# rpng/open_vins

Hardware: NVIDIA H100
Metric: msckf_updates_per_sec (higher is better)
Workload: dtype f64

## Files before the change

### open_vins_b200/csrc/chol_tiles.cuh

```cuda
#pragma once
#include "chol.cuh"
#ifdef CQ_PROBE
#include <cstdio>
#endif

#define CT_XP 12

__device__ __forceinline__ void ct_dmma(double &d0, double &d1, double a, double b) {
  asm volatile("mma.sync.aligned.m8n8k4.row.col.f64.f64.f64.f64 {%0,%1}, {%2}, {%3}, {%0,%1};" : "+d"(d0), "+d"(d1) : "d"(a), "d"(b));
}
__device__ __forceinline__ int ct_tri(int b) { return (b * (b + 1)) >> 1; }
__device__ __forceinline__ void ct_bar_group(int id, int nthreads) { asm volatile("bar.sync %0, %1;" ::"r"(id), "r"(nthreads) : "memory"); }
__device__ __forceinline__ size_t ct_idx(int i, int j) { return (size_t)(ct_tri(i >> 3) + (j >> 3)) * 64 + (i & 7) * 8 + (j & 7); }

struct CtView {
  double *T, *Xp0, *Xp1, *invd, *Linv0, *Linv1, *dummyT, *dummyX;
  int *flag;
};
__host__ __device__ inline size_t ct_view_doubles(int NRB) {
  return (size_t)((NRB * (NRB + 1)) / 2) * 64 + 2 * (size_t)NRB * 8 * CT_XP + (size_t)NRB * 8 + 128 + 64 + 2 * CT_XP;
}
__device__ __forceinline__ CtView ct_view_carve(double *base, int NRB, int *flag_word) {
  CtView v;
  v.T = base;
// ... 53 lines not shown
        d0 = (g == j) ? d * iv : d0 * iv;
    }
    const double lg = ag * iv, lc0 = ac0 * iv, lc1 = ac1 * iv;
    if (2 * q > j)
      d0 = fma(-lg, lc0, d0);
    if (2 * q + 1 > j)
      d1 = fma(-lg, lc1, d1);
  }
  if (lane < 8)
    invd[lane] = myinv;
  if (bad && lane == 0)
    *flag = 1;
}

__device__ __forceinline__ void ct_linv8(const double *Lt, const double *invd, double *Linv) {
  const int lane = threadIdx.x & 31, cc = lane & 7;
  double mc[8];
#pragma unroll
  for (int j = 0; j < 8; j++) {
    double s0 = (j == cc) ? 1.0 : 0.0, s1 = 0.0;
#pragma unroll
    for (int t = 0; t < j; t++) {
      if (t & 1)
        s1 = fma(-Lt[j * 8 + t], mc[t], s1);
      else
        s0 = fma(-Lt[j * 8 + t], mc[t], s0);
    }
    mc[j] = (s0 + s1) * invd[j];
  }
  if (lane < 8) {
#pragma unroll
    for (int i = 0; i < 8; i++)
      Linv[i * 8 + cc] = (i >= cc) ? mc[i] : 0.0;
  }
}

__device__ __forceinline__ void ct_panel_tile(const CtView &sm, int i, int k, const double *Linv, double *Xb) {
  const int lane = threadIdx.x & 31, g = lane >> 2, q = lane & 3;
  double *t = sm.T + (size_t)(ct_tri(i) + k) * 64;
  const double a0 = t[g * 8 + q], a1 = t[g * 8 + q + 4];
  const double b0 = Linv[g * 8 + q], b1 = Linv[g * 8 + q + 4];
  double2 d = make_double2(0.0, 0.0);
  ct_dmma(d.x, d.y, a0, b0);
  ct_dmma(d.x, d.y, a1, b1);
  *reinterpret_cast<double2 *>(t + 2 * lane) = d;
  *reinterpret_cast<double2 *>(Xb + (size_t)(8 * i + g) * CT_XP + 2 * q) = d;
}

__device__ __forceinline__ void ct_panel_rows(double *T, double *Xp, const double *invd, int i0, int stride, int nrows, int k, int nbk) {
  if (i0 >= nrows)
    return;
  const double *Lk = T + (size_t)(ct_tri(k) + k) * 64;
  double L[8][8], iv[8];
#pragma unroll
  for (int c = 0; c < 8; c++) {
    iv[c] = (c < nbk) ? invd[8 * k + c] : 0.0;
#pragma unroll
    for (int t2 = 0; t2 < 4; t2++) {
      if (2 * t2 < c) {
        const double2 v = *reinterpret_cast<const double2 *>(Lk + c * 8 + 2 * t2);
        L[c][2 * t2] = v.x;
        L[c][2 * t2 + 1] = v.y;
      }
    }
  }
  for (int i = i0; i < nrows; i += stride) {
    double *src = T + (size_t)(ct_tri(i >> 3) + k) * 64 + (i & 7) * 8;
    double v[8], x[8];
    {
      const double2 v01 = *reinterpret_cast<const double2 *>(src), v23 = *reinterpret_cast<const double2 *>(src + 2);
      const double2 v45 = *reinterpret_cast<const double2 *>(src + 4), v67 = *reinterpret_cast<const double2 *>(src + 6);
      v[0] = v01.x, v[1] = v01.y, v[2] = v23.x, v[3] = v23.y, v[4] = v45.x, v[5] = v45.y, v[6] = v67.x, v[7] = v67.y;
    }
#pragma unroll
    for (int c = 0; c < 8; c++) {
      x[c] = (c < nbk) ? v[c] * iv[c] : 0.0;
#pragma unroll
      for (int t = c + 1; t < 8; t++)
        v[t] = fma(-x[c], L[t][c], v[t]);
    }
    if (nbk == 8) {
      *reinterpret_cast<double2 *>(src) = make_double2(x[0], x[1]);
      *reinterpret_cast<double2 *>(src + 2) = make_double2(x[2], x[3]);
      *reinterpret_cast<double2 *>(src + 4) = make_double2(x[4], x[5]);
      *reinterpret_cast<double2 *>(src + 6) = make_double2(x[6], x[7]);
    } else {
#pragma unroll
      for (int c = 0; c < 8; c++)
        if (c < nbk)
          src[c] = x[c];
    }
    double *xp = Xp + (size_t)i * CT_XP;
    *reinterpret_cast<double2 *>(xp) = make_double2(x[0], x[1]);
    *reinterpret_cast<double2 *>(xp + 2) = make_double2(x[2], x[3]);
    *reinterpret_cast<double2 *>(xp + 4) = make_double2(x[4], x[5]);
    *reinterpret_cast<double2 *>(xp + 6) = make_double2(x[6], x[7]);
  }
}

struct CtTileOps {
  double a0, a1, b0, b1;
  double2 c;
  double2 *cp;
};
__device__ __forceinline__ void ct_tile_load(CtTileOps &o, const CtView &sm, const double *Xp, int bi, int bj, int lane, bool valid) {
  const int g = lane >> 2, q = lane & 3;
  const double *xa = valid ? Xp + (size_t)(8 * bi + g) * CT_XP + q : sm.dummyX + q;
  const double *xb = valid ? Xp + (size_t)(8 * bj + g) * CT_XP + q : sm.dummyX + q;
  o.cp = reinterpret_cast<double2 *>((valid ? sm.T + (size_t)(ct_tri(bi) + bj) * 64 : sm.dummyT) + 2 * lane);
  o.a0 = -xa[0];
  o.a1 = -xa[4];
  o.b0 = xb[0];
  o.b1 = xb[4];
  o.c = *o.cp;
}
__device__ __forceinline__ void ct_tile_mma(CtTileOps &o) {
  ct_dmma(o.c.x, o.c.y, o.a0, o.b0);
  ct_dmma(o.c.x, o.c.y, o.a1, o.b1);
}
__device__ __forceinline__ void ct_tile_mma_store(CtTileOps &o) {
  ct_tile_mma(o);
  *o.cp = o.c;
}

#ifdef CQ_PROBE
#define CT_PROBE_T(v) v = clock64()
#else
#define CT_PROBE_T(v) do { } while (0)
#endif

__device__ __forceinline__ void ct_trail_row(const CtView &sm, const double *Xk, int bi, int j0, int jmax, int lane) {
  const int g = lane >> 2, q = lane & 3;
  const double *xa = Xk + (size_t)(8 * bi + g) * CT_XP + q;
  const double a0 = -xa[0], a1 = -xa[4];
  double *trow = sm.T + (size_t)ct_tri(bi) * 64 + 2 * lane;
  for (int bj = j0; bj <= jmax; bj += 2) {
    const bool two = bj + 1 <= jmax;
    const double *xb0 = Xk + (size_t)(8 * bj + g) * CT_XP + q;
    const double *xb1 = two ? xb0 + 8 * CT_XP : sm.dummyX + q;
    double2 *c0p = reinterpret_cast<double2 *>(trow + (size_t)bj * 64);
    double2 *c1p = two ? c0p + 32 : reinterpret_cast<double2 *>(sm.dummyT + 2 * lane);
    const double b00 = xb0[0], b01 = xb0[4], b10 = xb1[0], b11 = xb1[4];
    double2 c0 = *c0p, c1 = *c1p;
    ct_dmma(c0.x, c0.y, a0, b00);
    ct_dmma(c1.x, c1.y, a0, b10);
    ct_dmma(c0.x, c0.y, a1, b01);
    ct_dmma(c1.x, c1.y, a1, b11);
    *c0p = c0;
    *c1p = c1;
  }
}

struct CtNoPublish {
  __device__ __forceinline__ void column(const CtView &, int) const {}
};
template <int THREADS, typename PUB = CtNoPublish>
__device__ __forceinline__ void ct_chol_tiles(const CtView &sm, int n, int nrows, bool strict, double floor_d, const PUB &pub = PUB()) {
  const int tid = threadIdx.x, lane = tid & 31, wid = tid >> 5;
  constexpr int NW = THREADS / 32, NH = NW - (NW + 3) / 4;
  static_assert(NH >= 1, "need at least one helper warp");
  const bool helper = (wid & 3) != 0;
  const int hr = wid - 1 - (wid >> 2);
  constexpr bool LINV = NW >= 8;
#ifdef CQ_PROBE
  long long p0 = 0, p1 = 0, p2 = 0, p3 = 0, p4 = 0, p5 = 0, acc[6] = {0, 0, 0, 0, 0, 0};
#endif
  const int NB = (n + 7) >> 3, NRB = (nrows + 7) >> 3;
  if (wid == 0) {
    double2 c = *reinterpret_cast<const double2 *>(sm.T + 2 * lane);
    ct_diag8_frag(c.x, c.y, min(8, n), sm.invd, strict, floor_d, sm.flag);
    *reinterpret_cast<double2 *>(sm.T + 2 * lane) = c;
    __syncwarp();
    if (LINV)
      asm volatile("bar.arrive 3, 64;" ::: "memory");
    ct_panel_rows(sm.T, sm.Xp0, sm.invd, lane < 8 ? 8 + lane : nrows, 1 << 30, nrows, 0, min(8, n));
  } else if (LINV && wid == 4) {
    asm volatile("bar.sync 3, 64;" ::: "memory");
    ct_linv8(sm.T, sm.invd, sm.Linv0);
  }
  __syncthreads();
  for (int k = 0; k < NB; k++) {
    const int par = k & 1;
    double *Xk = par ? sm.Xp1 : sm.Xp0, *Xn = par ? sm.Xp0 : sm.Xp1;
    const bool more = k + 1 < NB;
    CT_PROBE_T(p0);
#ifdef CQ_PROBE
    p1 = p2 = p3 = p4 = p0;
#endif
    if (wid == 0) {
      if (more) {
        const int k1 = k + 1, nbk1 = min(8, n - 8 * k1);
        CtTileOps o;
        ct_tile_load(o, sm, Xk, k1, k1, lane, true);
        ct_tile_mma(o);
        CT_PROBE_T(p1);
        ct_diag8_frag(o.c.x, o.c.y, nbk1, sm.invd + 8 * k1, strict, floor_d, sm.flag);
        *o.cp = o.c;
        __syncwarp();
        if (LINV)
          asm volatile("bar.arrive 3, 64;" ::: "memory");
        CT_PROBE_T(p2);
        asm volatile("bar.sync 2, %0;" ::"r"((NH + 1) * 32) : "memory");
        CT_PROBE_T(p3);
        ct_panel_rows(sm.T, Xn, sm.invd, lane < 8 ? 8 * (k + 2) + lane : nrows, 1 << 30, nrows, k1, nbk1);
        CT_PROBE_T(p4);
      }
    } else if (LINV && wid == 4) {
      if (more) {
        asm volatile("bar.sync 3, 64;" ::: "memory");
        ct_linv8(sm.T + (size_t)(ct_tri(k + 1) + k + 1) * 64, sm.invd + 8 * (k + 1), par ? sm.Linv0 : sm.Linv1);
      }
    } else if (helper) {
      if (LINV) {
        const double *Lk = par ? sm.Linv1 : sm.Linv0;
        for (int i = k + 2 + hr; i < NRB; i += NH)
          ct_panel_tile(sm, i, k, Lk, Xk);
      } else {
        ct_panel_rows(sm.T, Xk, sm.invd, 8 * (k + 2) + hr * 32 + lane, NH * 32, nrows, k, min(8, n - 8 * k));
      }
      if (NH > 1)
        ct_bar_group(1, NH * 32);
      else
        __syncwarp();
      CT_PROBE_T(p1);
      if (more) {
        for (int i = k + 2 + hr; i < NRB; i += 2 * NH) {
          CtTileOps o0, o1;
          ct_tile_load(o0, sm, Xk, i, k + 1, lane, true);
          ct_tile_load(o1, sm, Xk, i + NH, k + 1, lane, i + NH < NRB);
          ct_tile_mma_store(o0);
          ct_tile_mma_store(o1);
        }
        asm volatile("bar.arrive 2, %0;" ::"r"((NH + 1) * 32) : "memory");
        CT_PROBE_T(p2);
        const int R = NRB - (k + 2), jmaxc = NB - 1;
        for (int pr = hr; 2 * pr < R; pr += NH) {
          const int rb = R - 1 - pr;
          ct_trail_row(sm, Xk, k + 2 + rb, k + 2, min(k + 2 + rb, jmaxc), lane);
          if (rb != pr)
            ct_trail_row(sm, Xk, k + 2 + pr, k + 2, min(k + 2 + pr, jmaxc), lane);
        }
      }
      CT_PROBE_T(p3);
    } else if (wid == 8 && k > 0) {
      pub.column(sm, k - 1);
    }
    __syncthreads();
    CT_PROBE_T(p5);
#ifdef CQ_PROBE
    if (wid == 0) {
      acc[0] += p1 - p0, acc[1] += p2 - p1, acc[2] += p3 - p2, acc[3] += p4 - p3, acc[4] += p5 - p4;
    } else {
      acc[0] += p1 - p0, acc[1] += p2 - p1, acc[2] += p3 - p2, acc[3] += p5 - p3;
    }
    acc[5] += p5 - p0;
#endif
  }
#ifdef CQ_PROBE
  if (tid == 0)
    printf("chol n=%d W0 (cycles over %d steps): diag update %lld pivots %lld wait %lld rows below %lld step tail %lld | %lld\n", n, NB, acc[0], acc[1], acc[2], acc[3],
           acc[4], acc[5]);
  if (tid == 32 || tid == THREADS - 32)
    printf("chol n=%d helper warp %d: panel rows %lld column k+1 %lld trailing %lld wait %lld | %lld\n", n, wid, acc[0], acc[1], acc[2], acc[3], acc[5]);
#endif
}
```

### open_vins_b200/csrc/k_cholqr.cu

```cuda
#include "chol.cuh"
#include "chol_tiles.cuh"
#include "ovb_internal.cuh"
#include <math.h>
#include <cstdio>

#define CQ_MAXN 160
#define CQ_MAXB 20
#define CQ_MAXRB 22
#define CQ_GRAM_T 512
#define CQ_KB 32
#ifndef CQ_CHOL_T
#define CQ_CHOL_T 384
#endif
#define CQ_XP CT_XP
#define CQ_TRSM_T 640

namespace {

__device__ __forceinline__ void dmma(double &d0, double &d1, double a, double b) {
  asm volatile("mma.sync.aligned.m8n8k4.row.col.f64.f64.f64.f64 {%0,%1}, {%2}, {%3}, {%0,%1};" : "+d"(d0), "+d"(d1) : "d"(a), "d"(b));
}
__device__ __forceinline__ unsigned s_u32(const void *p) { return (unsigned)__cvta_generic_to_shared(p); }
__device__ __forceinline__ void cpa16(unsigned dst, const void *src, unsigned bytes) {
  asm volatile("cp.async.cg.shared.global [%0], [%1], 16, %2;" ::"r"(dst), "l"(src), "r"(bytes) : "memory");
}
__device__ __forceinline__ void cpa8(unsigned dst, const void *src, unsigned bytes) {
  asm volatile("cp.async.ca.shared.global [%0], [%1], 8, %2;" ::"r"(dst), "l"(src), "r"(bytes) : "memory");
}
__device__ __forceinline__ void cpa_commit() { asm volatile("cp.async.commit_group;" ::: "memory"); }
template <int N> __device__ __forceinline__ void cpa_wait() { asm volatile("cp.async.wait_group %0;" ::"n"(N) : "memory"); }
__device__ __forceinline__ void bar_group(int id, int nthreads) { asm volatile("bar.sync %0, %1;" ::"r"(id), "r"(nthreads) : "memory"); }
__device__ __forceinline__ int tri(int b) { return (b * (b + 1)) >> 1; }

__device__ __forceinline__ void cq_pub_store(unsigned long long *ctr, unsigned long long v) {
  asm volatile("st.release.gpu.global.u64 [%0], %1;" ::"l"(ctr), "l"(v) : "memory");
}
__device__ __forceinline__ unsigned long long cq_pub_load(const unsigned long long *ctr) {
  unsigned long long v;
  asm volatile("ld.acquire.gpu.global.u64 %0, [%1];" : "=l"(v) : "l"(ctr) : "memory");
  return v;
}
__device__ __forceinline__ void cq_fence_proxy() { asm volatile("fence.proxy.async.global;" ::: "memory"); }
__device__ __forceinline__ void cq_mbar_init(unsigned bar) { asm volatile("mbarrier.init.shared::cta.b64 [%0], 1;" ::"r"(bar) : "memory"); }
__device__ __forceinline__ void cq_mbar_arrive(unsigned bar) { asm volatile("mbarrier.arrive.shared::cta.b64 _, [%0];" ::"r"(bar) : "memory"); }
__device__ __forceinline__ void cq_mbar_wait(unsigned bar) {
  asm volatile("{\n\t.reg .pred p;\n\tCQ_MWAIT:\n\tmbarrier.try_wait.parity.shared::cta.b64 p, [%0], 0;\n\t@!p bra CQ_MWAIT;\n\t}" ::"r"(bar) : "memory");
}

__device__ __forceinline__ bool cq_tile_origin(int blk, int w, int BW, int nblk_side, int &ci, int &cj, int &offI, int &offJ, bool &diag) {
  int bI = 0, t = blk;
  while (t >= nblk_side - bI) {
    t -= nblk_side - bI;
    bI++;
  }
  const int bJ = bI + t;
  diag = (bI == bJ);
  int a, b;
  if (diag) {
    a = 0;
    int u = w;
    while (a < BW && u >= BW - a) {
      u -= BW - a;
      a++;
    }
    if (a >= BW)
      return false;
    b = a + u;
  } else {
    if (w >= BW * BW)
      return false;
    a = w / BW;
    b = w % BW;
  }
  offI = a * 32;
  offJ = (diag ? 0 : BW * 32) + b * 32;
  ci = (bI * BW + a) * 32;
  cj = (bJ * BW + b) * 32;
  return true;
}

template <int NT>
__device__ __forceinline__ void cq_issue_rows(double *buf, int pitch, const double *__restrict__ A, int ldA, int rc, int nrows, int r1, int nt, int cI0, int cJ0,
                                              int WI, int nrng) {
  const int units_per_row = nrng * WI / 2;
  for (int e = threadIdx.x; e < nrows * units_per_row; e += NT) {
    const int k = e / units_per_row, u = e - k * units_per_row;
    const int r = rc + k;
    const int dcol = 2 * u, col = (dcol < WI) ? cI0 + dcol : cJ0 + (dcol - WI);
    unsigned bytes = 0;
    if (r < r1)
      bytes = (col + 1 < nt) ? 16u : (col < nt ? 8u : 0u);
    const double *src = bytes ? (A + (size_t)r * ldA + col) : A;
    cpa16(s_u32(buf + (size_t)k * pitch + dcol), src, bytes);
  }
  cpa_commit();
}

__device__ __forceinline__ void cq_gram_kstep(double (&acc)[4][4][2], const double *row0, int pitch, int offI, int offJ, bool same, int g, int q) {
  const double *row = row0 + (size_t)q * pitch + g;
  double fa[4], fb[4];
#pragma unroll
  for (int b = 0; b < 4; b++)
    fa[b] = row[offI + 8 * b];
  if (same) {
#pragma unroll
    for (int b = 0; b < 4; b++)
      fb[b] = fa[b];
  } else {
#pragma unroll
    for (int b = 0; b < 4; b++)
      fb[b] = row[offJ + 8 * b];
  }
#pragma unroll
  for (int a = 0; a < 4; a++)
#pragma unroll
    for (int b = 0; b < 4; b++)
      dmma(acc[a][b][0], acc[a][b][1], fa[a], fb[b]);
}

}

__global__ void __launch_bounds__(CQ_GRAM_T) k_cq_gram(const double *__restrict__ A, int ldA, int m, int nt, int slab_rows, int BW, int nblk_side,
                                                      double *__restrict__ Gpart, int cs) {
  OVB_PDL_ENTER();
  extern __shared__ __align__(16) double gsm[];
  const int tid = threadIdx.x, lane = tid & 31, wid = tid >> 5, g = lane >> 2, q = lane & 3;
  int ci, cj, offI, offJ;
  bool diag;
  const bool active = cq_tile_origin(blockIdx.x, wid, BW, nblk_side, ci, cj, offI, offJ, diag);
  int bI = 0, tt = blockIdx.x;
  while (tt >= nblk_side - bI) {
    tt -= nblk_side - bI;
    bI++;
  }
  const int bJ = bI + tt;
  const int WI = BW * 32;
  const int nrng = (bI == bJ) ? 1 : 2;
  const int pitch = nrng * WI + 4;
  const int cI0 = bI * WI, cJ0 = bJ * WI;
  const int r0 = blockIdx.y * slab_rows, r1 = min(m, r0 + slab_rows);
  const int nchunks = (r1 > r0) ? (r1 - r0 + CQ_KB - 1) / CQ_KB : 0;
  double acc[4][4][2];
#pragma unroll
  for (int a = 0; a < 4; a++)
#pragma unroll
    for (int b = 0; b < 4; b++)
      acc[a][b][0] = acc[a][b][1] = 0.0;

  auto issue = [&](int c) { cq_issue_rows<CQ_GRAM_T>(gsm + (size_t)(c & 1) * CQ_KB * pitch, pitch, A, ldA, r0 + c * CQ_KB, CQ_KB, r1, nt, cI0, cJ0, WI, nrng); };
  if (nchunks > 0)
    issue(0);
  for (int c = 0; c < nchunks; c++) {
    if (c + 1 < nchunks) {
      issue(c + 1);
      cpa_wait<1>();
    } else {
      cpa_wait<0>();
    }
    __syncthreads();
    if (active) {
      const double *buf = gsm + (size_t)(c & 1) * CQ_KB * pitch;
#pragma unroll
      for (int ks = 0; ks < CQ_KB / 4; ks++)
        cq_gram_kstep(acc, buf + (size_t)4 * ks * pitch, pitch, offI, offJ, diag && offI == offJ, g, q);
    }
    __syncthreads();
  }
  if (cs <= 1) {
    if (active) {
      double *dst = Gpart + (((size_t)blockIdx.y * gridDim.x + blockIdx.x) * 16 + wid) * 1024;
#pragma unroll
      for (int a = 0; a < 4; a++)
#pragma unroll
        for (int b = 0; b < 4; b++)
          *reinterpret_cast<double2 *>(dst + (8 * a + g) * 32 + 8 * b + 2 * q) = make_double2(acc[a][b][0], acc[a][b][1]);
    }
    return;
  }
  double *stage = gsm;
  if (active) {
    double *dst = stage + (size_t)wid * 1024;
#pragma unroll
    for (int a = 0; a < 4; a++)
#pragma unroll
      for (int b = 0; b < 4; b++)
        *reinterpret_cast<double2 *>(dst + (8 * a + g) * 32 + 8 * b + 2 * q) = make_double2(acc[a][b][0], acc[a][b][1]);
  }
  asm volatile("barrier.cluster.arrive.release.aligned;" ::: "memory");
  asm volatile("barrier.cluster.wait.acquire.aligned;" ::: "memory");
  unsigned rank;
  asm volatile("mov.u32 %0, %%cluster_ctarank;" : "=r"(rank));
  if (active) {
    const int per = 1024 / cs;
    double *dst = Gpart + ((((size_t)blockIdx.y / cs) * gridDim.x + blockIdx.x) * 16 + wid) * 1024 + (size_t)rank * per;
    const unsigned base = s_u32(stage + (size_t)wid * 1024 + (size_t)rank * per);
    for (int e = lane; e < per; e += 32) {
      double sum = 0.0;
      for (int r = 0; r < cs; r++) {
        unsigned ra;
        double v;
        asm volatile("mapa.shared::cluster.u32 %0, %1, %2;" : "=r"(ra) : "r"(base + 8u * (unsigned)e), "r"((unsigned)r));
        asm volatile("ld.shared::cluster.f64 %0, [%1];" : "=d"(v) : "r"(ra) : "memory");
        sum += v;
      }
      dst[e] = sum;
    }
  }
  asm volatile("barrier.cluster.arrive.release.aligned;" ::: "memory");
  asm volatile("barrier.cluster.wait.acquire.aligned;" ::: "memory");
}

#define CQ_RED_T 1024
#define CQ_RED_CH 8
#define CQ_RED_GX (16 * CQ_RED_CH)
__global__ void __launch_bounds__(CQ_RED_T) k_cq_reduce(const double *__restrict__ Gpart, int nslab, int nblk, int BW, int nblk_side, int nt,
                                                       double *__restrict__ G, int ldG, int tiled) {
  OVB_PDL_ENTER();
  __shared__ double red[8][128];
  int ci, cj, offI, offJ;
  bool diag;
  const int w = blockIdx.x / CQ_RED_CH, ch = blockIdx.x % CQ_RED_CH, blk = blockIdx.y;
  if (!cq_tile_origin(blk, w, BW, nblk_side, ci, cj, offI, offJ, diag))
    return;
  if (ci >= nt || cj >= nt)
    return;
  const int el = threadIdx.x & 127, sg = threadIdx.x >> 7;
  const int e = ch * 128 + el;
  const double *src = Gpart + ((size_t)blk * 16 + w) * 1024 + e;
  const size_t stride = (size_t)nblk * 16 * 1024;
  double s0 = 0.0, s1 = 0.0;
  int sl = sg;
  for (; sl + 8 < nslab; sl += 16) {
    s0 += src[(size_t)sl * stride];
    s1 += src[(size_t)(sl + 8) * stride];
  }
  if (sl < nslab)
    s0 += src[(size_t)sl * stride];
  red[sg][el] = s0 + s1;
  __syncthreads();
  if (sg == 0) {
    const int i = ci + (e >> 5), j = cj + (e & 31);
    if (i < nt && j < nt && i <= j) {
      const double s = ((red[0][el] + red[1][el]) + (red[2][el] + red[3][el])) + ((red[4][el] + red[5][el]) + (red[6][el] + red[7][el]));
      if (tiled) {
        G[ct_idx(j, i)] = s;
        if ((i >> 3) == (j >> 3))
          G[(size_t)(tri(j >> 3) + (j >> 3)) * 64 + (i & 7) * 8 + (j & 7)] = s;
      } else {
        G[(size_t)i * ldG + j] = s;
        G[(size_t)j * ldG + i] = s;
      }
    }
  }
}

struct CqCholSmem {
  double T[(CQ_MAXRB * (CQ_MAXRB + 1) / 2) * 64];
  double Xp[2][CQ_MAXRB * 8 * CQ_XP];
  double invd[CQ_MAXRB * 8];
  double Linv[2][64];
  double red[32];
  double dummyT[64];
  double dummyX[2 * CQ_XP];
  int flag;
};

#define CQ_PK_INV ((CQ_MAXB * (CQ_MAXB + 1) / 2) * 64)
#define CQ_PK_DOUBLES (CQ_PK_INV + CQ_MAXB * 8)

namespace {

struct CqPublish {
  double *Lpk;
  unsigned long long *ctr, epoch;
  int n;
  __device__ __forceinline__ void column(const CtView &sm, int k) const {
    if (ctr == nullptr)
      return;
    const int lane = threadIdx.x & 31, NB = (n + 7) >> 3;
    for (int i = k; i < NB; i++) {
      const size_t o = (size_t)(ct_tri(i) + k) * 64 + 2 * lane;
      *reinterpret_cast<double2 *>(Lpk + o) = *reinterpret_cast<const double2 *>(sm.T + o);
    }
    if (lane < 8)
      Lpk[CQ_PK_INV + 8 * k + lane] = (8 * k + lane < n) ? sm.invd[8 * k + lane] : 1.0;
    cq_fence_proxy();
    __threadfence();
    __syncwarp();
    if (lane == 0)
      cq_pub_store(ctr, (epoch << 6) | (unsigned long long)(k + 2));
  }
  __device__ __forceinline__ int first_tile_el() const { return ctr ? (tri((n + 7) >> 3) - 1) * 64 : 0; }
  __device__ __forceinline__ int first_pivot() const { return ctr ? 8 * (((n + 7) >> 3) - 1) : 0; }
  __device__ __forceinline__ void finish() const {
    if (ctr == nullptr)
      return;
    cq_fence_proxy();
    __threadfence();
    __syncthreads();
    if (threadIdx.x == 0)
      cq_pub_store(ctr, (epoch << 6) | (unsigned long long)(((n + 7) >> 3) + 1));
  }
};

__device__ __forceinline__ void cq_chol_tiles(CqCholSmem &sm, int n, int nrows, bool strict, double floor_d, const CqPublish &pub) {
  CtView v;
  v.T = sm.T;
  v.Xp0 = sm.Xp[0];
  v.Xp1 = sm.Xp[1];
  v.invd = sm.invd;
  v.Linv0 = sm.Linv[0];
  v.Linv1 = sm.Linv[1];
  v.dummyT = sm.dummyT;
  v.dummyX = sm.dummyX;
  v.flag = &sm.flag;
  ct_chol_tiles<CQ_CHOL_T>(v, n, nrows, strict, floor_d, pub);
}

__device__ void cq_load_tiles(CqCholSmem &sm, const double *__restrict__ G, size_t ldG, int n, int nrows, const double *__restrict__ rhs, int ld_rhs) {
  const int tid = threadIdx.x, lane = tid & 31, wid = tid >> 5;
  const int NB = (n + 7) >> 3, NRB = (nrows + 7) >> 3;
  for (int i = wid; i < 8 * NRB; i += CQ_CHOL_T / 32) {
    const double *row = (i >= n && rhs != nullptr) ? rhs + (size_t)(i - n) * ld_rhs : G + (size_t)i * ldG;
    const int jmax = min(i | 7, 8 * NB - 1);
    double *dst = sm.T + (size_t)tri(i >> 3) * 64 + (i & 7) * 8;
    for (int j = 2 * lane; j <= jmax; j += 64) {
      unsigned bytes = 0;
      if (i < nrows)
        bytes = (j + 1 < n) ? 16u : (j < n ? 8u : 0u);
      cpa16(s_u32(dst + (size_t)(j >> 3) * 64 + (j & 7)), bytes ? (const void *)(row + j) : (const void *)G, bytes);
    }
  }
  cpa_commit();
  for (int e = tid; e < 2 * CQ_MAXRB * 8 * CQ_XP; e += CQ_CHOL_T)
    (&sm.Xp[0][0])[e] = 0.0;
  if (tid < 64)
    sm.dummyT[tid] = 0.0;
  if (tid < 2 * CQ_XP)
    sm.dummyX[tid] = 0.0;
  if (tid == 0)
    sm.flag = 0;
  cpa_wait<0>();
}

__device__ __forceinline__ double cq_el(const double *T, int i, int j) { return T[(size_t)(tri(i >> 3) + (j >> 3)) * 64 + (i & 7) * 8 + (j & 7)]; }

}

__global__ void __launch_bounds__(CQ_CHOL_T) k_cq_chol_gram(const double *__restrict__ G, int ldG, int n, double shift_rel, double *__restrict__ Lpk, int tiled,
                                                           unsigned long long *pub_ctr, unsigned long long epoch) {
  OVB_PDL_ENTER();
  if (pub_ctr != nullptr && threadIdx.x == 0)
    cq_pub_store(pub_ctr, (epoch << 6) | 1ull);
  const CqPublish pub{Lpk, pub_ctr, epoch, n};
  extern __shared__ __align__(16) unsigned char cq_raw[];
  CqCholSmem &sm = *reinterpret_cast<CqCholSmem *>(cq_raw);
  const int tid = threadIdx.x, lane = tid & 31, wid = tid >> 5;
#ifdef CQ_PROBE
  const long long q0 = clock64();
#endif
  if (tiled) {
    __shared__ __align__(8) unsigned long long g_bar;
    const unsigned bar = s_u32(&g_bar);
    const int NB = (n + 7) >> 3;
    if (tid == 0) {
      asm volatile("mbarrier.init.shared::cta.b64 [%0], 1;" ::"r"(bar) : "memory");
      asm volatile("fence.mbarrier_init.release.cluster;" ::: "memory");
    }
    __syncthreads();
    if (tid == 0) {
      const unsigned bytes = (unsigned)(tri(NB) * 64 * sizeof(double));
      asm volatile("mbarrier.arrive.expect_tx.shared::cta.b64 _, [%0], %1;" ::"r"(bar), "r"(bytes) : "memory");
      asm volatile("cp.async.bulk.shared::cluster.global.mbarrier::complete_tx::bytes [%0], [%1], %2, [%3];" ::"r"(s_u32(sm.T)), "l"(G), "r"(bytes), "r"(bar)
                   : "memory");
    }
    for (int e = tid; e < 2 * CQ_MAXRB * 8 * CQ_XP; e += CQ_CHOL_T)
      (&sm.Xp[0][0])[e] = 0.0;
    if (tid < 64)
      sm.dummyT[tid] = 0.0;
    if (tid < 2 * CQ_XP)
      sm.dummyX[tid] = 0.0;
    if (tid == 0)
      sm.flag = 0;
    asm volatile("{\n\t.reg .pred p;\n\tCQ_GWAIT:\n\tmbarrier.try_wait.parity.shared::cta.b64 p, [%0], 0;\n\t@p bra CQ_GDONE;\n\tbra CQ_GWAIT;\n\tCQ_GDONE:\n\t}" ::"r"(bar)
                 : "memory");
    const int r0 = n - 8 * (NB - 1);
    if (r0 < 8) {
      double *last = sm.T + (size_t)tri(NB - 1) * 64;
      for (int e = tid; e < NB * 64; e += CQ_CHOL_T)
        if (((e >> 3) & 7) >= r0)
          last[e] = 0.0;
    }
  } else {
    cq_load_tiles(sm, G, (size_t)ldG, n, n, nullptr, 0);
  }
  __syncthreads();
  double mx = 0.0;
  for (int i = tid; i < n; i += CQ_CHOL_T) {
    const double d = sm.T[(size_t)(tri(i >> 3) + (i >> 3)) * 64 + (i & 7) * 9];
    mx = (d > mx) ? d : mx;
  }
#pragma unroll
  for (int o = 16; o > 0; o >>= 1) {
    const double y = __shfl_xor_sync(0xffffffffu, mx, o);
    mx = (y > mx) ? y : mx;
  }
  if (lane == 0)
    sm.red[wid] = mx;
  __syncthreads();
  mx = 0.0;
  for (int w = 0; w < CQ_CHOL_T / 32; w++)
    mx = (sm.red[w] > mx) ? sm.red[w] : mx;
  const double shift = shift_rel * mx;
  for (int i = tid; i < n; i += CQ_CHOL_T)
    sm.T[(size_t)(tri(i >> 3) + (i >> 3)) * 64 + (i & 7) * 9] += shift;
  __syncthreads();
#ifdef CQ_PROBE
  const long long q1 = clock64();
#endif
  cq_chol_tiles(sm, n, n, false, 0.25 * shift, pub);
#ifdef CQ_PROBE
  const long long q2 = clock64();
#endif
  const int NB = (n + 7) >> 3;
  for (int e = pub.first_tile_el() + 2 * tid; e < tri(NB) * 64; e += 2 * CQ_CHOL_T)
// ... 13 lines not shown
  OVB_PDL_ENTER();
  if (pub_ctr != nullptr && threadIdx.x == 0)
    cq_pub_store(pub_ctr, (epoch << 6) | 1ull);
  const CqPublish pub{Lpk, pub_ctr, epoch, r};
  extern __shared__ __align__(16) unsigned char cq_raw[];
  CqCholSmem &sm = *reinterpret_cast<CqCholSmem *>(cq_raw);
  const int tid = threadIdx.x, lane = tid & 31, wid = tid >> 5;
  const int nrows = r + (res != nullptr ? 1 : 0);
  cq_load_tiles(sm, S, (size_t)ldS, r, nrows, res, 0);
  __syncthreads();
  if (floor_dev != nullptr)
    cq_chol_tiles(sm, r, nrows, false, *floor_dev, pub);
  else
    cq_chol_tiles(sm, r, nrows, true, 0.0, pub);
  if (Lpk != nullptr) {
    const int NB = (r + 7) >> 3;
    for (int e = pub.first_tile_el() + 2 * tid; e < tri(NB) * 64; e += 2 * CQ_CHOL_T)
      *reinterpret_cast<double2 *>(Lpk + e) = *reinterpret_cast<const double2 *>(sm.T + e);
    for (int e = pub.first_pivot() + tid; e < CQ_MAXB * 8; e += CQ_CHOL_T)
      Lpk[CQ_PK_INV + e] = (e < r) ? sm.invd[e] : 1.0;
    pub.finish();
  }
  for (int i = wid; i < r; i += CQ_CHOL_T / 32)
    for (int j = lane; j <= i; j += 32)
      S[(size_t)i * ldS + j] = cq_el(sm.T, i, j);
  if (res != nullptr)
    for (int j = tid; j < r; j += CQ_CHOL_T)
      w[j] = cq_el(sm.T, r, j);
  if (invdiag != nullptr)
    for (int j = tid; j < r; j += CQ_CHOL_T)
      invdiag[j] = sm.invd[j];
  if (tid == 0 && sm.flag && info != nullptr)
    info->not_spd = 1;
}

#define CQ_TRSM_NH 10
#define CQ_TRSM_SMEM (sizeof(double) * ((size_t)CQ_PK_DOUBLES + (size_t)(CQ_TRSM_T / 32) * CQ_TRSM_NH * 2 * 32))
template <int NH, bool WAIT = false>
__device__ __forceinline__ void cq_trsm_half(double (&acc)[NH][2], int b0, const double *Lt, const double *Ri, double *xs, int lane, unsigned cbar = 0) {
  const int g = lane >> 2, q = lane & 3;
#pragma unroll
  for (int jb = 0; jb < NH; jb++) {
    const int B = b0 + jb;
    if constexpr (WAIT)
      cq_mbar_wait(cbar + 8 * B);
    const double *Ld = Lt + (size_t)(tri(B) + B) * 64;
    const double *ri = Ri + B * 8;
    double x[8];
#pragma unroll
    for (int qq = 0; qq < 4; qq++) {
      x[2 * qq] = __shfl_sync(0xffffffffu, acc[jb][0], (lane & ~3) | qq);
      x[2 * qq + 1] = __shfl_sync(0xffffffffu, acc[jb][1], (lane & ~3) | qq);
    }
#pragma unroll
    for (int c = 0; c < 8; c++) {
      x[c] *= ri[c];
#pragma unroll
      for (int c2 = c + 1; c2 < 8; c2++)
        x[c2] -= x[c] * Ld[c2 * 8 + c];
    }
    acc[jb][0] = (q == 0) ? x[0] : (q == 1) ? x[2] : (q == 2) ? x[4] : x[6];
    acc[jb][1] = (q == 0) ? x[1] : (q == 1) ? x[3] : (q == 2) ? x[5] : x[7];
    const double af0 = -((q == 0) ? x[0] : (q == 1) ? x[1] : (q == 2) ? x[2] : x[3]);
    const double af1 = -((q == 0) ? x[4] : (q == 1) ? x[5] : (q == 2) ? x[6] : x[7]);
    if (xs != nullptr) {
      xs[(2 * jb) * 32 + lane] = af0;
      xs[(2 * jb + 1) * 32 + lane] = af1;
    }
#pragma unroll
    for (int j = jb + 1; j < NH; j++) {
      const double *lf = Lt + (size_t)(tri(b0 + j) + B) * 64 + g * 8 + q;
      dmma(acc[j][0], acc[j][1], af0, lf[0]);
      dmma(acc[j][0], acc[j][1], af1, lf[4]);
    }
  }
}

template <int NH>
__device__ __forceinline__ void cq_trsm_load(double (&acc)[NH][2], const double *arow, bool row_ok, int b0, int nt, int q) {
#pragma unroll
  for (int jb = 0; jb < NH; jb++) {
    const int col = 8 * (b0 + jb) + 2 * q;
    acc[jb][0] = acc[jb][1] = 0.0;
    if (row_ok) {
      if (col + 1 < nt) {
        const double2 v = *reinterpret_cast<const double2 *>(arow + col);
        acc[jb][0] = v.x;
        acc[jb][1] = v.y;
      } else if (col < nt) {
        acc[jb][0] = arow[col];
      }
    }
  }
}
template <int NH>
__device__ __forceinline__ void cq_trsm_store(const double (&acc)[NH][2], double *arow, bool row_ok, int b0, int nt, int q) {
  if (!row_ok)
    return;
#pragma unroll
  for (int jb = 0; jb < NH; jb++) {
    const int col = 8 * (b0 + jb) + 2 * q;
    if (col + 1 < nt)
      *reinterpret_cast<double2 *>(arow + col) = make_double2(acc[jb][0], acc[jb][1]);
    else if (col < nt)
      arow[col] = acc[jb][0];
  }
}

template <int NBP, int NT>
__device__ __forceinline__ void cq_fetch_factor(double *Lt, double *Ri, const double *__restrict__ Lpk, int NB) {
  const int tid = threadIdx.x;
  __shared__ __align__(8) unsigned long long l_bar;
  const unsigned bar = s_u32(&l_bar);
  if (tid == 0) {
    asm volatile("mbarrier.init.shared::cta.b64 [%0], 1;" ::"r"(bar) : "memory");
    asm volatile("fence.mbarrier_init.release.cluster;" ::: "memory");
  }
  __syncthreads();
  if (tid == 0) {
    const unsigned bytesL = (unsigned)(tri(NB) * 64 * sizeof(double)), bytesR = (unsigned)(NB * 8 * sizeof(double));
    asm volatile("mbarrier.arrive.expect_tx.shared::cta.b64 _, [%0], %1;" ::"r"(bar), "r"(bytesL + bytesR) : "memory");
    asm volatile("cp.async.bulk.shared::cluster.global.mbarrier::complete_tx::bytes [%0], [%1], %2, [%3];" ::"r"(s_u32(Lt)), "l"(Lpk), "r"(bytesL), "r"(bar)
                 : "memory");
    asm volatile("cp.async.bulk.shared::cluster.global.mbarrier::complete_tx::bytes [%0], [%1], %2, [%3];" ::"r"(s_u32(Ri)), "l"(Lpk + CQ_PK_INV), "r"(bytesR),
                 "r"(bar)
                 : "memory");
  }
  for (int e = tri(NB) * 64 + tid; e < tri(NBP) * 64; e += NT)
    Lt[e] = 0.0;
  for (int e = NB * 8 + tid; e < NBP * 8; e += NT)
    Ri[e] = 1.0;
  asm volatile("{\n\t.reg .pred p;\n\tCQ_LWAIT:\n\tmbarrier.try_wait.parity.shared::cta.b64 p, [%0], 0;\n\t@p bra CQ_LDONE;\n\tbra CQ_LWAIT;\n\tCQ_LDONE:\n\t}" ::"r"(bar)
               : "memory");
  __syncthreads();
}

template <int NBP, int NT>
__device__ __forceinline__ void cq_stream_init(unsigned long long *bars, double *Lt, double *Ri, int NB) {
  const int tid = threadIdx.x;
  if (tid == 0) {
    for (int j = 0; j <= NBP; j++)
      cq_mbar_init(s_u32(bars + j));
    asm volatile("fence.mbarrier_init.release.cluster;" ::: "memory");
  }
  for (int e = tri(NB) * 64 + tid; e < tri(NBP) * 64; e += NT)
    Lt[e] = 0.0;
  for (int e = NB * 8 + tid; e < NBP * 8; e += NT)
    Ri[e] = 1.0;
  __syncthreads();
}

#define CQ_STREAM_POLL_NS 20000000ull

__device__ void cq_stream_fetch(unsigned long long *bars, double *Lt, double *Ri, const double *__restrict__ Lpk, int NB, int NBP,
                                const unsigned long long *ctr, unsigned long long epoch) {
  const unsigned long long base = epoch << 6;
  unsigned long long t0, t;
  asm volatile("mov.u64 %0, %%globaltimer;" : "=l"(t0));
  bool poll = true;
  auto reach = [&](int s) {
    while (poll && cq_pub_load(ctr) < (base | (unsigned long long)s)) {
      asm volatile("mov.u64 %0, %%globaltimer;" : "=l"(t));
      if (t - t0 > CQ_STREAM_POLL_NS) {
        asm volatile("griddepcontrol.wait;" ::: "memory");
        poll = false;
      } else {
        __nanosleep(64);
      }
    }
  };
  reach(1);
  cq_mbar_arrive(s_u32(bars));
  for (int j = NB; j < NBP; j++)
    cq_mbar_arrive(s_u32(bars + 1 + j));
  for (int j = 0; j < NB; j++) {
    reach(j + 2);
    cq_fence_proxy();
    const unsigned bar = s_u32(bars + 1 + j);
    asm volatile("mbarrier.arrive.expect_tx.shared::cta.b64 _, [%0], %1;" ::"r"(bar), "r"((unsigned)((NB - j) * 64 + 8) * 8u) : "memory");
    for (int i = j; i < NB; i++) {
      const size_t o = (size_t)(tri(i) + j) * 64;
      asm volatile("cp.async.bulk.shared::cluster.global.mbarrier::complete_tx::bytes [%0], [%1], 512, [%2];" ::"r"(s_u32(Lt + o)), "l"(Lpk + o), "r"(bar)
                   : "memory");
    }
    asm volatile("cp.async.bulk.shared::cluster.global.mbarrier::complete_tx::bytes [%0], [%1], 64, [%2];" ::"r"(s_u32(Ri + 8 * j)), "l"(Lpk + CQ_PK_INV + 8 * j),
                 "r"(bar)
                 : "memory");
  }
  asm volatile("griddepcontrol.wait;" ::: "memory");
  for (int j = 0; j < NB; j++)
    cq_mbar_wait(s_u32(bars + 1 + j));
}

template <int NH1, int NH2, bool STREAM>
__device__ __forceinline__ void cq_trsm_rows(double *__restrict__ A, int ldA, int m, int nt, const double *__restrict__ Lpk,
                                             const unsigned long long *__restrict__ pub_ctr, unsigned long long epoch) {
  extern __shared__ __align__(16) double tsm[];
  double *Lt = tsm;
  double *Ri = tsm + CQ_PK_INV;
  double *Xs = tsm + CQ_PK_DOUBLES;
  const int tid = threadIdx.x, lane = tid & 31, wid = tid >> 5, g = lane >> 2, q = lane & 3;
  unsigned cbar = 0;
  if constexpr (STREAM) {
    asm volatile("griddepcontrol.launch_dependents;" ::: "memory");
    __shared__ __align__(8) unsigned long long bars[CQ_MAXB + 1];
    cq_stream_init<NH1 + NH2, CQ_TRSM_T>(bars, Lt, Ri, (nt + 7) >> 3);
    if (wid == CQ_TRSM_T / 32 - 1) {
      if (lane == 0)
        cq_stream_fetch(bars, Lt, Ri, Lpk, (nt + 7) >> 3, NH1 + NH2, pub_ctr, epoch);
      return;
    }
    cq_mbar_wait(s_u32(bars));
    cbar = s_u32(bars + 1);
  } else {
    OVB_PDL_ENTER();
    cq_fetch_factor<NH1 + NH2, CQ_TRSM_T>(Lt, Ri, Lpk, (nt + 7) >> 3);
  }
  double *xs = Xs + (size_t)wid * (CQ_TRSM_NH * 2 * 32);
  const int ngroups = (m + 7) >> 3;
  constexpr int NSW = CQ_TRSM_T / 32 - (STREAM ? 1 : 0);
  for (int rg = blockIdx.x + gridDim.x * wid; rg < ngroups; rg += gridDim.x * NSW) {
    const int row = 8 * rg + g;
    const bool row_ok = row < m;
    double *arow = A + (size_t)row * ldA;
#ifdef CQ_PROBE
    long long t0 = clock64(), t1, t2, t3 = 0, t4 = 0;
#endif
    {
      double acc[NH1][2];
      cq_trsm_load<NH1>(acc, arow, row_ok, 0, nt, q);
#ifdef CQ_PROBE
      t1 = clock64();
#endif
      cq_trsm_half<NH1, STREAM>(acc, 0, Lt, Ri, NH2 > 0 ? xs : nullptr, lane, cbar);
#ifdef CQ_PROBE
      t2 = clock64();
#endif
      cq_trsm_store<NH1>(acc, arow, row_ok, 0, nt, q);
    }
    if constexpr (NH2 > 0) {
      double acc[NH2][2];
      cq_trsm_load<NH2>(acc, arow, row_ok, NH1, nt, q);
      __syncwarp();
#pragma unroll 2
      for (int jb = 0; jb < NH1; jb++) {
        const double af0 = xs[(2 * jb) * 32 + lane], af1 = xs[(2 * jb + 1) * 32 + lane];
#pragma unroll
        for (int j = 0; j < NH2; j++) {
          const double *lf = Lt + (size_t)(tri(NH1 + j) + jb) * 64 + g * 8 + q;
          dmma(acc[j][0], acc[j][1], af0, lf[0]);
          dmma(acc[j][0], acc[j][1], af1, lf[4]);
        }
      }
#ifdef CQ_PROBE
      t3 = clock64();
#endif
      cq_trsm_half<NH2, STREAM>(acc, NH1, Lt, Ri, nullptr, lane, cbar);
#ifdef CQ_PROBE
      t4 = clock64();
#endif
      cq_trsm_store<NH2>(acc, arow, row_ok, NH1, nt, q);
      __syncwarp();
    }
#ifdef CQ_PROBE
    if (blockIdx.x == 0 && (tid == 0 || tid == 32 * 7) && rg < 40)
      printf("trsm rg=%d tid=%d: load %lld half1 %lld gemm+load %lld half2 %lld total %lld\n", rg, tid, t1 - t0, t2 - t1, t3 - t2, t4 - t3, clock64() - t0);
#endif
  }
}
template <int NH1, int NH2>
__global__ void __launch_bounds__(CQ_TRSM_T) k_cq_trsm(double *__restrict__ A, int ldA, int m, int nt, const double *__restrict__ Lpk) {
  cq_trsm_rows<NH1, NH2, false>(A, ldA, m, nt, Lpk, nullptr, 0);
}
template <int NH1, int NH2>
__global__ void __launch_bounds__(CQ_TRSM_T) k_cq_trsm(double *__restrict__ A, int ldA, int m, int nt, const double *__restrict__ Lpk,
                                                      const unsigned long long *__restrict__ pub_ctr, unsigned long long epoch) {
  cq_trsm_rows<NH1, NH2, true>(A, ldA, m, nt, Lpk, pub_ctr, epoch);
}
using CqTrsmKernel = void (*)(double *, int, int, int, const double *);
using CqTrsmStreamKernel = void (*)(double *, int, int, int, const double *, const unsigned long long *, unsigned long long);

template <bool STREAM>
static void cq_launch_trsm_t(ovb_ctx *ctx, int ctas, double *A, int ldA, int m, int nt, const double *Lpk, const unsigned long long *pub_ctr,
                             unsigned long long epoch) {
  const int NB = (nt + 7) / 8;
  const size_t smem = CQ_TRSM_SMEM;
  const dim3 grid(ctas), block(CQ_TRSM_T);
  auto go = [&](auto plain, auto streaming) {
    if constexpr (STREAM)
      ovb_launch(ctx, streaming, grid, block, smem, A, ldA, m, nt, Lpk, pub_ctr, epoch);
    else
      ovb_launch(ctx, plain, grid, block, smem, A, ldA, m, nt, Lpk);
  };
  if (NB <= 5)
    go((CqTrsmKernel)k_cq_trsm<5, 0>, (CqTrsmStreamKernel)k_cq_trsm<5, 0>);
  else if (NB <= 10)
    go((CqTrsmKernel)k_cq_trsm<10, 0>, (CqTrsmStreamKernel)k_cq_trsm<10, 0>);
  else if (NB <= 15)
    go((CqTrsmKernel)k_cq_trsm<10, 5>, (CqTrsmStreamKernel)k_cq_trsm<10, 5>);
  else
    go((CqTrsmKernel)k_cq_trsm<10, 10>, (CqTrsmStreamKernel)k_cq_trsm<10, 10>);
}
static void cq_launch_trsm(ovb_ctx *ctx, int ctas, double *A, int ldA, int m, int nt, const double *Lpk, const unsigned long long *pub_ctr = nullptr,
                           unsigned long long epoch = 0) {
  if (pub_ctr != nullptr)
    cq_launch_trsm_t<true>(ctx, ctas, A, ldA, m, nt, Lpk, pub_ctr, epoch);
  else
    cq_launch_trsm_t<false>(ctx, ctas, A, ldA, m, nt, Lpk, pub_ctr, epoch);
}

#define CQ_SG_SMEM (226 * 1024)

__host__ __device__ __forceinline__ int cq_sg_pitch(int BW, int NBP) {
  const int w = (8 * NBP > 32 * BW) ? 8 * NBP : 32 * BW;
  return ((w + 15) & ~15) + 4;
}

template <int NH1, int NH2>
__device__ __forceinline__ void cq_solve_group(double *xrow, bool row_ok, const double *Lt, const double *Ri, int lane, unsigned cbar) {
  constexpr int NBP = NH1 + NH2;
  const int g = lane >> 2, q = lane & 3;
  {
    double acc[NH1][2];
    cq_trsm_load<NH1>(acc, xrow, row_ok, 0, 8 * NBP, q);
    cq_trsm_half<NH1, true>(acc, 0, Lt, Ri, nullptr, lane, cbar);
    cq_trsm_store<NH1>(acc, xrow, row_ok, 0, 8 * NBP, q);
  }
  if constexpr (NH2 > 0) {
    double acc[NH2][2];
    __syncwarp();
    cq_trsm_load<NH2>(acc, xrow, row_ok, NH1, 8 * NBP, q);
#pragma unroll 2
    for (int jb = 0; jb < NH1; jb++) {
      const double af0 = -xrow[8 * jb + q], af1 = -xrow[8 * jb + 4 + q];
#pragma unroll
      for (int j = 0; j < NH2; j++) {
        const double *lf = Lt + (size_t)(tri(NH1 + j) + jb) * 64 + g * 8 + q;
        dmma(acc[j][0], acc[j][1], af0, lf[0]);
        dmma(acc[j][0], acc[j][1], af1, lf[4]);
      }
    }
    cq_trsm_half<NH2, true>(acc, NH1, Lt, Ri, nullptr, lane, cbar);
    cq_trsm_store<NH2>(acc, xrow, row_ok, NH1, 8 * NBP, q);
  }
}

template <int NH1, int NH2>
__global__ void __launch_bounds__(CQ_GRAM_T) k_cq_solve_gram(const double *__restrict__ A, int ldA, int m, int nt, const double *__restrict__ Lpk, int slab_rows,
                                                          int cb, int ntail_max, int BW, double *__restrict__ Gpart, double *__restrict__ Qtail,
                                                          const unsigned long long *__restrict__ pub_ctr, unsigned long long epoch) {
  asm volatile("griddepcontrol.launch_dependents;" ::: "memory");
  extern __shared__ __align__(16) double ssm[];
  double *Lt = ssm;
  double *Ri = ssm + CQ_PK_INV;
  double *X = ssm + CQ_PK_DOUBLES;
  constexpr int NBP = NH1 + NH2;
  const int pitch = cq_sg_pitch(BW, NBP);
  const int r0 = blockIdx.x * slab_rows, r1 = min(m, r0 + slab_rows);
  double *tail = Qtail + (size_t)blockIdx.x * ntail_max * pitch;
  auto split_at = [&](int rc) { return r1 - rc > cb && r1 - rc <= 8 * (CQ_GRAM_T / 32); };
  auto nbuf_at = [&](int rc) { return split_at(rc) ? cb & ~7 : min(cb, (r1 - rc + 3) & ~3); };
  constexpr int NF = CQ_GRAM_T - 32;
  const int lane = threadIdx.x & 31, wid = threadIdx.x >> 5, g = lane >> 2, q = lane & 3, lr = 8 * wid + g;
  const bool fetcher = threadIdx.x >= NF;
  __shared__ __align__(8) unsigned long long bars[CQ_MAXB + 1];
  cq_stream_init<NBP, CQ_GRAM_T>(bars, Lt, Ri, (nt + 7) >> 3);
  const unsigned cbar = s_u32(bars + 1);
  if (fetcher) {
    if (lane == 0)
      cq_stream_fetch(bars, Lt, Ri, Lpk, (nt + 7) >> 3, NBP, pub_ctr, epoch);
    __syncwarp();
  } else {
    cq_mbar_wait(s_u32(bars));
    if (r0 < r1)
      cq_issue_rows<NF>(X, pitch, A, ldA, r0, nbuf_at(r0), r1, nt, 0, 0, pitch - 4, 1);
  }
  for (int rc = r0, nbuf = nbuf_at(r0), ntail = 0; rc < r1; rc += nbuf + ntail, nbuf = nbuf_at(rc)) {
    ntail = split_at(rc) ? (r1 - rc - nbuf + 3) & ~3 : 0;
    const int nact = nbuf + ntail;
    const bool first = rc == r0;
    if (!first)
      cq_issue_rows<CQ_GRAM_T>(X, pitch, A, ldA, rc, nbuf, r1, nt, 0, 0, pitch - 4, 1);
    if (!(first && fetcher))
      for (int e = threadIdx.x; e < ntail * (pitch - 4); e += first ? NF : CQ_GRAM_T) {
        const int k = e / (pitch - 4), col = e - k * (pitch - 4), r = rc + nbuf + k;
        tail[(size_t)k * pitch + col] = (r < r1 && col < nt) ? A[(size_t)r * ldA + col] : 0.0;
      }
    cpa_wait<0>();
    if (!first) {
      bar_group(1, CQ_GRAM_T);
    } else if (fetcher) {
      asm volatile("bar.sync 3, %0;" ::"n"(CQ_GRAM_T) : "memory");
    } else {
      asm volatile("bar.arrive 3, %0;" ::"n"(CQ_GRAM_T) : "memory");
      bar_group(2, NF);
    }
    if (8 * wid < nbuf)
      cq_solve_group<NH1, NH2>(X + (size_t)min(lr, nbuf - 1) * pitch, lr < nbuf, Lt, Ri, lane, cbar);
    else if (8 * wid < nact)
      cq_solve_group<NH1, NH2>(tail + (size_t)min(lr - nbuf, ntail - 1) * pitch, lr < nact, Lt, Ri, lane, cbar);
    bar_group(1, CQ_GRAM_T);
    int ci, cj, offI, offJ;
    bool diag;
    const bool active = cq_tile_origin(0, wid, BW, 1, ci, cj, offI, offJ, diag);
    double *part = Gpart + ((size_t)blockIdx.x * 16 + wid) * 1024 + g * 32 + 2 * q;
    if (active) {
      double acc[4][4][2];
#pragma unroll
      for (int a = 0; a < 4; a++)
#pragma unroll
        for (int b = 0; b < 4; b++) {
          const double2 v = rc > r0 ? *reinterpret_cast<const double2 *>(part + a * 256 + 8 * b) : make_double2(0.0, 0.0);
          acc[a][b][0] = v.x;
          acc[a][b][1] = v.y;
        }
#pragma unroll 1
      for (int k = 0; k < nact; k += 4)
        cq_gram_kstep(acc, k < nbuf ? X + (size_t)k * pitch : tail + (size_t)(k - nbuf) * pitch, pitch, offI, offJ, offI == offJ, g, q);
#pragma unroll
      for (int a = 0; a < 4; a++)
#pragma unroll
        for (int b = 0; b < 4; b++)
          *reinterpret_cast<double2 *>(part + a * 256 + 8 * b) = make_double2(acc[a][b][0], acc[a][b][1]);
    }
    bar_group(1, CQ_GRAM_T);
  }
}

struct CqSgShape {
  int pitch, cb, ntail;
};
static CqSgShape cq_sg_shape(int nt, int BW, int slab_rows) {
  const int NB = (nt + 7) / 8, NBP = NB <= 5 ? 5 : NB <= 10 ? 10 : NB <= 15 ? 15 : 20;
  CqSgShape s;
  s.pitch = cq_sg_pitch(BW, NBP);
  const int round = slab_rows < 8 * (CQ_GRAM_T / 32) ? slab_rows : 8 * (CQ_GRAM_T / 32);
  const int fit = (int)((CQ_SG_SMEM - sizeof(double) * CQ_PK_DOUBLES) / (sizeof(double) * s.pitch)) & ~3;
  s.cb = fit < round ? fit : round;
  s.ntail = slab_rows > s.cb ? round - (s.cb & ~7) : 0;
  return s;
}
static size_t cq_solve_gram_scratch(int nslab, int nt, int BW, int slab_rows) {
  const CqSgShape s = cq_sg_shape(nt, BW, slab_rows);
  return (size_t)nslab * s.ntail * s.pitch;
}

template <int NH1, int NH2>
static void cq_launch_solve_gram_t(ovb_ctx *ctx, int nslab, const double *A, int ldA, int m, int nt, const double *Lpk, int slab_rows, int BW, double *Gpart,
                                   double *Qtail, const unsigned long long *pub_ctr, unsigned long long epoch) {
  const CqSgShape s = cq_sg_shape(nt, BW, slab_rows);
  const size_t smem = sizeof(double) * (CQ_PK_DOUBLES + (size_t)s.cb * s.pitch);
  ovb_launch(ctx, k_cq_solve_gram<NH1, NH2>, dim3(nslab), dim3(CQ_GRAM_T), smem, A, ldA, m, nt, Lpk, slab_rows, s.cb, s.ntail, BW, Gpart, Qtail, pub_ctr, epoch);
}
static void cq_launch_solve_gram(ovb_ctx *ctx, int nslab, const double *A, int ldA, int m, int nt, const double *Lpk, int slab_rows, int BW, double *Gpart,
                                 double *Qtail, const unsigned long long *pub_ctr, unsigned long long epoch) {
  const int NB = (nt + 7) / 8;
  if (NB <= 5)
    cq_launch_solve_gram_t<5, 0>(ctx, nslab, A, ldA, m, nt, Lpk, slab_rows, BW, Gpart, Qtail, pub_ctr, epoch);
  else if (NB <= 10)
    cq_launch_solve_gram_t<10, 0>(ctx, nslab, A, ldA, m, nt, Lpk, slab_rows, BW, Gpart, Qtail, pub_ctr, epoch);
  else if (NB <= 15)
    cq_launch_solve_gram_t<10, 5>(ctx, nslab, A, ldA, m, nt, Lpk, slab_rows, BW, Gpart, Qtail, pub_ctr, epoch);
  else
    cq_launch_solve_gram_t<10, 10>(ctx, nslab, A, ldA, m, nt, Lpk, slab_rows, BW, Gpart, Qtail, pub_ctr, epoch);
}

__global__ void __launch_bounds__(256) k_cq_trmm(const double *__restrict__ L2, const double *__restrict__ L1, int nt, double *__restrict__ Rout, int ldR) {
  OVB_PDL_ENTER();
  __shared__ double As[16][CQ_MAXN + 1];
  __shared__ double Bs[CQ_MAXN][17];
  const int ti = blockIdx.y, tj = blockIdx.x;
  const int tid = threadIdx.x, tx = tid & 15, ty = tid >> 4;
  const int n = nt - 1;
  const int i = ti * 16 + ty, j = tj * 16 + tx;
  double acc = 0.0;
  if (tj >= ti) {
    const int k0 = ti * 16, k1 = min(nt, tj * 16 + 16);
    const int K = k1 - k0;
    for (int e = tid; e < 16 * K; e += 256) {
      const int a = e / K, k = e - a * K;
      const int ii = ti * 16 + a, kk = k0 + k;
      As[a][k] = (ii < nt && kk >= ii) ? L2[(size_t)(tri(kk >> 3) + (ii >> 3)) * 64 + (kk & 7) * 8 + (ii & 7)] : 0.0;
    }
    for (int e = tid; e < 16 * K; e += 256) {
      const int k = e >> 4, b = e & 15;
      const int kk = k0 + k, jj = tj * 16 + b;
      Bs[k][b] = (jj < nt && jj >= kk) ? L1[(size_t)(tri(jj >> 3) + (kk >> 3)) * 64 + (jj & 7) * 8 + (kk & 7)] : 0.0;
    }
    __syncthreads();
    double a0 = 0.0, a1 = 0.0, a2 = 0.0, a3 = 0.0;
    int k = 0;
    for (; k + 3 < K; k += 4) {
      a0 += As[ty][k] * Bs[k][tx];
      a1 += As[ty][k + 1] * Bs[k + 1][tx];
      a2 += As[ty][k + 2] * Bs[k + 2][tx];
      a3 += As[ty][k + 3] * Bs[k + 3][tx];
    }
    for (; k < K; k++)
      a0 += As[ty][k] * Bs[k][tx];
    acc = (a0 + a1) + (a2 + a3);
  }
  if (i < n && j < nt)
    Rout[(size_t)i * ldR + j] = (j >= i) ? acc : 0.0;
}

#define CQ_GN_T 256
__global__ void __launch_bounds__(CQ_GN_T) k_cq_gemm_nt(double *__restrict__ C, int ldc, const double *__restrict__ A, int lda, const double *__restrict__ B,
                                                       int ldb, int M, int N, int K, int lower_only) {
  OVB_PDL_ENTER();
  __shared__ __align__(16) double As[64][36];
  __shared__ __align__(16) double Bs[64][36];
  const int m0 = blockIdx.y * 64, n0 = blockIdx.x * 64;
  if (lower_only && n0 > m0 + 63)
    return;
  const int tid = threadIdx.x, lane = tid & 31, wid = tid >> 5, g = lane >> 2, q = lane & 3;
  const int wm = (wid >> 2) * 32, wn = (wid & 3) * 16;
  double acc[4][2][2];
#pragma unroll
  for (int a = 0; a < 4; a++)
#pragma unroll
    for (int b = 0; b < 2; b++)
      acc[a][b][0] = acc[a][b][1] = 0.0;
  for (int k0 = 0; k0 < K; k0 += 32) {
    for (int e = tid; e < 64 * 16; e += CQ_GN_T) {
      const int r = e >> 4, u = e & 15, k = k0 + 2 * u;
      unsigned ba = 0, bb = 0;
      if (m0 + r < M)
        ba = (k + 1 < K) ? 16u : (k < K ? 8u : 0u);
      if (n0 + r < N)
        bb = (k + 1 < K) ? 16u : (k < K ? 8u : 0u);
      cpa16(s_u32(&As[r][2 * u]), ba ? (const void *)(A + (size_t)(m0 + r) * lda + k) : (const void *)A, ba);
      cpa16(s_u32(&Bs[r][2 * u]), bb ? (const void *)(B + (size_t)(n0 + r) * ldb + k) : (const void *)B, bb);
    }
    cpa_commit();
    cpa_wait<0>();
    __syncthreads();
#pragma unroll
    for (int ks = 0; ks < 8; ks++) {
      double fa[4], fb[2];
#pragma unroll
      for (int a = 0; a < 4; a++)
        fa[a] = As[wm + 8 * a + g][4 * ks + q];
#pragma unroll
      for (int b = 0; b < 2; b++)
        fb[b] = Bs[wn + 8 * b + g][4 * ks + q];
#pragma unroll
      for (int a = 0; a < 4; a++)
#pragma unroll
        for (int b = 0; b < 2; b++)
          dmma(acc[a][b][0], acc[a][b][1], fa[a], fb[b]);
    }
    __syncthreads();
  }
#pragma unroll
  for (int a = 0; a < 4; a++)
#pragma unroll
    for (int b = 0; b < 2; b++) {
      const int i = m0 + wm + 8 * a + g, j = n0 + wn + 8 * b + 2 * q;
      if (i < M) {
        double *c = C + (size_t)i * ldc + j;
        if (j + 1 < N) {
          double2 v = *reinterpret_cast<double2 *>(c);
          v.x -= acc[a][b][0];
          v.y -= acc[a][b][1];
          *reinterpret_cast<double2 *>(c) = v;
        } else if (j < N) {
          c[0] -= acc[a][b][0];
        }
      }
    }
}

__global__ void __launch_bounds__(256) k_cq_shift(double *__restrict__ G, int ldG, int n, double shift_rel, double *__restrict__ floor_out) {
  OVB_PDL_ENTER();
  __shared__ double red[8];
  double mx = 0.0;
  for (int i = threadIdx.x; i < n; i += 256) {
    const double d = G[(size_t)i * ldG + i];
    mx = (d > mx) ? d : mx;
  }
#pragma unroll
  for (int o = 16; o > 0; o >>= 1) {
    const double y = __shfl_xor_sync(0xffffffffu, mx, o);
    mx = (y > mx) ? y : mx;
  }
  if ((threadIdx.x & 31) == 0)
    red[threadIdx.x >> 5] = mx;
  __syncthreads();
  mx = 0.0;
  for (int w = 0; w < 8; w++)
    mx = (red[w] > mx) ? red[w] : mx;
  const double shift = shift_rel * mx;
  for (int i = threadIdx.x; i < n; i += 256)
    G[(size_t)i * ldG + i] += shift;
  if (threadIdx.x == 0)
    *floor_out = 0.25 * shift;
}

__global__ void __launch_bounds__(256) k_cq_trmm_wide(const double *__restrict__ L2, const double *__restrict__ L1, int ldL, int nt, double *__restrict__ Rout,
                                                     int ldR) {
  OVB_PDL_ENTER();
  __shared__ double As[32][33];
  __shared__ double Bs[32][33];
  const int ti = blockIdx.y, tj = blockIdx.x;
  const int tid = threadIdx.x, tx = tid & 31, ty = tid >> 5;
  const int n = nt - 1;
  double acc[4] = {0, 0, 0, 0};
  if (tj >= ti) {
    for (int tk = ti; tk <= tj; tk++) {
      for (int e = tid; e < 1024; e += 256) {
        const int a = e >> 5, b = e & 31;
        const int k = tk * 32 + a, i = ti * 32 + b;
        As[a][b] = (k < nt && i < nt && k >= i) ? L2[(size_t)k * ldL + i] : 0.0;
        const int j = tj * 32 + a, k2 = tk * 32 + b;
        Bs[a][b] = (j < nt && k2 < nt && j >= k2) ? L1[(size_t)j * ldL + k2] : 0.0;
      }
      __syncthreads();
#pragma unroll 8
      for (int kk = 0; kk < 32; kk++) {
        const double b = Bs[tx][kk];
#pragma unroll
        for (int u = 0; u < 4; u++)
          acc[u] += As[kk][ty + 8 * u] * b;
      }
      __syncthreads();
    }
  }
#pragma unroll
  for (int u = 0; u < 4; u++) {
    const int i = ti * 32 + ty + 8 * u, j = tj * 32 + tx;
    if (i < n && j < nt)
      Rout[(size_t)i * ldR + j] = (j >= i) ? acc[u] : 0.0;
  }
}

#define CQ_GRAM_CS 4
static void cq_launch_gram(ovb_ctx *ctx, int nblk, int nslab_padded, size_t smem, const double *A, int ldA, int m, int nt, int slab_rows, int BW, int nblk_side,
                           double *Gpart, int cs) {
  cudaLaunchConfig_t cfg = {};
  cfg.gridDim = dim3(nblk, nslab_padded);
  cfg.blockDim = dim3(CQ_GRAM_T);
  cfg.dynamicSmemBytes = smem;
  cfg.stream = ctx->stream;
  cudaLaunchAttribute at[2];
  int na = 0;
  if (ctx->tsqr_pdl && !ctx->prof_on) {
    at[na].id = cudaLaunchAttributeProgrammaticStreamSerialization;
    at[na].val.programmaticStreamSerializationAllowed = 1;
    na++;
  }
  if (cs > 1) {
    at[na].id = cudaLaunchAttributeClusterDimension;
    at[na].val.clusterDim.x = 1;
    at[na].val.clusterDim.y = cs;
    at[na].val.clusterDim.z = 1;
    na++;
// ... 61 lines not shown
  double *Lpk = nullptr;
  if (cq_ensure_G(ctx)) {
    const int ldW = CQ_MAXN + 8;
    Lpk = ctx->d_G + (size_t)3 * ldW * ldW;
  }
  const unsigned long long epoch = (epoch_out != nullptr && Lpk != nullptr) ? ++ctx->pub_epoch : 0;
  ovb_launch(ctx, k_cq_chol_ekf, dim3(1), dim3(CQ_CHOL_T), sizeof(CqCholSmem), S, ldS, r, res, w, invdiag, ctx->d_info, Lpk, (const double *)nullptr,
             epoch ? ctx->d_pub : (unsigned long long *)nullptr, epoch);
  if (Lpk_out)
    *Lpk_out = Lpk;
  if (epoch_out)
    *epoch_out = epoch;
  return true;
}

bool launch_trsm_rows(ovb_ctx *ctx, double *A, int ldA, int m, int nt, const double *Lpk, unsigned long long epoch) {
  if (nt > CQ_MAXN || (ldA & 1) || m < 1 || Lpk == nullptr)
    return false;
  cq_attrs(ctx);
  const int ngroups = (m + 7) / 8;
  int ctas = ngroups;
  if (ctas > ctx->sm_count)
    ctas = ctx->sm_count;
  cq_launch_trsm(ctx, ctas, A, ldA, m, nt, Lpk, epoch ? ctx->d_pub : nullptr, epoch);
  return true;
}

#define CQ_WB 128
#define CQ_WMAX 520
#define CQ_WBLOCKS ((CQ_WMAX + CQ_WB - 1) / CQ_WB)
static bool cq_ensure_wide(ovb_ctx *ctx) {
  const size_t need = (size_t)2 * CQ_WMAX * CQ_WMAX + (size_t)2 * CQ_WBLOCKS * CQ_PK_DOUBLES + 64;
  if (need > ctx->cqw_cap) {
    if (ctx->d_cqw)
      cudaFree(ctx->d_cqw);
    ctx->d_cqw = nullptr;
    if (cudaMalloc(&ctx->d_cqw, sizeof(double) * need) != cudaSuccess)
      return false;
    ctx->cqw_cap = need;
  }
  return true;
}
static void cq_gemm_nt(ovb_ctx *ctx, double *C, int ldc, const double *A, int lda, const double *B, int ldb, int M, int N, int K, int lower_only) {
  if (M <= 0 || N <= 0 || K <= 0)
    return;
  ovb_launch(ctx, k_cq_gemm_nt, dim3((N + 63) / 64, (M + 63) / 64), dim3(CQ_GN_T), (size_t)0, C, ldc, A, lda, B, ldb, M, N, K, lower_only);
}
static void cq_trsm_any(ovb_ctx *ctx, double *A, int ldA, int m, int nt, const double *Lpk) {
  const int ngroups = (m + 7) / 8;
  int ctas = (ngroups + CQ_TRSM_T / 32 - 1) / (CQ_TRSM_T / 32);
  if (ngroups <= ctx->sm_count)
    ctas = ngroups;
  if (ctas > ctx->sm_count)
    ctas = ctx->sm_count;
  cq_launch_trsm(ctx, ctas, A, ldA, m, nt, Lpk);
}
static void cq_chol_blocked(ovb_ctx *ctx, double *S, int ld, int n, int extra, double *Lpk, const double *floor_dev, DevUpdateInfo *info) {
  for (int J = 0, b = 0; J < n; J += CQ_WB, b++) {
    const int nb = (n - J < CQ_WB) ? n - J : CQ_WB;
    double *Lb = Lpk + (size_t)b * CQ_PK_DOUBLES;
    ovb_launch(ctx, k_cq_chol_ekf, dim3(1), dim3(CQ_CHOL_T), sizeof(CqCholSmem), S + (size_t)J * ld + J, ld, nb, (const double *)nullptr, (double *)nullptr,
               (double *)nullptr, info, Lb, floor_dev, (unsigned long long *)nullptr, 0ull);
    const int mrem = n + extra - (J + nb);
    if (mrem > 0) {
      double *panel = S + (size_t)(J + nb) * ld + J;
      cq_trsm_any(ctx, panel, ld, mrem, nb, Lb);
      const int ncols = n - (J + nb);
      cq_gemm_nt(ctx, S + (size_t)(J + nb) * ld + (J + nb), ld, panel, ld, panel, ld, mrem, ncols, nb, 1);
    }
  }
}
static void cq_trsm_blocked(ovb_ctx *ctx, double *X, int ldx, int m, int n, const double *S, int ld, const double *Lpk) {
  for (int J = 0, b = 0; J < n; J += CQ_WB, b++) {
    const int nb = (n - J < CQ_WB) ? n - J : CQ_WB;
    if (J > 0)
      cq_gemm_nt(ctx, X + J, ldx, X, ldx, S + (size_t)J * ld, ld, m, nb, J, 0);
    cq_trsm_any(ctx, X + J, ldx, m, nb, Lpk + (size_t)b * CQ_PK_DOUBLES);
  }
}

__global__ void k_cq_copy_row(const double *__restrict__ src, double *__restrict__ dst, int n) {
  OVB_PDL_ENTER();
  const int i = blockIdx.x * blockDim.x + threadIdx.x;
  if (i < n)
    dst[i] = src[i];
}
__global__ void k_cq_inv_diag(const double *__restrict__ S, int ld, int n, double *__restrict__ inv) {
  OVB_PDL_ENTER();
  const int i = blockIdx.x * blockDim.x + threadIdx.x;
  if (i < n) {
    const double d = S[(size_t)i * ld + i];
    inv[i] = d != 0.0 ? 1.0 / d : 0.0;
  }
}

bool launch_chol_solve_wide(ovb_ctx *ctx, double *S, int ldS, int r, double *w, double *invdiag, double *M, int ldM, int N, bool gate_only) {
  if (r > CQ_WMAX - 8 || (ldS & 1) || (ldM & 1) || r + 1 > ctx->cfg.max_state + 1)
    return false;
  cq_attrs(ctx);
  if (!cq_ensure_wide(ctx))
    return false;
  double *Lpk = ctx->d_cqw + (size_t)2 * CQ_WMAX * CQ_WMAX;
  ovb_launch(ctx, k_cq_copy_row, dim3((r + 127) / 128), dim3(128), (size_t)0, (const double *)w, S + (size_t)r * ldS, r);
  cq_chol_blocked(ctx, S, ldS, r, 1, Lpk, nullptr, ctx->d_info);
  ovb_launch(ctx, k_cq_copy_row, dim3((r + 127) / 128), dim3(128), (size_t)0, (const double *)(S + (size_t)r * ldS), w, r);
  ovb_launch(ctx, k_cq_inv_diag, dim3((r + 127) / 128), dim3(128), (size_t)0, (const double *)S, ldS, r, invdiag);
  if (!gate_only)
    cq_trsm_blocked(ctx, M, ldM, N, r, S, ldS, Lpk);
  return true;
}

static int cq_compress_wide(ovb_ctx *ctx, double *A, int m, int n, int ldA, double *Rout, int ldR) {
  const int nt = n + 1;
  if (nt > CQ_WMAX - 7 || !cq_ensure_wide(ctx))
    return -1;
  const int nT = (nt + 31) / 32, BW = 4, nblk_side = (nT + BW - 1) / BW, nblk = nblk_side * (nblk_side + 1) / 2;
  int nslab = ctx->sm_count / nblk;
  if (nslab < 1)
    nslab = 1;
  const int max_slabs = (m + CQ_KB - 1) / CQ_KB;
  if (nslab > max_slabs)
    nslab = max_slabs;
  int slab_rows = (((m + nslab - 1) / nslab) + 3) & ~3;
  nslab = (m + slab_rows - 1) / slab_rows;
  const size_t need_part = (size_t)nslab * nblk * 16 * 1024;
  if (need_part > ctx->Gpart_cap) {
    if (ctx->d_Gpart)
      cudaFree(ctx->d_Gpart);
    ctx->d_Gpart = nullptr;
    if (cudaMalloc(&ctx->d_Gpart, sizeof(double) * need_part) != cudaSuccess)
      return -1;
    ctx->Gpart_cap = need_part;
  }
  double *G1 = ctx->d_cqw, *G2 = G1 + (size_t)CQ_WMAX * CQ_WMAX, *Lpk1 = G2 + (size_t)CQ_WMAX * CQ_WMAX, *Lpk2 = Lpk1 + (size_t)CQ_WBLOCKS * CQ_PK_DOUBLES;
  double *floor_dev = Lpk2 + (size_t)CQ_WBLOCKS * CQ_PK_DOUBLES;
  const size_t gram_smem = sizeof(double) * 2 * CQ_KB * (size_t)(2 * BW * 32 + 4);
  int launches = 0;
  for (int pass = 0; pass < 2; pass++) {
    double *G = pass == 0 ? G1 : G2;
    cq_launch_gram(ctx, nblk, nslab, gram_smem, (const double *)A, ldA, m, nt, slab_rows, BW, nblk_side, ctx->d_Gpart, 1);
    ovb_launch(ctx, k_cq_reduce, dim3(CQ_RED_GX, nblk), dim3(CQ_RED_T), (size_t)0, (const double *)ctx->d_Gpart, nslab, nblk, BW, nblk_side, nt, G, (int)CQ_WMAX, 0);
    ovb_launch(ctx, k_cq_shift, dim3(1), dim3(256), (size_t)0, G, (int)CQ_WMAX, nt, pass == 0 ? 1e-11 : 1e-13, floor_dev + pass);
    cq_chol_blocked(ctx, G, CQ_WMAX, nt, 0, pass == 0 ? Lpk1 : Lpk2, floor_dev + pass, (DevUpdateInfo *)nullptr);
    if (pass == 0)
      cq_trsm_blocked(ctx, A, ldA, m, nt, G1, CQ_WMAX, Lpk1);
    launches += 3 + 3 * ((nt + CQ_WB - 1) / CQ_WB);
  }
  const int nT32 = (nt + 31) / 32;
  ovb_launch(ctx, k_cq_trmm_wide, dim3(nT32, nT32), dim3(256), (size_t)0, (const double *)G2, (const double *)G1, (int)CQ_WMAX, nt, Rout, ldR);
  ctx->n_launch += launches + 1;
  return launches + 1;
}

int launch_compress_cholqr2(ovb_ctx *ctx, double *A, int m, int n, int ldA, double *Rout, int ldR) {
  const int nt = n + 1;
  if ((ldA & 1) || m < 1)
    return -1;
  cq_attrs(ctx);
  if (nt > CQ_MAXN)
    return cq_compress_wide(ctx, A, m, n, ldA, Rout, ldR);
  const int nT = (nt + 31) / 32;
  const int BW = nT, nblk_side = 1, nblk = 1;
  int nslab = ctx->sm_count;
  const int max_slabs = (m + CQ_KB - 1) / CQ_KB;
  if (nslab > max_slabs)
    nslab = max_slabs;
  int slab_rows = (m + nslab - 1) / nslab;
  slab_rows = (slab_rows + 3) & ~3;
  nslab = (m + slab_rows - 1) / slab_rows;
  const int cs = (ctx->gram_cluster && nslab >= 2 * CQ_GRAM_CS) ? CQ_GRAM_CS : 1;
  const int nslab_pad = (nslab + cs - 1) / cs * cs, npart = nslab_pad / cs;
  const size_t part_doubles = (size_t)nslab_pad * nblk * 16 * 1024;
  const size_t need_part = part_doubles + cq_solve_gram_scratch(nslab, nt, BW, slab_rows);
  const int ldW = CQ_MAXN + 8;
  if (!cq_ensure_G(ctx))
    return -1;
  if (need_part > ctx->Gpart_cap) {
    const size_t cap = need_part + need_part / 2;
    if (ctx->d_Gpart)
      cudaFree(ctx->d_Gpart);
    ctx->d_Gpart = nullptr;
    ctx->Gpart_cap = 0;
    if (cudaMalloc(&ctx->d_Gpart, sizeof(double) * cap) != cudaSuccess)
      return -1;
    ctx->Gpart_cap = cap;
  }
  double *G = ctx->d_G, *L1 = G + (size_t)ldW * ldW, *L2 = L1 + (size_t)ldW * ldW;
  static_assert(CQ_PK_DOUBLES <= (CQ_MAXN + 8) * (CQ_MAXN + 8), "packed factor must fit its slot");
  size_t gram_smem = sizeof(double) * 2 * CQ_KB * (size_t)(BW * 32 + 4);
  if (cs > 1 && gram_smem < sizeof(double) * 16 * 1024)
    gram_smem = sizeof(double) * 16 * 1024;
  cq_launch_gram(ctx, nblk, nslab_pad, gram_smem, (const double *)A, ldA, m, nt, slab_rows, BW, nblk_side, ctx->d_Gpart, cs);
  ovb_launch(ctx, k_cq_reduce, dim3(CQ_RED_GX, nblk), dim3(CQ_RED_T), (size_t)0, (const double *)ctx->d_Gpart, npart, nblk, BW, nblk_side, nt, G, ldW, 1);
  const unsigned long long epoch = ++ctx->pub_epoch;
  ovb_launch(ctx, k_cq_chol_gram, dim3(1), dim3(CQ_CHOL_T), sizeof(CqCholSmem), (const double *)G, ldW, nt, 1e-11, L1, 1, ctx->d_pub, epoch);
  cq_launch_solve_gram(ctx, nslab, (const double *)A, ldA, m, nt, (const double *)L1, slab_rows, BW, ctx->d_Gpart, ctx->d_Gpart + part_doubles, ctx->d_pub, epoch);
  ovb_launch(ctx, k_cq_reduce, dim3(CQ_RED_GX, nblk), dim3(CQ_RED_T), (size_t)0, (const double *)ctx->d_Gpart, nslab, nblk, BW, nblk_side, nt, G, ldW, 1);
  ovb_launch(ctx, k_cq_chol_gram, dim3(1), dim3(CQ_CHOL_T), sizeof(CqCholSmem), (const double *)G, ldW, nt, 1e-13, L2, 1, (unsigned long long *)nullptr, 0ull);
  const int nT16 = (nt + 15) / 16;
  ovb_launch(ctx, k_cq_trmm, dim3(nT16, nT16), dim3(256), (size_t)0, (const double *)L2, (const double *)L1, nt, Rout, ldR);
  ctx->n_launch += 7;
  return 7;
}
```

### open_vins_b200/csrc/k_ekf.cu

```cuda
#include "chol.cuh"
#include "ovb_internal.cuh"

#define EK_T 32

__global__ void __launch_bounds__(256) k_ekf_gemm(int mode, const double *__restrict__ P, int ldP, const double *__restrict__ H, int ldH,
                                                  const double *__restrict__ Min, int ldM, const DevUpdateInfo *__restrict__ info, int X, int Y,
                                                  int K, double *__restrict__ Cout, int ldC, double sigma2, const double *__restrict__ Rdiag) {
  OVB_PDL_ENTER();
  __shared__ double As[EK_T][EK_T + 1];
  __shared__ double Bs[EK_T][EK_T + 1];
  const int x0 = blockIdx.x * EK_T, y0 = blockIdx.y * EK_T;
  if (mode == 1 && y0 > x0 + EK_T - 1)
    return;
  const int tid = threadIdx.x, tx = tid & 31, ty = tid >> 5;
  double acc[4] = {0, 0, 0, 0};
  const int *cs = info->col_state;
  for (int j0 = 0; j0 < K; j0 += EK_T) {
    for (int e = tid; e < EK_T * EK_T; e += 256) {
      int jj = e >> 5, q = e & 31;
      int j = j0 + jj;
      double av = 0.0, bv = 0.0;
      if (j < K) {
        if (mode == 0) {
          int a = x0 + q;
// ... 192 lines not shown
    if (a < N && b < N && b >= a) {
      double v = P[(size_t)a * ldP + b] - acc[u];
      P[(size_t)a * ldP + b] = v;
      P[(size_t)b * ldP + a] = v;
      if (a == b && v < 0.0)
        atomicMin(&info->neg_diag_index, a);
      if (!isfinite(v))
        info->nonfinite = 1;
    }
  }
  if (a0 == b0 && tid < EK_T && a0 + tid < N)
    dx[a0 + tid] = dxa;
}

#define EK1_KMAX 160
__device__ __forceinline__ void ek_cpa8(double *dst_smem, const double *src) {
  asm volatile("cp.async.ca.shared.global [%0], [%1], 8;" ::"r"((unsigned)__cvta_generic_to_shared(dst_smem)), "l"(src) : "memory");
}
__global__ void __launch_bounds__(256) k_ekf_gemm1(int mode, const double *__restrict__ P, int ldP, const double *__restrict__ H, int ldH,
                                                   const double *__restrict__ Min, int ldM, const DevUpdateInfo *__restrict__ info, int X, int Y,
                                                   int K, double *__restrict__ Cout, int ldC, double sigma2, const double *__restrict__ Rdiag) {
  OVB_PDL_ENTER();
  extern __shared__ __align__(16) double g1[];
  const int x0 = blockIdx.x * EK_T, y0 = blockIdx.y * EK_T;
  if (mode == 1 && y0 > x0 + EK_T - 1)
    return;
  const int tid = threadIdx.x, tx = tid & 31, ty = tid >> 5;
  const int *cs = info->col_state;
  const int pk = K | 1;
  double *Gs = g1, *Hs = g1 + (size_t)K * 33;
  const double *Gsrc = (mode == 0) ? P : Min;
  const int ldG = (mode == 0) ? ldP : ldM;
  const int g0 = (mode == 0) ? x0 : y0, gmax = (mode == 0) ? X : Y;
  const int h0 = (mode == 0) ? y0 : x0, hmax = (mode == 0) ? Y : X;
  __shared__ int cs_s[EK1_KMAX];
  for (int j = tid; j < K; j += 256)
    cs_s[j] = cs[j];
  __syncthreads();
  for (int e = tid; e < K * 32; e += 256) {
    const int j = e >> 5, a = e & 31;
    if (g0 + a < gmax)
      ek_cpa8(&Gs[j * 33 + a], &Gsrc[(size_t)cs_s[j] * ldG + g0 + a]);
    else
      Gs[j * 33 + a] = 0.0;
  }
  for (int i = ty; i < 32; i += 8)
    for (int j = tx; j < K; j += 32) {
      if (h0 + i < hmax)
        ek_cpa8(&Hs[i * pk + j], &H[(size_t)(h0 + i) * ldH + j]);
      else
        Hs[i * pk + j] = 0.0;
    }
  asm volatile("cp.async.commit_group;" ::: "memory");
  asm volatile("cp.async.wait_group 0;" ::: "memory");
  __syncthreads();
  double acc[4] = {0, 0, 0, 0};
  if (mode == 0) {
    for (int j = 0; j < K; j++) {
      const double gv = Gs[j * 33 + tx];
#pragma unroll
      for (int u = 0; u < 4; u++)
        acc[u] += gv * Hs[(ty + 8 * u) * pk + j];
    }
#pragma unroll
    for (int u = 0; u < 4; u++) {
      const int a = x0 + tx, i = y0 + ty + 8 * u;
      if (a < X && i < Y)
        Cout[(size_t)a * ldC + i] = acc[u];
    }
  } else {
    for (int j = 0; j < K; j++) {
      const double gv = Gs[j * 33 + tx];
#pragma unroll
      for (int u = 0; u < 4; u++)
        acc[u] += Hs[(ty + 8 * u) * pk + j] * gv;
    }
#pragma unroll
    for (int u = 0; u < 4; u++) {
      const int i = x0 + ty + 8 * u, k = y0 + tx;
      if (i < X && k < Y) {
        double v = acc[u];
        if (i == k)
          v += Rdiag ? Rdiag[i] : sigma2;
        Cout[(size_t)i * ldC + k] = v;
      }
    }
  }
}

__global__ void __launch_bounds__(256) k_ekf_downdate1(double *__restrict__ P, int ldP, const double *__restrict__ Yin, int ldY, int N, int r,
                                                       const double *__restrict__ w, double *__restrict__ dx, DevUpdateInfo *__restrict__ info) {
  OVB_PDL_ENTER();
  extern __shared__ __align__(16) double d1[];
  const int a0 = blockIdx.x * EK_T, b0 = blockIdx.y * EK_T;
  if (b0 < a0)
    return;
  const int tid = threadIdx.x, tx = tid & 31, ty = tid >> 5;
  if (info->not_spd) {
    if (a0 == b0 && tid < EK_T && a0 + tid < N)
      dx[a0 + tid] = 0.0;
    return;
  }
  const int pk = r | 1;
  double *As = d1, *Bs = d1 + (size_t)32 * pk, *ws = Bs + (size_t)32 * pk;
  for (int i = ty; i < 32; i += 8)
    for (int k = tx; k < r; k += 32) {
      if (a0 + i < N)
        ek_cpa8(&As[i * pk + k], &Yin[(size_t)(a0 + i) * ldY + k]);
      else
        As[i * pk + k] = 0.0;
      if (b0 + i < N)
        ek_cpa8(&Bs[i * pk + k], &Yin[(size_t)(b0 + i) * ldY + k]);
      else
        Bs[i * pk + k] = 0.0;
    }
  for (int k = tid; k < r; k += 256)
    ek_cpa8(&ws[k], &w[k]);
  asm volatile("cp.async.commit_group;" ::: "memory");
  asm volatile("cp.async.wait_group 0;" ::: "memory");
  __syncthreads();
  double acc[4] = {0, 0, 0, 0};
  for (int k = 0; k < r; k++) {
    const double bv = Bs[tx * pk + k];
#pragma unroll
    for (int u = 0; u < 4; u++)
      acc[u] += As[(ty + 8 * u) * pk + k] * bv;
  }
#pragma unroll
  for (int u = 0; u < 4; u++) {
    const int a = a0 + ty + 8 * u, b = b0 + tx;
    if (a < N && b < N && b >= a) {
      const double v = P[(size_t)a * ldP + b] - acc[u];
      P[(size_t)a * ldP + b] = v;
      P[(size_t)b * ldP + a] = v;
      if (a == b && v < 0.0)
        atomicMin(&info->neg_diag_index, a);
      if (!isfinite(v))
        info->nonfinite = 1;
    }
  }
  if (a0 == b0 && tid < EK_T && a0 + tid < N) {
    double s0 = 0.0, s1 = 0.0;
    int k = 0;
    for (; k + 1 < r; k += 2) {
      s0 += As[tid * pk + k] * ws[k];
      s1 += As[tid * pk + k + 1] * ws[k + 1];
    }
    if (k < r)
      s0 += As[tid * pk + k] * ws[k];
    dx[a0 + tid] = s0 + s1;
  }
}

__global__ void k_ekf_prep(DevUpdateInfo *info, const int *skip) {
  OVB_PDL_ENTER();
  info->neg_diag_index = 0x7fffffff;
  info->not_spd = (skip && *skip) ? 1 : 0;
  info->nonfinite = 0;
}

void launch_ekf_update(ovb_ctx *ctx, const double *H, int ldHm, int r, int n, bool gate_only, double sigma2, const double *Rdiag_dev,
                       const int *skip_dev) {
  const int N = ctx->N;
  const int ld = ctx->ldP;
  double *P = ctx->P[ctx->cur];
  ovb_launch(ctx, k_ekf_prep, dim3(1), dim3(1), (size_t)(0), ctx->d_info, skip_dev);
  if (r <= 0 || n <= 0)
    return;
  if (!ctx->attr_done[2]) {
    cudaFuncSetAttribute(k_ekf_chol, cudaFuncAttributeMaxDynamicSharedMemorySize, 200 * 1024);
    cudaFuncSetAttribute(k_ekf_trsm, cudaFuncAttributeMaxDynamicSharedMemorySize, 200 * 1024);
    cudaFuncSetAttribute(k_ekf_gemm1, cudaFuncAttributeMaxDynamicSharedMemorySize, 100 * 1024);
    cudaFuncSetAttribute(k_ekf_downdate1, cudaFuncAttributeMaxDynamicSharedMemorySize, 100 * 1024);
    ctx->attr_done[2] = 1;
  }
  const bool one_shot = ctx->ekf_chol_dmma && n <= EK1_KMAX && r <= EK1_KMAX;
  dim3 g0((N + EK_T - 1) / EK_T, (r + EK_T - 1) / EK_T);
  dim3 g1((r + EK_T - 1) / EK_T, (r + EK_T - 1) / EK_T);
  if (one_shot) {
    const size_t sm01 = sizeof(double) * ((size_t)n * 33 + (size_t)32 * (n | 1));
    ovb_launch(ctx, k_ekf_gemm1, dim3(g0), dim3(256), sm01, 0, P, ld, H, ldHm, nullptr, 0, ctx->d_info, N, r, n, ctx->d_M, ld, 0.0, nullptr);
    ovb_launch(ctx, k_ekf_gemm1, dim3(g1), dim3(256), sm01, 1, P, ld, H, ldHm, ctx->d_M, ld, ctx->d_info, r, r, n, ctx->d_S, ld, sigma2, Rdiag_dev);
  } else {
    ovb_launch(ctx, k_ekf_gemm, dim3(g0), dim3(256), (size_t)(0), 0, P, ld, H, ldHm, nullptr, 0, ctx->d_info, N, r, n, ctx->d_M, ld, 0.0, nullptr);
    ovb_launch(ctx, k_ekf_gemm, dim3(g1), dim3(256), (size_t)(0), 1, P, ld, H, ldHm, ctx->d_M, ld, ctx->d_info, r, r, n, ctx->d_S, ld, sigma2, Rdiag_dev);
  }
  size_t chol_bytes = sizeof(double) * (size_t)(r + 1) * (size_t)(r | 1);
  int use_smem = chol_bytes <= 200 * 1024;
  double *invdiag = ctx->d_w + ctx->cfg.max_state;
  double *Lpk = nullptr;
  unsigned long long epoch = 0;
  const bool dmma_chol = ctx->ekf_chol_dmma && launch_chol_ekf_dmma(ctx, ctx->d_S, ld, r, ctx->d_w, ctx->d_w, invdiag, &Lpk, gate_only ? nullptr : &epoch);
  const bool wide = !dmma_chol && ctx->ekf_chol_dmma && r < ld && launch_chol_solve_wide(ctx, ctx->d_S, ld, r, ctx->d_w, invdiag, ctx->d_M, ld, N, gate_only);
  if (wide) {
    if (gate_only)
      return;
    dim3 g2w((N + EK_T - 1) / EK_T, (N + EK_T - 1) / EK_T);
    ovb_launch(ctx, k_ekf_downdate, dim3(g2w), dim3(256), (size_t)(0), P, ld, (const double *)ctx->d_M, ld, N, r, ctx->d_w, ctx->d_dx, ctx->d_info);
    return;
  }
  if (!dmma_chol)
    ovb_launch(ctx, k_ekf_chol, dim3(1), dim3(EKC_THREADS), (size_t)(use_smem ? chol_bytes : 0), ctx->d_S, ld, r, ctx->d_w, ctx->d_w, invdiag, ctx->d_info, use_smem);
  if (gate_only)
    return;
  const double *Yd = ctx->d_Y;
  if (dmma_chol && Lpk != nullptr && launch_trsm_rows(ctx, ctx->d_M, ld, N, r, Lpk, epoch)) {
    Yd = ctx->d_M;
  } else {
    size_t trsm_small = sizeof(double) * ((size_t)TR_ROWS * r + r);
    size_t trsm_full = trsm_small + sizeof(double) * (size_t)r * (size_t)(r | 1);
    int L_in_smem = trsm_full <= 200 * 1024;
    ovb_launch(ctx, k_ekf_trsm, dim3((N + TR_ROWS - 1) / TR_ROWS), dim3(32 * TR_ROWS), (size_t)(L_in_smem ? trsm_full : trsm_small), ctx->d_M, ld, ctx->d_S, ld, invdiag, N,
               r, ctx->d_Y, ld, L_in_smem, ctx->d_info);
  }
  dim3 g2((N + EK_T - 1) / EK_T, (N + EK_T - 1) / EK_T);
  if (one_shot) {
    const size_t smd = sizeof(double) * ((size_t)64 * (r | 1) + r);
    ovb_launch(ctx, k_ekf_downdate1, dim3(g2), dim3(256), smd, P, ld, Yd, ld, N, r, ctx->d_w, ctx->d_dx, ctx->d_info);
  } else {
    ovb_launch(ctx, k_ekf_downdate, dim3(g2), dim3(256), (size_t)(0), P, ld, Yd, ld, N, r, ctx->d_w, ctx->d_dx, ctx->d_info);
  }
}


__global__ void k_cov_init_augment(double *__restrict__ P, int ld, int N, int k, int n, const DevUpdateInfo *__restrict__ info,
                                   const double *__restrict__ Hx, const double *__restrict__ Hinv, double sigma2, const int *__restrict__ skip) {
  extern __shared__ double ism[];
  double *m = ism, *M = ism + (size_t)N * k;
  const int tid = threadIdx.x;
  if (skip && *skip)
    return;
  for (int a = tid; a < N; a += blockDim.x) {
    for (int i = 0; i < k; i++) {
      double acc = 0.0;
      for (int j = 0; j < n; j++)
        acc += P[(size_t)a * ld + info->col_state[j]] * Hx[i * n + j];
      m[a * k + i] = acc;
    }
  }
  __syncthreads();
  if (tid < k * k) {
    const int i = tid / k, i2 = tid % k;
    double acc = 0.0;
    for (int j = 0; j < n; j++)
      acc += Hx[i * n + j] * m[info->col_state[j] * k + i2];
    M[i * k + i2] = acc + (i == i2 ? sigma2 : 0.0);
  }
  __syncthreads();
  if (tid < k * k) {
    const int i = tid / k, i2 = tid % k;
    if (i2 < i)
      M[i * k + i2] = M[i2 * k + i];
  }
  __syncthreads();
  for (int a = tid; a < N; a += blockDim.x) {
    for (int q = 0; q < k; q++) {
      double acc = 0.0;
      for (int i = 0; i < k; i++)
        acc += m[a * k + i] * Hinv[q * k + i];
      P[(size_t)a * ld + N + q] = -acc;
      P[(size_t)(N + q) * ld + a] = -acc;
    }
  }
  if (tid < k * k) {
    const int q = tid / k, q2 = tid % k;
    double acc = 0.0;
    for (int i = 0; i < k; i++)
      for (int i2 = 0; i2 < k; i2++)
        acc += Hinv[q * k + i] * M[i * k + i2] * Hinv[q2 * k + i2];
    if (q <= q2) {
      P[(size_t)(N + q) * ld + N + q2] = acc;
      P[(size_t)(N + q2) * ld + N + q] = acc;
    }
  }
}

bool launch_cov_init_augment(ovb_ctx *ctx, int k, int n, const double *Hx_dev, const double *Hinv_dev, double sigma2, const int *skip_dev) {
  const int N = ctx->N;
  size_t smem = sizeof(double) * ((size_t)N * k + (size_t)k * k);
  if (smem > 200 * 1024)
    return false;
  if (!ctx->attr_done[5]) {
    cudaFuncSetAttribute(k_cov_init_augment, cudaFuncAttributeMaxDynamicSharedMemorySize, 200 * 1024);
    ctx->attr_done[5] = 1;
  }
  k_cov_init_augment<<<1, 256, smem, ctx->stream>>>(ctx->P[ctx->cur], ctx->ldP, N, k, n, ctx->d_info, Hx_dev, Hinv_dev, sigma2, skip_dev);
  return cudaGetLastError() == cudaSuccess;
}

__global__ void k_init_prep(const DevFeat *__restrict__ feat, DevInitSys *__restrict__ sys, DevUpdateInfo *__restrict__ info, int k, int n) {
  const int tid = threadIdx.x;
  const bool ok = feat->status == OVB_FEAT_OK;
  if (ok)
    for (int j = tid; j < n; j += blockDim.x)
      info->col_state[j] = sys->col_state[j];
  if (tid != 0)
    return;
  sys->status = feat->status;
  sys->chi2 = feat->chi2;
  int fail = sys->n != n ? 2 : 0;
  const int o = 3 - k;
  double A[9], Inv[9];
  for (int i = 0; i < k; i++)
    for (int j = 0; j < k; j++) {
      A[i * k + j] = sys->HL[(o + i) * 3 + o + j];
      Inv[i * k + j] = (i == j) ? 1.0 : 0.0;
    }
  for (int c0 = 0; c0 < k && !fail; c0++) {
    int piv = c0;
    for (int i = c0 + 1; i < k; i++)
      if (fabs(A[i * k + c0]) > fabs(A[piv * k + c0]))
        piv = i;
    if (!(fabs(A[piv * k + c0]) > 0.0)) {
      fail = 1;
      break;
    }
    if (piv != c0)
      for (int j = 0; j < k; j++) {
        double t = A[c0 * k + j];
        A[c0 * k + j] = A[piv * k + j];
        A[piv * k + j] = t;
        t = Inv[c0 * k + j];
        Inv[c0 * k + j] = Inv[piv * k + j];
        Inv[piv * k + j] = t;
      }
    const double d = A[c0 * k + c0];
    for (int j = 0; j < k; j++) {
      A[c0 * k + j] /= d;
      Inv[c0 * k + j] /= d;
    }
    for (int i = 0; i < k; i++) {
      if (i == c0)
        continue;
      const double f = A[i * k + c0];
      for (int j = 0; j < k; j++) {
        A[i * k + j] -= f * A[c0 * k + j];
        Inv[i * k + j] -= f * Inv[c0 * k + j];
      }
    }
  }
  for (int q = 0; q < 3; q++) {
    double acc = 0.0;
    if (q < k)
      for (int i = 0; i < k; i++)
        acc += Inv[q * k + i] * sys->res[o + i];
    sys->dx_new[q] = acc;
  }
  for (int i = 0; i < k * k; i++)
    sys->Hinv[i] = Inv[i];
  sys->fail = ok ? fail : 0;
  sys->skip = (!ok || fail) ? 1 : 0;
}

void launch_init_prep(ovb_ctx *ctx, int feat, int k, int n) {
  k_init_prep<<<1, 256, 0, ctx->stream>>>(ctx->d_feat + feat, ctx->d_init, ctx->d_info, k, n);
}

__global__ void k_cov_clone(double *P, int ld, int N, int old_off, int size, const int *neg_diag) {
  int idx = blockIdx.x * blockDim.x + threadIdx.x;
  int N2 = N + size;
  if (idx >= N2 * size || (neg_diag && *neg_diag != 0x7fffffff))
    return;
  int i = idx / size, j = idx % size;
  double v;
  if (i < N)
    v = P[(size_t)i * ld + old_off + j];
  else
    v = P[(size_t)(old_off + (i - N)) * ld + old_off + j];
  double vr = (i < N) ? P[(size_t)(old_off + j) * ld + i] : v;
  P[(size_t)i * ld + N + j] = v;
  if (i < N)
    P[(size_t)(N + j) * ld + i] = vr;
}
__global__ void k_cov_dt_cols(double *P, int ld, int N2, int new_off, int size, int dt_off, const double *dnc, const int *neg_diag) {
  int idx = blockIdx.x * blockDim.x + threadIdx.x;
  if (idx >= N2 * size || (neg_diag && *neg_diag != 0x7fffffff))
    return;
  int i = idx / size, j = idx % size;
  P[(size_t)i * ld + new_off + j] += P[(size_t)i * ld + dt_off] * dnc[j];
}
__global__ void k_cov_dt_rows(double *P, int ld, int N2, int new_off, int size, int dt_off, const double *dnc, const int *neg_diag) {
  int idx = blockIdx.x * blockDim.x + threadIdx.x;
  if (idx >= N2 * size || (neg_diag && *neg_diag != 0x7fffffff))
    return;
  int i = idx / N2, j = idx % N2;
  P[(size_t)(new_off + i) * ld + j] += dnc[i] * P[(size_t)dt_off * ld + j];
}

void launch_cov_clone(ovb_ctx *ctx, int old_off, int size, const double *dnc_dt_dev, int dt_off, const int *neg_diag_dev) {
  double *P = ctx->P[ctx->cur];
  int N = ctx->N, N2 = N + size;
  int tot = N2 * size;
  k_cov_clone<<<(tot + 255) / 256, 256, 0, ctx->stream>>>(P, ctx->ldP, N, old_off, size, neg_diag_dev);
  if (dnc_dt_dev) {
    k_cov_dt_cols<<<(tot + 255) / 256, 256, 0, ctx->stream>>>(P, ctx->ldP, N2, N, size, dt_off, dnc_dt_dev, neg_diag_dev);
    k_cov_dt_rows<<<(tot + 255) / 256, 256, 0, ctx->stream>>>(P, ctx->ldP, N2, N, size, dt_off, dnc_dt_dev, neg_diag_dev);
  }
}

__global__ void k_cov_marg(const double *Pin, double *Pout, int ld, int N, int off, int size) {
  int N2 = N - size;
  int i = blockIdx.y * blockDim.y + threadIdx.y, j = blockIdx.x * blockDim.x + threadIdx.x;
  if (i >= N2 || j >= N2)
    return;
  int si = i < off ? i : i + size, sj = j < off ? j : j + size;
  double v = (i >= off && j < off) ? Pin[(size_t)sj * ld + si] : Pin[(size_t)si * ld + sj];
  Pout[(size_t)i * ld + j] = v;
}

void launch_cov_marginalize(ovb_ctx *ctx, int off, int size) {
  int N2 = ctx->N - size;
  dim3 b(32, 8), g((N2 + 31) / 32, (N2 + 7) / 8);
  k_cov_marg<<<g, b, 0, ctx->stream>>>(ctx->P[ctx->cur], ctx->P[ctx->cur ^ 1], ctx->ldP, ctx->N, off, size);
}

__global__ void k_prop_C(const double *P, int ld, int N, int p, int q, const int *old_idx, const double *Phi, double *Cbuf, int ldC) {
  int idx = blockIdx.x * blockDim.x + threadIdx.x;
  if (idx >= N * p)
    return;
  int a = idx / p, j = idx % p;
  double acc = 0.0;
  for (int k = 0; k < q; k++)
    acc += P[(size_t)a * ld + old_idx[k]] * Phi[(size_t)j * q + k];
  Cbuf[(size_t)a * ldC + j] = acc;
}
__global__ void k_prop_PCP(const double *Cbuf, int ldC, int p, int q, const int *old_idx, const double *Phi, const double *Q, double *Sbuf,
                           int ldS) {
  int idx = blockIdx.x * blockDim.x + threadIdx.x;
  if (idx >= p * p)
    return;
  int i = idx / p, j = idx % p;
  double acc = (i <= j) ? Q[(size_t)i * p + j] : Q[(size_t)j * p + i];
  for (int k = 0; k < q; k++)
    acc += Phi[(size_t)i * q + k] * Cbuf[(size_t)old_idx[k] * ldC + j];
  Sbuf[(size_t)i * ldS + j] = acc;
}
__global__ void k_prop_write(double *P, int ld, int N, int new_off, int p, const double *Cbuf, int ldC, const double *Sbuf, int ldS,
                             DevUpdateInfo *info) {
  int idx = blockIdx.x * blockDim.x + threadIdx.x;
  if (idx >= N * p)
    return;
  int a = idx / p, j = idx % p;
  if (a >= new_off && a < new_off + p) {
    double v = Sbuf[(size_t)(a - new_off) * ldS + j];
    P[(size_t)a * ld + new_off + j] = v;
    if (a - new_off == j && v < 0.0)
      atomicMin(&info->neg_diag_index, a);
  } else {
    double v = Cbuf[(size_t)a * ldC + j];
    P[(size_t)a * ld + new_off + j] = v;
    P[(size_t)(new_off + j) * ld + a] = v;
  }
}

void launch_cov_propagate(ovb_ctx *ctx, int new_off, int p, int q, const int *old_idx_dev, const double *Phi_dev, const double *Q_dev) {
  double *P = ctx->P[ctx->cur];
  int N = ctx->N, ld = ctx->ldP;
  ovb_launch(ctx, k_ekf_prep, dim3(1), dim3(1), (size_t)(0), ctx->d_info, (const int *)nullptr);
  k_prop_C<<<(N * p + 255) / 256, 256, 0, ctx->stream>>>(P, ld, N, p, q, old_idx_dev, Phi_dev, ctx->d_M, ld);
  k_prop_PCP<<<(p * p + 255) / 256, 256, 0, ctx->stream>>>(ctx->d_M, ld, p, q, old_idx_dev, Phi_dev, Q_dev, ctx->d_S, ld);
  k_prop_write<<<(N * p + 255) / 256, 256, 0, ctx->stream>>>(P, ld, N, new_off, p, ctx->d_M, ld, ctx->d_S, ld, ctx->d_info);
}

#define PA_THREADS 1024

__device__ __forceinline__ void pa_stage(double *dst, const double *src, int count, int tid) {
  for (int e = tid; e < count; e += PA_THREADS) {
    const unsigned d = (unsigned)__cvta_generic_to_shared(dst + e);
    asm volatile("cp.async.ca.shared.global [%0], [%1], 8;" ::"r"(d), "l"(src + e) : "memory");
  }
}

__global__ void __launch_bounds__(PA_THREADS) k_prop_accumulate(int n, int steps, const double *__restrict__ F, const double *__restrict__ G,
                                                                const double *__restrict__ qc, double *__restrict__ Phi_out,
                                                                double *__restrict__ Q_out) {
  extern __shared__ double pa_sm[];
  const int tid = threadIdx.x, nn = n * n, rec = nn + 12 * n + 4, npairs = n * (n + 1) / 2;
  double *Phi = pa_sm, *Phi2 = Phi + nn, *Q = Phi2 + nn, *T = Q + nn, *stg = T + nn;
  unsigned char *pi = (unsigned char *)(stg + 2 * rec), *pj = pi + npairs;
  for (int e = tid; e < nn; e += PA_THREADS) {
    Phi[e] = (e / n == e % n) ? 1.0 : 0.0;
    Q[e] = 0.0;
  }
  if (tid < n)
    for (int j = tid, t = tid * n - tid * (tid - 1) / 2; j < n; j++, t++)
      pi[t] = (unsigned char)tid, pj[t] = (unsigned char)j;
  auto stage = [&](int s) {
    double *r = stg + (s & 1) * rec;
    pa_stage(r, F + (size_t)s * nn, nn, tid);
    pa_stage(r + nn, G + (size_t)s * 12 * n, 12 * n, tid);
    pa_stage(r + nn + 12 * n, qc + (size_t)s * 4, 4, tid);
    asm volatile("cp.async.commit_group;" ::: "memory");
  };
  if (steps > 0)
    stage(0);
  for (int s = 0; s < steps; s++) {
    asm volatile("cp.async.wait_all;" ::: "memory");
    __syncthreads();
    if (s + 1 < steps)
      stage(s + 1);
    const double *f = stg + (s & 1) * rec, *g = f + nn, *w = g + 12 * n;
    for (int e = tid; e < 2 * nn; e += PA_THREADS) {
      const bool phi = e >= nn;
      const int ee = phi ? e - nn : e, i = ee / n, j = ee % n;
      const double *B = phi ? Phi : Q;
      double acc = 0.0;
      for (int k = 0; k < n; k++)
        acc = __dadd_rn(acc, __dmul_rn(f[i * n + k], B[k * n + j]));
      (phi ? Phi2 : T)[ee] = acc;
    }
    __syncthreads();
    for (int t = tid; t < npairs; t += PA_THREADS) {
      const int i = pi[t], j = pj[t];
      double qij = 0.0, qji = 0.0, tij = 0.0, tji = 0.0;
      for (int k = 0; k < 12; k++) {
        qij = __dadd_rn(qij, __dmul_rn(__dmul_rn(g[i * 12 + k], w[k / 3]), g[j * 12 + k]));
        qji = __dadd_rn(qji, __dmul_rn(__dmul_rn(g[j * 12 + k], w[k / 3]), g[i * 12 + k]));
      }
      for (int k = 0; k < n; k++) {
        tij = __dadd_rn(tij, __dmul_rn(T[i * n + k], f[j * n + k]));
        tji = __dadd_rn(tji, __dmul_rn(T[j * n + k], f[i * n + k]));
      }
      const double qd = __dmul_rn(0.5, __dadd_rn(qij, qji));
      const double v = __dmul_rn(0.5, __dadd_rn(__dadd_rn(tij, qd), __dadd_rn(tji, qd)));
      Q[i * n + j] = v;
      Q[j * n + i] = v;
    }
    double *x = Phi;
    Phi = Phi2, Phi2 = x;
  }
  __syncthreads();
  for (int e = tid; e < nn; e += PA_THREADS) {
    Phi_out[e] = Phi[e];
    Q_out[e] = Q[e];
  }
}

static size_t prop_accumulate_smem(int n) {
  const size_t nn = (size_t)n * n;
  return sizeof(double) * (4 * nn + 2 * (nn + 12 * (size_t)n + 4)) + (size_t)n * (n + 1);
}

bool launch_prop_accumulate(ovb_ctx *ctx, int n, int steps, const double *F_dev, const double *G_dev, const double *qc_dev, double *Phi_dev,
                            double *Q_dev) {
  const size_t smem = prop_accumulate_smem(n);
  if (!ctx->attr_done[7]) {
    if (cudaFuncSetAttribute(k_prop_accumulate, cudaFuncAttributeMaxDynamicSharedMemorySize, (int)prop_accumulate_smem(OVB_PROP_MAX_N)) != cudaSuccess)
      return false;
    ctx->attr_done[7] = 1;
  }
  k_prop_accumulate<<<1, PA_THREADS, smem, ctx->stream>>>(n, steps, F_dev, G_dev, qc_dev, Phi_dev, Q_dev);
  return cudaGetLastError() == cudaSuccess;
}
```

### open_vins_b200/csrc/ovb_api.cu

```cuda
#include "ovb_internal.cuh"
#include <chrono>
#include <algorithm>
#include <cmath>
#include <cstdio>
#include <cstdlib>
#include <cstring>
#include <new>
#include <vector>

static const double g_chi2_table[OVB_CHI2_TABLE_LEN] = {
#include "chi2_table.inc"
};

unsigned char *ovb_feat_order_ptr(ovb_ctx *ctx) { return ctx->d_feat_order; }

static size_t align_up(size_t v, size_t a) { return (v + a - 1) / a * a; }

extern "C" {

static ovb_status ensure_stage(ovb_ctx *ctx, size_t doubles);

int ovb_abi_version(void) { return OVB_ABI_VERSION; }

double ovb_chi2_quantile95(int dof) {
// ... 782 lines not shown
    e = cudaMemcpyAsync(ctx->d_grp, ctx->h_grp, sizeof(DevGroup) * (size_t)pk->n_groups, cudaMemcpyHostToDevice, ctx->stream);
    ctx->last_h2d_bytes += sizeof(DevGroup) * (size_t)pk->n_groups;
  }
  if (e != cudaSuccess) {
    snprintf(ctx->err, sizeof(ctx->err), "H2D arena copy: %s", cudaGetErrorString(e));
    return OVB_ERR_CUDA;
  }
  return OVB_OK;
}

static void unpack_feats(ovb_ctx *ctx, int F, ovb_feat_out *out) {
  if (!out)
    return;
  for (int f = 0; f < F; f++) {
    const DevFeat &d = ctx->h_feat[f];
    if (out->status)
      out->status[f] = d.status;
    if (out->anchor_cam)
      out->anchor_cam[f] = d.anchor_cam;
    if (out->anchor_clone)
      out->anchor_clone[f] = d.anchor_clone;
    if (out->chi2)
      out->chi2[f] = d.chi2;
    for (int k = 0; k < 3; k++) {
      if (out->p_FinA)
        out->p_FinA[3 * f + k] = d.p_FinA[k];
      if (out->p_FinG)
        out->p_FinG[3 * f + k] = d.p_FinG[k];
    }
  }
}

ovb_status ovb_triangulate(ovb_ctx *ctx, const ovb_frame *frame, const ovb_feat_batch *feats, const ovb_opts *opts, ovb_feat_out *out) {
  if (!ctx || !out)
    return OVB_ERR_ARG;
  OVB_CUDA_CHECK(ctx, cudaSetDevice(ctx->device));
  Packed pk;
  int saveN = ctx->N;
  if (ctx->N == 0)
    ctx->N = ctx->cfg.max_state;
  ovb_status st = pack_inputs(ctx, frame, feats, opts, nullptr, &pk, nullptr, false);
  ctx->N = saveN;
  if (st != OVB_OK)
    return st;
  launch_cam_poses(ctx);
  launch_triangulate(ctx, pk.n_feats, pk.bv);
  OVB_CUDA_CHECK(ctx, cudaGetLastError());
  OVB_CUDA_CHECK(ctx, cudaMemcpyAsync(ctx->h_feat, ctx->d_feat, sizeof(DevFeat) * (size_t)pk.n_feats, cudaMemcpyDeviceToHost, ctx->stream));
  OVB_CUDA_CHECK(ctx, cudaStreamSynchronize(ctx->stream));
  unpack_feats(ctx, pk.n_feats, out);
  return OVB_OK;
}

ovb_status ovb_feature_jacobians(ovb_ctx *ctx, const ovb_frame *frame, const ovb_feat_batch *feats, const ovb_opts *opts, ovb_feat_out *out,
                                 int stage, double *Hf_out, double *Hx_out, double *res_out, int32_t *row_off_out, int32_t *ncols_out,
                                 int32_t *col_index_out, int ld_out) {
  if (!ctx || !out || !row_off_out || !ncols_out || !col_index_out)
    return OVB_ERR_ARG;
  if (ctx->N < 1) {
    snprintf(ctx->err, sizeof(ctx->err), "ovb_feature_jacobians: no covariance loaded (ovb_cov_set)");
    return OVB_ERR_ARG;
  }
  OVB_CUDA_CHECK(ctx, cudaSetDevice(ctx->device));
  Packed pk;
  ovb_status st = pack_inputs(ctx, frame, feats, opts, out, &pk);
  if (st != OVB_OK)
    return st;
  const int F = pk.n_feats, n_all = pk.n_all;
  if (ld_out < n_all)
    return OVB_ERR_ARG;
  *ncols_out = n_all;
  for (int s = 0, c = 0; s < ctx->h_frame->n_slots; s++)
    for (int k = 0; k < ctx->h_frame->slot_size[s]; k++)
      col_index_out[c++] = ctx->h_frame->slot_off[s] + k;
  launch_cam_poses(ctx);
  if (stage == 0) {
    int rows = 2 * pk.n_meas;
    size_t need = (size_t)rows * (OVB_MAX_COLS + 4);
    if (!ctx->d_dump || need > ctx->dump_cap) {
      if (ctx->d_dump)
        cudaFree(ctx->d_dump);
      ctx->dump_cap = need;
      OVB_CUDA_CHECK(ctx, cudaMalloc(&ctx->d_dump, sizeof(double) * ctx->dump_cap));
    }
    ctx->dump_rows = rows;
    OVB_CUDA_CHECK(ctx, cudaMemsetAsync(ctx->d_dump, 0, sizeof(double) * need, ctx->stream));
    launch_feature_system(ctx, F, pk.bv, pk.ldH, 1);
    OVB_CUDA_CHECK(ctx, cudaGetLastError());
    std::vector<double> host(need);
    OVB_CUDA_CHECK(ctx, cudaMemcpyAsync(host.data(), ctx->d_dump, sizeof(double) * need, cudaMemcpyDeviceToHost, ctx->stream));
    OVB_CUDA_CHECK(ctx, cudaStreamSynchronize(ctx->stream));
    int dump_rows = rows;
    const double *dHf = host.data(), *dres = host.data() + (size_t)dump_rows * 3, *dHx = host.data() + (size_t)dump_rows * 4;
    for (int f = 0; f <= F; f++)
      row_off_out[f] = 2 * feats->meas_off[f];
    for (int i = 0; i < rows; i++) {
      if (Hf_out)
        for (int k = 0; k < 3; k++)
          Hf_out[(size_t)i * 3 + k] = dHf[(size_t)i * 3 + k];
      if (res_out)
        res_out[i] = dres[i];
      if (Hx_out)
        for (int j = 0; j < n_all; j++)
          Hx_out[(size_t)i * ld_out + j] = dHx[(size_t)i * OVB_MAX_COLS + j];
    }
    return OVB_OK;
  }
  launch_feature_system(ctx, F, pk.bv, pk.ldH, 0);
  OVB_CUDA_CHECK(ctx, cudaGetLastError());
  std::vector<double> host((size_t)pk.m_total * pk.ldH);
  if (pk.m_total > 0)
    OVB_CUDA_CHECK(ctx, cudaMemcpyAsync(host.data(), ctx->d_Hs, sizeof(double) * host.size(), cudaMemcpyDeviceToHost, ctx->stream));
  OVB_CUDA_CHECK(ctx, cudaMemcpyAsync(ctx->h_feat, ctx->d_feat, sizeof(DevFeat) * (size_t)F, cudaMemcpyDeviceToHost, ctx->stream));
  OVB_CUDA_CHECK(ctx, cudaStreamSynchronize(ctx->stream));
  unpack_feats(ctx, F, out);
  for (int f = 0; f < F; f++)
    row_off_out[f] = ctx->h_feat[f].row0;
  row_off_out[F] = pk.m_total;
  for (int i = 0; i < pk.m_total; i++) {
    if (res_out)
      res_out[i] = host[(size_t)i * pk.ldH + n_all];
    if (Hx_out)
      for (int j = 0; j < n_all; j++)
        Hx_out[(size_t)i * ld_out + j] = host[(size_t)i * pk.ldH + j];
  }
  return OVB_OK;
}

static void make_givens(double p, double q, double &gc, double &gs) {
  if (q == 0.0) {
    gc = p < 0.0 ? -1.0 : 1.0;
    gs = 0.0;
  } else if (p == 0.0) {
    gc = 0.0;
    gs = q < 0.0 ? 1.0 : -1.0;
  } else if (std::fabs(p) > std::fabs(q)) {
    const double t = q / p;
    double u = std::sqrt(1.0 + t * t);
    if (p < 0.0)
      u = -u;
    gc = 1.0 / u;
    gs = -t * gc;
  } else {
    const double t = p / q;
    double u = std::sqrt(1.0 + t * t);
    if (q < 0.0)
      u = -u;
    gs = -1.0 / u;
    gc = -t * gs;
  }
}

__global__ void k_take_z(const double *R, int ldR, int rows, int col, double *w);
static int compress_system(ovb_ctx *ctx, int mode, double *A, int m, int n, int ldA, double *Rout, int ldR);

ovb_status ovb_slam_delayed_init(ovb_ctx *ctx, const ovb_frame *frame, const ovb_feat_batch *feats, const ovb_opts *opts, const double *sigma_pix,
                                 const double *chi2_multipler, ovb_init_callback on_init, void *user, ovb_feat_out *out, int32_t *lm_off_out) {
  return ovb_slam_delayed_init_reps(ctx, frame, feats, opts, nullptr, sigma_pix, chi2_multipler, on_init, user, out, lm_off_out);
}

ovb_status ovb_slam_delayed_init_reps(ovb_ctx *ctx, const ovb_frame *frame, const ovb_feat_batch *feats, const ovb_opts *opts,
                                      const int32_t *feat_rep, const double *sigma_pix, const double *chi2_multipler, ovb_init_callback on_init,
                                      void *user, ovb_feat_out *out, int32_t *lm_off_out) {
  if (!ctx || !frame || !feats || !opts || !out || !out->status || !out->p_FinA || !out->p_FinG || !out->anchor_cam || !out->anchor_clone || !lm_off_out)
    return OVB_ERR_ARG;
  const int F = feats->n_feats;
  auto rep_of = [&](int f) { return feat_rep ? feat_rep[f] : opts->feat_rep; };
  int n_single = 0;
  for (int f = 0; f < F; f++) {
    if (rep_of(f) < OVB_REP_GLOBAL_3D || rep_of(f) > OVB_REP_ANCHORED_INVERSE_DEPTH_SINGLE) {
      snprintf(ctx->err, sizeof(ctx->err), "feature %d: representation %d is not an ovb_feat_rep", f, rep_of(f));
      return OVB_ERR_ARG;
    }
    n_single += rep_of(f) == OVB_REP_ANCHORED_INVERSE_DEPTH_SINGLE ? 1 : 0;
  }
  if (n_single > 0 && n_single < F) {
    snprintf(ctx->err, sizeof(ctx->err), "ovb_slam_delayed_init: ANCHORED_INVERSE_DEPTH_SINGLE mixed with a 3-wide representation in one call");
    return OVB_ERR_ARG;
  }
  for (int f = 0; f < F; f++)
    lm_off_out[f] = -1;
  if (F <= 0)
    return OVB_OK;
  int64_t *cnt = ctx->init_counters;
  cnt[0] = cnt[1] = cnt[2] = cnt[3] = 0;
  OVB_CUDA_CHECK(ctx, cudaSetDevice(ctx->device));
  Packed pk;
  const int saveN = ctx->N;
  if (ctx->N == 0)
    ctx->N = ctx->cfg.max_state;
  ovb_status st = pack_inputs(ctx, frame, feats, opts, nullptr, &pk, nullptr, false, feat_rep, sigma_pix, chi2_multipler);
  ctx->N = saveN;
  if (st != OVB_OK)
    return st;
  st = feature_scratch_reserve(ctx, F, false, true);
  if (st != OVB_OK)
    return st;
  cnt[2] += (int64_t)ctx->last_h2d_bytes;
  launch_cam_poses(ctx);
  launch_triangulate(ctx, F, pk.bv);
  OVB_CUDA_CHECK(ctx, cudaGetLastError());
  OVB_CUDA_CHECK(ctx, cudaMemcpyAsync(ctx->h_feat, ctx->d_feat, sizeof(DevFeat) * (size_t)F, cudaMemcpyDeviceToHost, ctx->stream));
  OVB_CUDA_CHECK(ctx, cudaStreamSynchronize(ctx->stream));
  cnt[1]++;
  cnt[3] += (int64_t)(sizeof(DevFeat) * (size_t)F);
  unpack_feats(ctx, F, out);
  if (!ctx->d_init) {
    OVB_CUDA_CHECK(ctx, cudaMalloc(&ctx->d_init, sizeof(DevInitSys)));
    OVB_CUDA_CHECK(ctx, cudaMallocHost(&ctx->h_init, sizeof(DevInitSys)));
  }
  std::vector<int> sched_of(F);
  for (int i = 0; i < F; i++)
    sched_of[ctx->h_feat[i].sched] = i;
  const DevFrame *hf = ctx->h_frame;
  const unsigned char *hkeys = ctx->h_blob + (pk.bv.keys - ctx->d_blob);
  bool moved = false;
  for (int f = 0; f < F; f++) {
    if (out->status[f] != OVB_FEAT_OK)
      continue;
    const DevFeat &d = ctx->h_feat[f];
    const int rep = rep_of(f);
    const int k = rep == OVB_REP_ANCHORED_INVERSE_DEPTH_SINGLE ? 1 : 3;
    const int N0 = ctx->N;
    if (N0 < 1) {
      snprintf(ctx->err, sizeof(ctx->err), "ovb_slam_delayed_init: no covariance loaded (ovb_cov_set)");
      return OVB_ERR_ARG;
    }
    if (!(d.sigma_sq > 0.0))
      return OVB_ERR_ARG;
    if (N0 + k > ctx->ldP) {
      snprintf(ctx->err, sizeof(ctx->err), "initialize: covariance would grow to %d (max_state %d)", N0 + k, ctx->ldP);
      return OVB_ERR_CAPACITY;
    }
    unsigned long long seen = 0ull;
    for (int q = d.key0; q < d.key1; q++) {
      const int key = hkeys[q];
      if (opts->do_calib_camera_pose && hf->cam_ext_slot[key] >= 0)
        seen |= 1ull << hf->cam_ext_slot[key];
      if (opts->do_calib_camera_intrinsics && hf->cam_intr_slot[key] >= 0)
        seen |= 1ull << hf->cam_intr_slot[key];
      for (int i = d.m0; i < d.m1; i++)
        if (feats->cam[i] == key)
          seen |= 1ull << hf->clone_slot[feats->clone[i]];
    }
    if (rep >= OVB_REP_ANCHORED_3D) {
      seen |= 1ull << hf->clone_slot[d.anchor_clone];
      if (opts->do_calib_camera_pose && hf->cam_ext_slot[d.anchor_cam] >= 0)
        seen |= 1ull << hf->cam_ext_slot[d.anchor_cam];
    }
    int n = 0;
    for (int s = 0; s < hf->n_slots; s++)
      if ((seen >> s) & 1ull)
        n += hf->slot_size[s];
    if (n > ctx->cfg.max_state)
      return OVB_ERR_CAPACITY;
    cnt[0]++;
    if (moved) {
      copy_frame_values(ctx->h_frame, frame);
      OVB_CUDA_CHECK(ctx, cudaMemcpyAsync(ctx->d_frame, ctx->h_frame, sizeof(DevFrame), cudaMemcpyHostToDevice, ctx->stream));
      cnt[2] += (int64_t)sizeof(DevFrame);
      launch_cam_poses(ctx);
    }
    launch_feature_init(ctx, sched_of[f], pk.bv, pk.ldH);
    launch_init_prep(ctx, f, k, n);
    const int *skip = &ctx->d_init->skip;
    if (!launch_cov_init_augment(ctx, k, n, ctx->d_init->HR, ctx->d_init->Hinv, d.sigma_sq, skip)) {
      snprintf(ctx->err, sizeof(ctx->err), "ovb_slam_delayed_init: covariance augmentation kernel could not be launched (N=%d, k=%d)", N0, k);
      return OVB_ERR_CAPACITY;
    }
    const double *Hdev = ctx->d_Hs + (size_t)d.row0 * pk.ldH;
    const int rows = 2 * (d.m1 - d.m0) - 3;
    int rr = rows;
    if (rows > n) {
      rr = compress_system(ctx, OVB_COMPRESS_CHOLQR2, ctx->d_Hs + (size_t)d.row0 * pk.ldH, rows, n, pk.ldH, ctx->d_R, pk.ldH);
      Hdev = ctx->d_R;
    }
    ovb_launch(ctx, k_take_z, dim3((rr + 127) / 128), dim3(128), (size_t)(0), Hdev, pk.ldH, rr, n, ctx->d_w);
    ctx->N = N0 + k;
    launch_ekf_update(ctx, Hdev, pk.ldH, rr, n, false, d.sigma_sq, nullptr, skip);
    ctx->N = N0;
    OVB_CUDA_CHECK(ctx, cudaGetLastError());
    const size_t flag_bytes = sizeof(DevUpdateInfo) - offsetof(DevUpdateInfo, neg_diag_index);
    OVB_CUDA_CHECK(ctx, cudaMemcpyAsync(ctx->h_init, ctx->d_init, OVB_INIT_HEAD_BYTES, cudaMemcpyDeviceToHost, ctx->stream));
    OVB_CUDA_CHECK(ctx, cudaMemcpyAsync(&ctx->h_info->neg_diag_index, &ctx->d_info->neg_diag_index, flag_bytes, cudaMemcpyDeviceToHost, ctx->stream));
    OVB_CUDA_CHECK(ctx, cudaMemcpyAsync(ctx->h_dx, ctx->d_dx, sizeof(double) * (size_t)(N0 + k), cudaMemcpyDeviceToHost, ctx->stream));
    OVB_CUDA_CHECK(ctx, cudaStreamSynchronize(ctx->stream));
    cnt[1]++;
    cnt[3] += (int64_t)(OVB_INIT_HEAD_BYTES + flag_bytes + sizeof(double) * (size_t)(N0 + k));
    const DevInitSys *hs = ctx->h_init;
    if (hs->fail == 1) {
      snprintf(ctx->err, sizeof(ctx->err), "initialize: H_L is rank deficient");
      return OVB_ERR_ARG;
    }
    if (hs->fail == 2) {
      snprintf(ctx->err, sizeof(ctx->err), "ovb_slam_delayed_init: feature %d touches %d columns, the host counted %d", f, ctx->h_init->n, n);
      return OVB_ERR_CUDA;
    }
    if (out->chi2)
      out->chi2[f] = hs->chi2;
    if (hs->status != OVB_FEAT_OK) {
      out->status[f] = hs->status;
      continue;
    }
    ctx->N = N0 + k;
    if (ctx->h_info->not_spd) {
      snprintf(ctx->err, sizeof(ctx->err), "EKFUpdate: innovation covariance not positive definite");
      return OVB_ERR_NOT_SPD;
    }
    if (ctx->h_info->nonfinite)
      return OVB_ERR_NONFINITE;
    if (ctx->h_info->neg_diag_index != 0x7fffffff) {
      snprintf(ctx->err, sizeof(ctx->err), "EKFUpdate: diagonal at %d is negative", ctx->h_info->neg_diag_index);
      return OVB_ERR_NEG_DIAG;
    }
    lm_off_out[f] = N0;
    if (on_init) {
      on_init(user, f, N0, k, hs->dx_new, ctx->h_dx, N0 + k);
      moved = true;
    }
  }
  return OVB_OK;
}

ovb_status ovb_last_init_counters(const ovb_ctx *ctx, int64_t out[4]) {
  if (!ctx || !out)
    return OVB_ERR_ARG;
  for (int i = 0; i < 4; i++)
    out[i] = ctx->init_counters[i];
  return OVB_OK;
}

__global__ void k_take_z(const double *R, int ldR, int rows, int col, double *w) {
  OVB_PDL_ENTER();
  int i = blockIdx.x * blockDim.x + threadIdx.x;
  if (i < rows)
    w[i] = R[(size_t)i * ldR + col];
}
__global__ void k_fill_zero_dx(double *dx, int N) {
  int i = blockIdx.x * blockDim.x + threadIdx.x;
  if (i < N)
    dx[i] = 0.0;
}

__global__ void k_group_take_z(const double *__restrict__ R, int ldR, int rows, int n, const int *__restrict__ col_state,
                               const double *__restrict__ dx_acc, double *__restrict__ w, DevUpdateInfo *__restrict__ info) {
  OVB_PDL_ENTER();
  const int i = blockIdx.x * blockDim.x + threadIdx.x;
  if (i < n)
    info->col_state[i] = col_state[i];
  if (i < rows) {
    const double *Ri = R + (size_t)i * ldR;
    double z = Ri[n];
    for (int j = 0; j < n; j++)
      z -= Ri[j] * dx_acc[col_state[j]];
    w[i] = z;
  }
}
__global__ void k_group_accumulate(const double *__restrict__ dx, double *__restrict__ dx_acc, int N, const DevUpdateInfo *__restrict__ info,
                                   int *__restrict__ flags) {
  OVB_PDL_ENTER();
  const int i = blockIdx.x * blockDim.x + threadIdx.x;
  if (i < N)
    dx_acc[i] += dx[i];
  if (i == 0) {
    if (info->not_spd)
      flags[0] = 1;
    if (info->nonfinite)
      flags[1] = 1;
  }
}
__global__ void k_group_finish(double *__restrict__ P, int ldP, int N, const double *__restrict__ P_prior, const double *__restrict__ dx_acc,
                               double *__restrict__ dx, DevUpdateInfo *__restrict__ info, const int *__restrict__ flags) {
  OVB_PDL_ENTER();
  const bool failed = flags[0] || flags[1] || info->neg_diag_index != 0x7fffffff;
  const int j = blockIdx.x * blockDim.x + threadIdx.x, i = blockIdx.y * blockDim.y + threadIdx.y;
  if (i == 0 && j < N)
    dx[j] = failed ? 0.0 : dx_acc[j];
  if (i == 0 && j == 0) {
    info->not_spd = flags[0];
    info->nonfinite = flags[1];
  }
  if (failed && i < N && j < N)
    P[(size_t)i * ldP + j] = P_prior[(size_t)i * ldP + j];
}

static int compress_system(ovb_ctx *ctx, int mode, double *A, int m, int n, int ldA, double *Rout, int ldR) {
  if (mode == OVB_COMPRESS_CHOLQR2 && launch_compress_cholqr2(ctx, A, m, n, ldA, Rout, ldR) >= 0)
    return n;
  if (mode == OVB_COMPRESS_NORMAL_EQUATIONS && launch_compress_gram(ctx, A, m, n, ldA, Rout, ldR) >= 0)
    return n;
  launch_tsqr(ctx, A, m, n, ldA, Rout, ldR);
  return std::min(m, n);
}

static int enqueue_slam_groups(ovb_ctx *ctx, int n_groups, int ldH);
static int enqueue_update(ovb_ctx *ctx, int F, BlobView bv, int ldH, int m_total, int n_all, int col_order, cudaEvent_t *ev,
                          bool slam = false, int n_groups = 1) {
  const int N = ctx->N;
  ctx->n_launch = 0;
  ctx->n_launch_tsqr_level = 0;
  ctx->prof_n = 0;
  if (!slam) {
    launch_cam_poses(ctx);
    launch_triangulate(ctx, F, bv);
    ctx->n_launch += 2;
  }
  ctx->n_launch += 1;
  if (ev)
    cudaEventRecord(ev[1], ctx->stream);
  launch_feature_system(ctx, F, bv, ldH, slam ? 2 : 0);
  if (ev)
    cudaEventRecord(ev[2], ctx->stream);
  {
    cudaEventRecord(ctx->ev_fork, ctx->stream);
    cudaStreamWaitEvent(ctx->side_stream, ctx->ev_fork, 0);
    cudaStream_t main_stream = ctx->stream;
    ctx->stream = ctx->side_stream;
    if (slam) {
      launch_column_map_slam(ctx, F, n_groups == 1);
    } else {
      launch_column_map(ctx, F, bv, 3);
    }
    ctx->stream = main_stream;
    cudaEventRecord(ctx->ev_join, ctx->side_stream);
  }
  if (ev)
    cudaEventRecord(ev[3], ctx->stream);
  if (slam && n_groups > 1) {
    cudaStreamWaitEvent(ctx->stream, ctx->ev_join, 0);
    if (ev)
      cudaEventRecord(ev[4], ctx->stream);
    const int r = enqueue_slam_groups(ctx, n_groups, ldH);
    if (ev)
      cudaEventRecord(ev[5], ctx->stream);
    return r;
  }
  const int ldR = ldH;
  const double *Rfinal = ctx->d_R;
  int r = 0;
  if (m_total > 0) {
    r = compress_system(ctx, ctx->h_opts->o.compress, ctx->d_Hs, m_total, n_all, ldH, ctx->d_R, ldR);
    cudaStreamWaitEvent(ctx->stream, ctx->ev_join, 0);
    if (col_order == OVB_COLS_REFERENCE_FIRST_SEEN) {
      launch_reorder_R(ctx, ctx->d_R, n_all, ldR, ctx->d_R2, ldR);
      Rfinal = ctx->d_R2;
    }
  }
  else
    cudaStreamWaitEvent(ctx->stream, ctx->ev_join, 0);
  if (ev)
    cudaEventRecord(ev[4], ctx->stream);
  if (r > 0) {
    ovb_launch(ctx, k_take_z, dim3((r + 127) / 128), dim3(128), (size_t)(0), Rfinal, ldR, r, n_all, ctx->d_w);
    launch_ekf_update(ctx, Rfinal, ldR, r, n_all, false, slam ? 1.0 : ctx->h_opts->sigma_pix_sq, nullptr);
    ctx->n_launch += 7;
  } else {
    k_fill_zero_dx<<<(N + 127) / 128, 128, 0, ctx->stream>>>(ctx->d_dx, N);
    ctx->n_launch += 1;
  }
  if (ev)
    cudaEventRecord(ev[5], ctx->stream);
  return r;
}

static int enqueue_slam_groups(ovb_ctx *ctx, int n_groups, int ldH) {
  const int N = ctx->N, ld = ctx->ldP;
  double *P = ctx->P[ctx->cur];
  double *acc = ctx->d_grp_acc;
  int *flags = (int *)(acc + ctx->cfg.max_state);
  cudaMemcpyAsync(ctx->P_snap, P, sizeof(double) * (size_t)ld * N, cudaMemcpyDeviceToDevice, ctx->stream);
  cudaMemsetAsync(acc, 0, sizeof(double) * ((size_t)ctx->cfg.max_state + 4), ctx->stream);
  int r_total = 0;
  for (int g = 0; g < n_groups; g++) {
    const DevGroup &G = ctx->h_grp[g];
    if (G.rows == 0)
      continue;
    const int n = G.n_cols;
    const int r = compress_system(ctx, ctx->h_opts->o.compress, ctx->d_Hs + (size_t)G.row0 * ldH, G.rows, n, ldH, ctx->d_R, ldH);
    ovb_launch(ctx, k_group_take_z, dim3((n + 127) / 128), dim3(128), (size_t)0, (const double *)ctx->d_R, ldH, r, n,
               (const int *)ctx->d_grp[g].col_state, (const double *)acc, ctx->d_w, ctx->d_info);
    launch_ekf_update(ctx, ctx->d_R, ldH, r, n, false, 1.0, nullptr);
    ovb_launch(ctx, k_group_accumulate, dim3((N + 255) / 256), dim3(256), (size_t)0, (const double *)ctx->d_dx, acc, N,
               (const DevUpdateInfo *)ctx->d_info, flags);
    ctx->n_launch += 8;
    r_total += r;
  }
  if (r_total > 0) {
    ovb_launch(ctx, k_group_finish, dim3((N + 31) / 32, (N + 7) / 8), dim3(32, 8), (size_t)0, P, ld, N, (const double *)ctx->P_snap,
               (const double *)acc, ctx->d_dx, ctx->d_info, (const int *)flags);
  } else {
    k_fill_zero_dx<<<(N + 127) / 128, 128, 0, ctx->stream>>>(ctx->d_dx, N);
  }
  ctx->n_launch += 1;
  return r_total;
}

ovb_status ovb_set_profile(ovb_ctx *ctx, int enabled) {
  if (!ctx)
    return OVB_ERR_ARG;
  OVB_CUDA_CHECK(ctx, cudaSetDevice(ctx->device));
  if (enabled && ctx->prof_ev[0] == nullptr)
    for (int i = 0; i < 2 * 96; i++)
      OVB_CUDA_CHECK(ctx, cudaEventCreate(&ctx->prof_ev[i]));
  ctx->prof_on = enabled ? 1 : 0;
  ctx->prof_n = 0;
  return OVB_OK;
}

ovb_status ovb_profile_read(ovb_ctx *ctx, char *names, int name_cap, float *us, int cap, int *n) {
  if (!ctx || !names || !us || !n || name_cap < 1)
    return OVB_ERR_ARG;
  OVB_CUDA_CHECK(ctx, cudaSetDevice(ctx->device));
  int w = 0, k = 0;
  for (; k < ctx->prof_n && k < cap; k++) {
    float ms = 0.f;
    if (cudaEventElapsedTime(&ms, ctx->prof_ev[2 * k], ctx->prof_ev[2 * k + 1]) != cudaSuccess)
      cudaGetLastError();
    us[k] = 1e3f * ms;
    const char *nm = nullptr;
    if (cudaFuncGetName(&nm, ctx->prof_fn[k]) != cudaSuccess || !nm) {
      cudaGetLastError();
      nm = "?";
    }
    for (const char *c = nm; *c && w < name_cap - 2; c++)
      names[w++] = *c;
    names[w++] = 0;
  }
  if (w < name_cap)
    names[w] = 0;
  *n = k;
  return OVB_OK;
}

ovb_status ovb_last_host_us(const ovb_ctx *ctx, double out[4]) {
  if (!ctx || !out)
    return OVB_ERR_ARG;
  for (int i = 0; i < 4; i++)
    out[i] = ctx->host_us[i];
  return OVB_OK;
}

ovb_status ovb_last_counters(const ovb_ctx *ctx, int64_t out[4]) {
  if (!ctx || !out)
    return OVB_ERR_ARG;
  out[0] = ctx->n_launch;
  out[1] = ctx->n_launch_tsqr_level;
  out[2] = (int64_t)ctx->last_h2d_bytes;
  out[3] = (int64_t)ctx->last_d2h_bytes;
  return OVB_OK;
}

ovb_status ovb_set_slam_unbounded(ovb_ctx *ctx, int enabled) {
  if (!ctx)
    return OVB_ERR_ARG;
  ctx->slam_unbounded = enabled ? 1 : 0;
  return OVB_OK;
}

ovb_status ovb_set_replay(ovb_ctx *ctx, int enabled) {
  if (!ctx)
    return OVB_ERR_ARG;
  OVB_CUDA_CHECK(ctx, cudaSetDevice(ctx->device));
  if (enabled && !ctx->P_snap)
    OVB_CUDA_CHECK(ctx, cudaMalloc(&ctx->P_snap, sizeof(double) * (size_t)ctx->ldP * ctx->ldP));
  ctx->replay_enabled = enabled ? 1 : 0;
  ctx->last_pk_valid = 0;
  return OVB_OK;
}

ovb_status ovb_msckf_replay(ovb_ctx *ctx, int steps, int flush_l2, float *ms_per_step, float stage_ms_sum[5]) {
  if (!ctx || steps < 1 || !ms_per_step)
    return OVB_ERR_ARG;
  if (!ctx->replay_enabled || !ctx->last_pk_valid) {
    snprintf(ctx->err, sizeof(ctx->err), "ovb_msckf_replay: call ovb_set_replay(ctx,1) and ovb_msckf_update first");
    return OVB_ERR_ARG;
  }
  OVB_CUDA_CHECK(ctx, cudaSetDevice(ctx->device));
  const size_t flush_bytes = (size_t)256 << 20;
  if (flush_l2 && !ctx->d_flush)
    OVB_CUDA_CHECK(ctx, cudaMalloc(&ctx->d_flush, flush_bytes));
  std::vector<cudaEvent_t> evs((size_t)steps * 6);
  for (auto &e : evs)
    OVB_CUDA_CHECK(ctx, cudaEventCreate(&e));
  const size_t Pbytes = sizeof(double) * (size_t)ctx->ldP * ctx->N;
  for (int s = 0; s < steps; s++) {
    if (flush_l2)
      cudaMemsetAsync(ctx->d_flush, s & 0xff, flush_bytes, ctx->stream);
    cudaMemcpyAsync(ctx->P[ctx->cur], ctx->P_snap, Pbytes, cudaMemcpyDeviceToDevice, ctx->stream);
    cudaEvent_t *ev = &evs[(size_t)s * 6];
    cudaEventRecord(ev[0], ctx->stream);
    enqueue_update(ctx, ctx->last_n_feats, ctx->last_bv, ctx->last_ldH, ctx->last_m_total, ctx->last_n_all, ctx->last_col_order,
                   ev);
  }
  OVB_CUDA_CHECK(ctx, cudaGetLastError());
  OVB_CUDA_CHECK(ctx, cudaStreamSynchronize(ctx->stream));
  if (stage_ms_sum)
    for (int k = 0; k < 5; k++)
      stage_ms_sum[k] = 0.f;
  for (int s = 0; s < steps; s++) {
    cudaEvent_t *ev = &evs[(size_t)s * 6];
    cudaEventElapsedTime(&ms_per_step[s], ev[0], ev[5]);
    if (stage_ms_sum)
      for (int k = 0; k < 5; k++) {
        float t;
        cudaEventElapsedTime(&t, ev[k], ev[k + 1]);
        stage_ms_sum[k] += t;
      }
  }
// ... 138 lines not shown
    dx[i] = ctx->h_dx[i];
  ctx->stage_pending = 1;
  cudaEventElapsedTime(&ctx->stage_ms[5], ctx->ev[0], ctx->ev[6]);
  const DevUpdateInfo *inf = ctx->h_info;
  if (stats) {
    stats->n_feats_in = F;
    stats->n_feats_used = inf->n_feats_used;
    stats->rows_stacked = inf->rows_stacked;
    stats->cols_stacked = inf->n_used;
    stats->rows_update = inf->rows_stacked;
    stats->neg_diag_index = (r > 0 && inf->neg_diag_index != 0x7fffffff) ? inf->neg_diag_index : -1;
    stats->ms_total = ctx->stage_ms[5];
  }
  if (r > 0) {
    if (inf->not_spd) {
      snprintf(ctx->err, sizeof(ctx->err), "EKFUpdate: innovation covariance not positive definite");
      return OVB_ERR_NOT_SPD;
    }
    if (inf->nonfinite) {
      snprintf(ctx->err, sizeof(ctx->err), "EKFUpdate: non-finite covariance entry");
      return OVB_ERR_NONFINITE;
    }
    if (inf->neg_diag_index != 0x7fffffff) {
      snprintf(ctx->err, sizeof(ctx->err), "EKFUpdate: diagonal at %d is negative", inf->neg_diag_index);
      return OVB_ERR_NEG_DIAG;
    }
  }
  return OVB_OK;
}

ovb_status ovb_last_stage_ms(const ovb_ctx *ctx, float ms[6]) {
  if (!ctx || !ms)
    return OVB_ERR_ARG;
  if (ctx->stage_pending) {
    for (int s = 0; s < 5; s++)
      cudaEventElapsedTime(&ctx->stage_ms[s], ctx->ev[s], ctx->ev[s + 1]);
    ctx->stage_pending = 0;
  }
  for (int i = 0; i < 6; i++)
    ms[i] = ctx->stage_ms[i];
  return OVB_OK;
}

ovb_status ovb_set_stream(ovb_ctx *ctx, void *cuda_stream) {
  if (!ctx)
    return OVB_ERR_ARG;
  if (!cuda_stream) {
    snprintf(ctx->err, sizeof(ctx->err), "ovb_set_stream: pass an explicit (non-default) CUDA stream handle");
    return OVB_ERR_ARG;
  }
  OVB_CUDA_CHECK(ctx, cudaSetDevice(ctx->device));
  OVB_CUDA_CHECK(ctx, cudaStreamSynchronize(ctx->stream));
  if (ctx->own_stream && ctx->stream)
    cudaStreamDestroy(ctx->stream);
  ctx->stream = (cudaStream_t)cuda_stream;
  ctx->own_stream = 0;
  return OVB_OK;
}

ovb_status ovb_shard_partition(const int32_t *meas_off, int n_feats, int world, int32_t *bounds) {
  if (!meas_off || !bounds || n_feats < 0 || world < 1)
    return OVB_ERR_ARG;
  long long total = 0;
  for (int f = 0; f < n_feats; f++)
    total += std::max(2 * (meas_off[f + 1] - meas_off[f]) - 3, 0);
  bounds[0] = 0;
  long long cum = 0;
  int f = 0;
  for (int r = 1; r < world; r++) {
    const double target = (double)total * r / world;
    while (f < n_feats && (double)cum < target) {
      cum += std::max(2 * (meas_off[f + 1] - meas_off[f]) - 3, 0);
      f++;
    }
    bounds[r] = f;
  }
  bounds[world] = n_feats;
  return OVB_OK;
}

ovb_status ovb_msckf_shard_compress_range(ovb_ctx *ctx, const ovb_frame *frame, const ovb_feat_batch *feats, int f0, int f1, const ovb_opts *opts,
                                          double *R_dev, int R_cap_doubles, int *n_cols, int *ld) {
  if (!ctx || !feats || f0 < 0 || f1 < f0 || f1 > feats->n_feats)
    return OVB_ERR_ARG;
  const int F = f1 - f0, m0 = feats->meas_off[f0], m1 = feats->meas_off[f1];
  std::vector<int32_t> moff((size_t)F + 1), koff;
  for (int f = 0; f <= F; f++)
    moff[(size_t)f] = feats->meas_off[f0 + f] - m0;
  ovb_feat_batch v = *feats;
  v.n_feats = F;
  v.n_meas = m1 - m0;
  v.meas_off = moff.data();
  v.cam = feats->cam + m0;
  v.clone = feats->clone + m0;
  v.uv = feats->uv + 2 * (size_t)m0;
  v.uvn = feats->uvn + 2 * (size_t)m0;
  if (feats->cam_keys_off && feats->cam_keys) {
    const int k0 = feats->cam_keys_off[f0];
    koff.resize((size_t)F + 1);
    for (int f = 0; f <= F; f++)
      koff[(size_t)f] = feats->cam_keys_off[f0 + f] - k0;
    v.cam_keys_off = koff.data();
    v.cam_keys = feats->cam_keys + k0;
  }
  return ovb_msckf_shard_compress(ctx, frame, &v, opts, R_dev, R_cap_doubles, n_cols, ld);
}

ovb_status ovb_msckf_shard_compress(ovb_ctx *ctx, const ovb_frame *frame, const ovb_feat_batch *feats, const ovb_opts *opts, double *R_dev,
                                    int R_cap_doubles, int *n_cols, int *ld) {
  if (!ctx || !frame || !feats || !opts || !R_dev || !n_cols || !ld || ctx->N < 1)
    return OVB_ERR_ARG;
  OVB_CUDA_CHECK(ctx, cudaSetDevice(ctx->device));
  cudaEventRecord(ctx->ev[0], ctx->stream);
  Packed pk;
  ovb_opts o2 = *opts;
  o2.col_order = OVB_COLS_CANONICAL;
  ovb_status st = pack_inputs(ctx, frame, feats, &o2, nullptr, &pk);
  if (st != OVB_OK)
    return st;
  cudaEventRecord(ctx->ev[1], ctx->stream);
  *n_cols = pk.n_all;
  *ld = pk.ldH;
  if ((size_t)pk.n_all * pk.ldH > (size_t)R_cap_doubles)
    return OVB_ERR_CAPACITY;
  ctx->last_n_feats = pk.n_feats;
  ctx->last_n_all = pk.n_all;
  ctx->last_ldH = pk.ldH;
  ctx->n_launch = 0;
  ctx->n_launch_tsqr_level = 0;
  launch_cam_poses(ctx);
  launch_triangulate(ctx, pk.n_feats, pk.bv);
  launch_feature_system(ctx, pk.n_feats, pk.bv, pk.ldH, 0);
  launch_column_map(ctx, pk.n_feats, pk.bv);
  ctx->n_launch += 3;
  if (pk.m_total > 0)
    compress_system(ctx, o2.compress, ctx->d_Hs, pk.m_total, pk.n_all, pk.ldH, R_dev, pk.ldH);
  else
    OVB_CUDA_CHECK(ctx, cudaMemsetAsync(R_dev, 0, sizeof(double) * (size_t)pk.n_all * pk.ldH, ctx->stream));
  cudaEventRecord(ctx->ev[4], ctx->stream);
  OVB_CUDA_CHECK(ctx, cudaGetLastError());
  return OVB_OK;
}

ovb_status ovb_msckf_shard_finish(ovb_ctx *ctx, double *stacked_dev, int n_blocks, ovb_feat_out *out, double *dx, ovb_stats *stats) {
  if (!ctx || !stacked_dev || n_blocks < 1 || !dx || ctx->N < 1)
    return OVB_ERR_ARG;
  OVB_CUDA_CHECK(ctx, cudaSetDevice(ctx->device));
  const int N = ctx->N, n_all = ctx->last_n_all, ld = ctx->last_ldH, F = ctx->last_n_feats;
  const double *Rfinal = stacked_dev;
  if (n_blocks > 1) {
    compress_system(ctx, ctx->h_opts->o.compress, stacked_dev, n_blocks * n_all, n_all, ld, ctx->d_R, ld);
    Rfinal = ctx->d_R;
  }
  ovb_launch(ctx, k_take_z, dim3((n_all + 127) / 128), dim3(128), (size_t)(0), Rfinal, ld, n_all, n_all, ctx->d_w);
  launch_ekf_update(ctx, Rfinal, ld, n_all, n_all, false, ctx->h_opts->sigma_pix_sq, nullptr);
  ctx->n_launch += 7;
  cudaEventRecord(ctx->ev[5], ctx->stream);
  OVB_CUDA_CHECK(ctx, cudaGetLastError());
  OVB_CUDA_CHECK(ctx, cudaMemcpyAsync(ctx->h_feat, ctx->d_feat, sizeof(DevFeat) * (size_t)F, cudaMemcpyDeviceToHost, ctx->stream));
  OVB_CUDA_CHECK(ctx, cudaMemcpyAsync(ctx->h_info, ctx->d_info, ctx->info_bytes + sizeof(double) * (size_t)N, cudaMemcpyDeviceToHost,
                                      ctx->stream));
  ctx->last_d2h_bytes = sizeof(DevFeat) * (size_t)F + ctx->info_bytes + sizeof(double) * (size_t)N;
  cudaEventRecord(ctx->ev[6], ctx->stream);
  OVB_CUDA_CHECK(ctx, cudaStreamSynchronize(ctx->stream));
  unpack_feats(ctx, F, out);
  for (int i = 0; i < N; i++)
    dx[i] = ctx->h_dx[i];
  ctx->stage_pending = 0;
  cudaEventElapsedTime(&ctx->stage_ms[5], ctx->ev[0], ctx->ev[6]);
  cudaEventElapsedTime(&ctx->stage_ms[3], ctx->ev[0], ctx->ev[4]);
  cudaEventElapsedTime(&ctx->stage_ms[4], ctx->ev[4], ctx->ev[5]);
  cudaEventElapsedTime(&ctx->stage_ms[0], ctx->ev[1], ctx->ev[5]);
  const DevUpdateInfo *inf = ctx->h_info;
  if (stats) {
    memset(stats, 0, sizeof(*stats));
    stats->n_feats_in = F;
    int used = 0, rows = 0;
    for (int f = 0; f < F; f++)
      if (ctx->h_feat[f].status == OVB_FEAT_OK) {
        used++;
        rows += 2 * (ctx->h_feat[f].m1 - ctx->h_feat[f].m0) - 3;
      }
    stats->n_feats_used = used;
    stats->rows_stacked = rows;
    stats->cols_stacked = n_all;
    stats->rows_update = n_all;
    stats->neg_diag_index = inf->neg_diag_index != 0x7fffffff ? inf->neg_diag_index : -1;
    stats->ms_total = ctx->stage_ms[5];
  }
  if (inf->not_spd)
    return OVB_ERR_NOT_SPD;
  if (inf->nonfinite)
    return OVB_ERR_NONFINITE;
  if (inf->neg_diag_index != 0x7fffffff)
    return OVB_ERR_NEG_DIAG;
  return OVB_OK;
}

__global__ void k_whiten_rows(double *A, int ld, int m, int ncols) {
  int i = blockIdx.x;
  double s = 1.0 / sqrt(A[(size_t)i * ld + ncols]);
  __syncthreads();
  for (int j = threadIdx.x; j < ncols; j += blockDim.x)
    A[(size_t)i * ld + j] *= s;
}

static ovb_status ensure_stage(ovb_ctx *ctx, size_t doubles) {
  if (doubles <= ctx->stage_cap && ctx->h_stage)
    return OVB_OK;
  if (ctx->h_stage)
    cudaFreeHost(ctx->h_stage);
  ctx->h_stage = nullptr;
  ctx->stage_cap = 0;
  OVB_CUDA_CHECK(ctx, cudaMallocHost(&ctx->h_stage, sizeof(double) * doubles));
  ctx->stage_cap = doubles;
  return OVB_OK;
}

static ovb_status stage_dense(ovb_ctx *ctx, const double *H, int m, int n, const double *res, const double *extra, int *ld_out) {
  int ld = (int)align_up((size_t)n + 2, 4);
  if ((size_t)std::max(m, n) * ld > ctx->Hs_cap) {
    snprintf(ctx->err, sizeof(ctx->err), "dense system %d x %d exceeds the reserved staging matrix (max_rows/max_state)", m, n);
    return OVB_ERR_CAPACITY;
  }
  ovb_status st = ensure_stage(ctx, (size_t)std::max(m, n) * ld);
  if (st != OVB_OK)
    return st;
  double *hs = ctx->h_stage;
  for (int i = 0; i < m; i++) {
    memcpy(hs + (size_t)i * ld, H + (size_t)i * n, sizeof(double) * n);
    hs[(size_t)i * ld + n] = res[i];
    for (int j = n + 1; j < ld; j++)
      hs[(size_t)i * ld + j] = 0.0;
    if (extra)
      hs[(size_t)i * ld + n + 1] = extra[i];
  }
  OVB_CUDA_CHECK(ctx, cudaMemcpyAsync(ctx->d_Hs, hs, sizeof(double) * (size_t)m * ld, cudaMemcpyHostToDevice, ctx->stream));
  *ld_out = ld;
  return OVB_OK;
}

ovb_status ovb_compress(ovb_ctx *ctx, const double *H, int m, int n, const double *res, double *R_out, double *z_out) {
  if (!ctx || !H || !res || !R_out || !z_out || m < 1 || n < 1)
    return OVB_ERR_ARG;
  if (n + 8 > ctx->cfg.max_state + 8)
    return OVB_ERR_CAPACITY;
  OVB_CUDA_CHECK(ctx, cudaSetDevice(ctx->device));
  int ld;
  ovb_status st = stage_dense(ctx, H, m, n, res, nullptr, &ld);
  if (st != OVB_OK)
    return st;
  launch_tsqr(ctx, ctx->d_Hs, m, n, ld, ctx->d_R, ld);
  OVB_CUDA_CHECK(ctx, cudaGetLastError());
  double *hs = ctx->h_stage;
  OVB_CUDA_CHECK(ctx, cudaMemcpyAsync(hs, ctx->d_R, sizeof(double) * (size_t)n * ld, cudaMemcpyDeviceToHost, ctx->stream));
  OVB_CUDA_CHECK(ctx, cudaStreamSynchronize(ctx->stream));
  for (int i = 0; i < n; i++) {
    for (int j = 0; j < n; j++)
      R_out[(size_t)i * n + j] = hs[(size_t)i * ld + j];
    z_out[i] = hs[(size_t)i * ld + n];
  }
  return OVB_OK;
}

ovb_status ovb_compress_gram(ovb_ctx *ctx, const double *H, int m, int n, const double *res, double *R_out, double *z_out) {
  if (!ctx || !H || !res || !R_out || !z_out || m < 1 || n < 1)
    return OVB_ERR_ARG;
  if (n > ctx->cfg.max_state)
    return OVB_ERR_CAPACITY;
  OVB_CUDA_CHECK(ctx, cudaSetDevice(ctx->device));
  int ld;
  ovb_status st = stage_dense(ctx, H, m, n, res, nullptr, &ld);
  if (st != OVB_OK)
    return st;
  if (launch_compress_gram(ctx, ctx->d_Hs, m, n, ld, ctx->d_R, ld) < 0)
    return OVB_ERR_CUDA;
  OVB_CUDA_CHECK(ctx, cudaGetLastError());
  double *hs = ctx->h_stage;
  OVB_CUDA_CHECK(ctx, cudaMemcpyAsync(hs, ctx->d_R, sizeof(double) * (size_t)n * ld, cudaMemcpyDeviceToHost, ctx->stream));
  OVB_CUDA_CHECK(ctx, cudaStreamSynchronize(ctx->stream));
  for (int i = 0; i < n; i++) {
    for (int j = 0; j < n; j++)
      R_out[(size_t)i * n + j] = hs[(size_t)i * ld + j];
    z_out[i] = hs[(size_t)i * ld + n];
  }
  return OVB_OK;
}

ovb_status ovb_compress_cholqr2(ovb_ctx *ctx, const double *H, int m, int n, const double *res, double *R_out, double *z_out) {
  if (!ctx || !H || !res || !R_out || !z_out || m < 1 || n < 1)
    return OVB_ERR_ARG;
  if (n > ctx->cfg.max_state)
    return OVB_ERR_CAPACITY;
  OVB_CUDA_CHECK(ctx, cudaSetDevice(ctx->device));
  int ld;
  ovb_status st = stage_dense(ctx, H, m, n, res, nullptr, &ld);
  if (st != OVB_OK)
    return st;
  if (launch_compress_cholqr2(ctx, ctx->d_Hs, m, n, ld, ctx->d_R, ld) < 0) {
    snprintf(ctx->err, sizeof(ctx->err), "ovb_compress_cholqr2: %d columns exceed what this path takes", n);
    return OVB_ERR_CAPACITY;
  }
  OVB_CUDA_CHECK(ctx, cudaGetLastError());
  double *hs = ctx->h_stage;
  OVB_CUDA_CHECK(ctx, cudaMemcpyAsync(hs, ctx->d_R, sizeof(double) * (size_t)n * ld, cudaMemcpyDeviceToHost, ctx->stream));
  OVB_CUDA_CHECK(ctx, cudaStreamSynchronize(ctx->stream));
  for (int i = 0; i < n; i++) {
    for (int j = 0; j < n; j++)
      R_out[(size_t)i * n + j] = hs[(size_t)i * ld + j];
    z_out[i] = hs[(size_t)i * ld + n];
  }
  return OVB_OK;
}

ovb_status ovb_ekf_update(ovb_ctx *ctx, const int *off, const int *sz, int nvar, const double *H, int r, const double *res, double sigma2,
                          const double *Rdiag, double *dx) {
  if (!ctx || !off || !sz || !H || !res || !dx || nvar < 1 || r < 1)
    return OVB_ERR_ARG;
  if (ctx->N < 1)
    return OVB_ERR_ARG;
  const int N = ctx->N;
  int n = 0;
  for (int i = 0; i < nvar; i++) {
    if (off[i] < 0 || sz[i] < 1 || off[i] + sz[i] > N)
      return OVB_ERR_ARG;
    n += sz[i];
  }
  if (n > OVB_MAX_COLS || n > ctx->cfg.max_state)
    return OVB_ERR_CAPACITY;
  OVB_CUDA_CHECK(ctx, cudaSetDevice(ctx->device));
  if (Rdiag)
    for (int i = 0; i < r; i++)
      if (!(Rdiag[i] > 0.0))
        return OVB_ERR_ARG;
  int ld;
  ovb_status st = stage_dense(ctx, H, r, n, res, Rdiag, &ld);
  if (st != OVB_OK)
    return st;
  DevUpdateInfo *hi = ctx->h_info;
  memset(hi, 0, sizeof(*hi));
  int c = 0;
  for (int i = 0; i < nvar; i++)
    for (int k = 0; k < sz[i]; k++)
      hi->col_state[c++] = off[i] + k;
  OVB_CUDA_CHECK(ctx, cudaMemcpyAsync(ctx->d_info, hi, sizeof(DevUpdateInfo), cudaMemcpyHostToDevice, ctx->stream));
  const double *Hdev = ctx->d_Hs;
  int rr = r;
  double s2 = sigma2;
  if (Rdiag) {
    k_whiten_rows<<<r, 128, 0, ctx->stream>>>(ctx->d_Hs, ld, r, n + 1);
    s2 = 1.0;
  }
  if (r > n) {
    rr = compress_system(ctx, OVB_COMPRESS_CHOLQR2, ctx->d_Hs, r, n, ld, ctx->d_R, ld);
    Hdev = ctx->d_R;
  }
  ovb_launch(ctx, k_take_z, dim3((rr + 127) / 128), dim3(128), (size_t)(0), Hdev, ld, rr, n, ctx->d_w);
  launch_ekf_update(ctx, Hdev, ld, rr, n, false, s2, nullptr);
  OVB_CUDA_CHECK(ctx, cudaGetLastError());
  OVB_CUDA_CHECK(ctx, cudaMemcpyAsync(ctx->h_info, ctx->d_info, sizeof(DevUpdateInfo), cudaMemcpyDeviceToHost, ctx->stream));
  OVB_CUDA_CHECK(ctx, cudaMemcpyAsync(ctx->h_dx, ctx->d_dx, sizeof(double) * (size_t)N, cudaMemcpyDeviceToHost, ctx->stream));
  OVB_CUDA_CHECK(ctx, cudaStreamSynchronize(ctx->stream));
  for (int i = 0; i < N; i++)
    dx[i] = ctx->h_dx[i];
  if (ctx->h_info->not_spd) {
    snprintf(ctx->err, sizeof(ctx->err), "EKFUpdate: innovation covariance not positive definite");
    return OVB_ERR_NOT_SPD;
  }
  if (ctx->h_info->nonfinite)
    return OVB_ERR_NONFINITE;
  if (ctx->h_info->neg_diag_index != 0x7fffffff) {
    snprintf(ctx->err, sizeof(ctx->err), "EKFUpdate: diagonal at %d is negative", ctx->h_info->neg_diag_index);
    return OVB_ERR_NEG_DIAG;
  }
  return OVB_OK;
}

ovb_status ovb_cov_initialize(ovb_ctx *ctx, const int *off, const int *sz, int nvar, const double *H_R_in, const double *H_L_in,
                              const double *res_in, int r, int k, double sigma2, double chi2_mult, int *accepted, double *dx_new, double *dx) {
  if (!ctx || !off || !sz || !H_R_in || !H_L_in || !res_in || !accepted || !dx_new || !dx || nvar < 1 || k < 1 || k > 3 || r < k)
    return OVB_ERR_ARG;
  if (ctx->N < 1 || !(sigma2 > 0.0))
    return OVB_ERR_ARG;
  const int N = ctx->N;
  int n = 0;
  for (int i = 0; i < nvar; i++) {
    if (off[i] < 0 || sz[i] < 1 || off[i] + sz[i] > N)
      return OVB_ERR_ARG;
    n += sz[i];
  }
  if (n > OVB_MAX_COLS || n > ctx->cfg.max_state)
    return OVB_ERR_CAPACITY;
  if (N + k > ctx->ldP) {
    snprintf(ctx->err, sizeof(ctx->err), "initialize: covariance would grow to %d (max_state %d)", N + k, ctx->ldP);
    return OVB_ERR_CAPACITY;
  }
  OVB_CUDA_CHECK(ctx, cudaSetDevice(ctx->device));
  *accepted = 0;
  std::vector<double> HR(H_R_in, H_R_in + (size_t)r * n), HL(H_L_in, H_L_in + (size_t)r * k), res(res_in, res_in + r);
  auto rot = [](double c, double s, double &x, double &y) {
    const double x0 = x, y0 = y;
    x = c * x0 - s * y0;
    y = s * x0 + c * y0;
  };
  for (int c0 = 0; c0 < k; ++c0) {
    for (int m = r - 1; m > c0; m--) {
      double gc, gs;
      make_givens(HL[(size_t)(m - 1) * k + c0], HL[(size_t)m * k + c0], gc, gs);
      for (int j = c0; j < k; j++)
        rot(gc, gs, HL[(size_t)(m - 1) * k + j], HL[(size_t)m * k + j]);
      rot(gc, gs, res[m - 1], res[m]);
      for (int j = 0; j < n; j++)
        rot(gc, gs, HR[(size_t)(m - 1) * n + j], HR[(size_t)m * n + j]);
    }
  }
  double A[9], Inv[9];
  for (int i = 0; i < k; i++)
    for (int j = 0; j < k; j++) {
      A[i * k + j] = HL[(size_t)i * k + j];
      Inv[i * k + j] = (i == j) ? 1.0 : 0.0;
    }
  for (int c0 = 0; c0 < k; c0++) {
    int piv = c0;
    for (int i = c0 + 1; i < k; i++)
      if (std::fabs(A[i * k + c0]) > std::fabs(A[piv * k + c0]))
        piv = i;
    if (!(std::fabs(A[piv * k + c0]) > 0.0)) {
      snprintf(ctx->err, sizeof(ctx->err), "initialize: H_L is rank deficient");
      return OVB_ERR_ARG;
    }
    if (piv != c0)
      for (int j = 0; j < k; j++) {
        std::swap(A[c0 * k + j], A[piv * k + j]);
        std::swap(Inv[c0 * k + j], Inv[piv * k + j]);
      }
    const double d = A[c0 * k + c0];
    for (int j = 0; j < k; j++) {
      A[c0 * k + j] /= d;
      Inv[c0 * k + j] /= d;
    }
    for (int i = 0; i < k; i++) {
      if (i == c0)
        continue;
      const double f = A[i * k + c0];
      for (int j = 0; j < k; j++) {
        A[i * k + j] -= f * A[c0 * k + j];
        Inv[i * k + j] -= f * Inv[c0 * k + j];
      }
    }
  }
  DevUpdateInfo *hi = ctx->h_info;
  memset(hi, 0, sizeof(*hi));
  {
    int c = 0;
    for (int i = 0; i < nvar; i++)
      for (int q = 0; q < sz[i]; q++)
        hi->col_state[c++] = off[i] + q;
  }
  const int rup = r - k;
  const double *Hdev = nullptr;
  int ld = 0, rr = 0;
  if (rup > 0) {
    ovb_status st = stage_dense(ctx, HR.data() + (size_t)k * n, rup, n, res.data() + k, nullptr, &ld);
    if (st != OVB_OK)
      return st;
    OVB_CUDA_CHECK(ctx, cudaMemcpyAsync(ctx->d_info, hi, sizeof(DevUpdateInfo), cudaMemcpyHostToDevice, ctx->stream));
    Hdev = ctx->d_Hs;
    rr = rup;
    double res2 = 0.0;
    for (int i = k; i < r; i++)
      res2 += res[i] * res[i];
    const bool compressed = rup > n;
    if (compressed) {
      launch_tsqr(ctx, ctx->d_Hs, rup, n, ld, ctx->d_R, ld);
      Hdev = ctx->d_R;
      rr = n;
    }
    ovb_launch(ctx, k_take_z, dim3((rr + 127) / 128), dim3(128), (size_t)(0), Hdev, ld, rr, n, ctx->d_w);
    std::vector<double> zh((size_t)rr), wh((size_t)rr);
    OVB_CUDA_CHECK(ctx, cudaMemcpyAsync(zh.data(), ctx->d_w, sizeof(double) * (size_t)rr, cudaMemcpyDeviceToHost, ctx->stream));
    launch_ekf_update(ctx, Hdev, ld, rr, n, true, sigma2, nullptr);
    OVB_CUDA_CHECK(ctx, cudaGetLastError());
    OVB_CUDA_CHECK(ctx, cudaMemcpyAsync(wh.data(), ctx->d_w, sizeof(double) * (size_t)rr, cudaMemcpyDeviceToHost, ctx->stream));
    OVB_CUDA_CHECK(ctx, cudaMemcpyAsync(ctx->h_info, ctx->d_info, sizeof(DevUpdateInfo), cudaMemcpyDeviceToHost, ctx->stream));
    OVB_CUDA_CHECK(ctx, cudaStreamSynchronize(ctx->stream));
    double chi2 = 0.0, z2 = 0.0;
    for (int i = 0; i < rr; i++) {
      chi2 += wh[(size_t)i] * wh[(size_t)i];
      z2 += zh[(size_t)i] * zh[(size_t)i];
    }
    if (compressed)
      chi2 += std::max(0.0, res2 - z2) / sigma2;
    if (ctx->h_info->not_spd)
      chi2 = NAN;
    const double chi2_check = g_chi2_table[std::min(r, OVB_CHI2_TABLE_LEN - 1)];
    if (!(chi2 <= chi2_mult * chi2_check))
      return OVB_OK;
  } else {
    OVB_CUDA_CHECK(ctx, cudaMemcpyAsync(ctx->d_info, hi, sizeof(DevUpdateInfo), cudaMemcpyHostToDevice, ctx->stream));
  }
  {
    std::vector<double> stage((size_t)k * n + (size_t)k * k);
    for (int i = 0; i < k; i++)
      for (int j = 0; j < n; j++)
        stage[(size_t)i * n + j] = HR[(size_t)i * n + j];
    for (int i = 0; i < k * k; i++)
      stage[(size_t)k * n + i] = Inv[i];
    OVB_CUDA_CHECK(ctx, cudaMemcpyAsync(ctx->d_Y, stage.data(), sizeof(double) * stage.size(), cudaMemcpyHostToDevice, ctx->stream));
    const bool launched = launch_cov_init_augment(ctx, k, n, ctx->d_Y, ctx->d_Y + (size_t)k * n, sigma2);
    OVB_CUDA_CHECK(ctx, cudaStreamSynchronize(ctx->stream));
    if (!launched) {
      snprintf(ctx->err, sizeof(ctx->err), "ovb_cov_initialize: covariance augmentation kernel could not be launched (N=%d, k=%d)", N, k);
      return OVB_ERR_CAPACITY;
    }
  }
  ctx->N = N + k;
  for (int q = 0; q < k; q++) {
    double acc = 0.0;
    for (int i = 0; i < k; i++)
      acc += Inv[q * k + i] * res[i];
    dx_new[q] = acc;
  }
  *accepted = 1;
  for (int i = 0; i < N + k; i++)
    dx[i] = 0.0;
  if (rup > 0) {
    ovb_launch(ctx, k_take_z, dim3((rr + 127) / 128), dim3(128), (size_t)(0), Hdev, ld, rr, n, ctx->d_w);
    launch_ekf_update(ctx, Hdev, ld, rr, n, false, sigma2, nullptr);
    OVB_CUDA_CHECK(ctx, cudaGetLastError());
    OVB_CUDA_CHECK(ctx, cudaMemcpyAsync(ctx->h_info, ctx->d_info, sizeof(DevUpdateInfo), cudaMemcpyDeviceToHost, ctx->stream));
    OVB_CUDA_CHECK(ctx, cudaMemcpyAsync(ctx->h_dx, ctx->d_dx, sizeof(double) * (size_t)(N + k), cudaMemcpyDeviceToHost, ctx->stream));
    OVB_CUDA_CHECK(ctx, cudaStreamSynchronize(ctx->stream));
    for (int i = 0; i < N + k; i++)
      dx[i] = ctx->h_dx[i];
    if (ctx->h_info->not_spd) {
      snprintf(ctx->err, sizeof(ctx->err), "EKFUpdate: innovation covariance not positive definite");
      return OVB_ERR_NOT_SPD;
    }
    if (ctx->h_info->nonfinite)
      return OVB_ERR_NONFINITE;
    if (ctx->h_info->neg_diag_index != 0x7fffffff) {
      snprintf(ctx->err, sizeof(ctx->err), "EKFUpdate: diagonal at %d is negative", ctx->h_info->neg_diag_index);
      return OVB_ERR_NEG_DIAG;
    }
  }
  return OVB_OK;
}

}
```

### open_vins_b200/csrc/ovb_internal.cuh

```cuda
#pragma once
#include "../../include/ovb200.h"
#include <cuda_runtime.h>
#include <stdint.h>

#define OVB_BIG_MAX_MEAS 128
#define OVB_MAX_COLS 512
#define OVB_NB 16
#define OVB_CR 256
#define OVB_PROP_MAX_N 64
#define OVB_PROP_STEPS_RESERVE 64

struct DevFrame {
  int n_clones, n_cams;
  int n_slots;
  int n_all;
  double clone_R[OVB_MAX_CLONES][9];
  double clone_p[OVB_MAX_CLONES][3];
  double clone_R_fej[OVB_MAX_CLONES][9];
  double clone_p_fej[OVB_MAX_CLONES][3];
  double cam_R[OVB_MAX_CAMS][9];
  double cam_p[OVB_MAX_CAMS][3];
  double cam_intr[OVB_MAX_CAMS][8];
  int cam_model[OVB_MAX_CAMS];
  int slot_off[OVB_MAX_VARS];
// ... 39 lines not shown
  double chi2;
  double p_FinG_fej[3];
  double sigma_sq;
  double chi2_mult;
  int lm_off;
  unsigned short lm_col, grp;
};

struct DevUpdateInfo {
  int n_used;
  int n_feats_used;
  int rows_stacked;
  int n_order;
  int order_slot[OVB_MAX_VARS];
  int col_state[OVB_MAX_COLS];
  int col_canon[OVB_MAX_COLS];
  int neg_diag_index;
  int not_spd;
  int nonfinite;
};

struct DevInitSys {
  int status;
  int skip;
  int fail;
  int pad;
  double chi2;
  double dx_new[3];
  int n;
  int col_state[OVB_MAX_COLS];
  double HL[9];
  double res[3];
  double HR[3 * OVB_MAX_COLS];
  double Hinv[9];
};
#define OVB_INIT_HEAD_BYTES (4 * sizeof(int) + 4 * sizeof(double))

struct BlobView {
  const uint8_t *cam;
  const uint16_t *clone;
  const float *uv;
  const float *uvn;
  const uint8_t *keys;
};

struct ovb_ctx {
  ovb_config cfg;
  int device;
  cudaStream_t stream;
  int own_stream;
  cudaStream_t side_stream;
  cudaStream_t side_stream2;
  cudaEvent_t ev_fork, ev_join, ev_join2;
  int feat_classes;
  cudaEvent_t ev[8];
  char err[256];
  int N, ldP;
  double *P[2];
  int cur;
  unsigned char *d_arena, *h_arena;
  size_t arena_bytes, off_opts, off_feat, off_blob;
  DevFrame *d_frame;
  DevOpts *d_opts;
  DevFeat *d_feat;
  unsigned char *d_blob;
  DevFrame *h_frame;
  DevOpts *h_opts;
  DevFeat *h_feat;
  unsigned char *h_blob;
  size_t blob_cap;
  DevCamPoses *d_cc;
  unsigned char *d_feat_order;
  DevUpdateInfo *d_info;
  DevUpdateInfo *h_info;
  double *h_dx;
  double *h_stage;
  size_t stage_cap;
  double *d_chi2_table;
  double *d_Hs;
  size_t Hs_cap;
  double *d_W[2];
  size_t W_cap;
  double *d_R;
  double *d_R2;
  double *d_M;
  double *d_S;
  double *d_Y;
  double *d_w;
  double *d_dx;
  double *d_scratch;
  size_t scratch_per_cta;
  int scratch_ctas;
  double *d_long;
  size_t long_cap;
  double *d_dump;
  size_t dump_cap;
  int dump_rows;
  int max_rows;
  int sm_count;
  size_t info_bytes;
  int attr_done[8];
  int tsqr_pdl;
  int tsqr_cluster;
  int gram_cluster;
  int ekf_chol_dmma;
  mutable float stage_ms[6];
  mutable int stage_pending;
  double host_us[4];
  int replay_enabled, last_pk_valid;
  int last_n_feats, last_m_total, last_ldH, last_n_all, last_col_order;
  BlobView last_bv;
  double *P_snap;
  void *d_flush;
  DevGroup *d_grp, *h_grp;
  int grp_cap;
  double *d_grp_acc;
  int slam_unbounded;
  int n_launch, n_launch_tsqr_level;
  double *d_Gpart, *d_G;
  size_t Gpart_cap, G_cap;
  double *d_cqw;
  size_t cqw_cap;
  unsigned long long *d_pub;
  unsigned long long pub_epoch;
  size_t last_h2d_bytes, last_d2h_bytes;
  DevInitSys *d_init, *h_init;
  int64_t init_counters[4];
  double *d_imu, *h_imu;
  size_t imu_cap;
  int prof_on, prof_n;
  cudaEvent_t prof_ev[2 * 96];
  const void *prof_fn[96];
};

#define OVB_CUDA_CHECK(ctx, call)                                                                                     \
  do {                                                                                                                \
    cudaError_t e_ = (call);                                                                                          \
    if (e_ != cudaSuccess) {                                                                                          \
      snprintf((ctx)->err, sizeof((ctx)->err), "%s:%d %s: %s", __FILE__, __LINE__, #call, cudaGetErrorString(e_));    \
      return OVB_ERR_CUDA;                                                                                            \
    }                                                                                                                 \
  } while (0)

void launch_cam_poses(ovb_ctx *ctx);
void launch_triangulate(ovb_ctx *ctx, int n_feats, BlobView bv);
void launch_feature_system(ovb_ctx *ctx, int n_feats, BlobView bv, int ldH, int mode);
ovb_status feature_scratch_reserve(ovb_ctx *ctx, int n_feats, bool slam, bool init = false);
void launch_feature_init(ovb_ctx *ctx, int sched, BlobView bv, int ldH);
void launch_init_prep(ovb_ctx *ctx, int feat, int k, int n);
void launch_column_map(ovb_ctx *ctx, int n_feats, BlobView bv, int rows_drop = 3);
void launch_column_map_slam(ovb_ctx *ctx, int n_feats, bool full_map);
void launch_tsqr(ovb_ctx *ctx, double *A, int m, int n, int ldA, double *Rout, int ldR);
int launch_compress_gram(ovb_ctx *ctx, const double *A, int m, int n, int ldA, double *Rout, int ldR);
int launch_compress_cholqr2(ovb_ctx *ctx, double *A, int m, int n, int ldA, double *Rout, int ldR);
bool launch_chol_ekf_dmma(ovb_ctx *ctx, double *S, int ldS, int r, const double *res, double *w, double *invdiag, double **Lpk_out,
                          unsigned long long *epoch_out);
bool launch_trsm_rows(ovb_ctx *ctx, double *A, int ldA, int m, int nt, const double *Lpk, unsigned long long epoch);
bool launch_chol_solve_wide(ovb_ctx *ctx, double *S, int ldS, int r, double *w, double *invdiag, double *M, int ldM, int N, bool gate_only);
void launch_reorder_R(ovb_ctx *ctx, const double *Rin, int n_all, int ldRin, double *Rout, int ldRout);
void launch_ekf_update(ovb_ctx *ctx, const double *H, int ldHm, int r, int n, bool gate_only, double sigma2, const double *Rdiag_dev,
                       const int *skip_dev = nullptr);
bool launch_cov_init_augment(ovb_ctx *ctx, int k, int n, const double *Hx_dev, const double *Hinv_dev, double sigma2,
                             const int *skip_dev = nullptr);
void launch_cov_clone(ovb_ctx *ctx, int old_off, int size, const double *dnc_dt_dev, int dt_off, const int *neg_diag_dev = nullptr);
void launch_cov_marginalize(ovb_ctx *ctx, int off, int size);
void launch_cov_propagate(ovb_ctx *ctx, int new_off, int p, int q, const int *old_idx_dev, const double *Phi_dev, const double *Q_dev);
bool launch_prop_accumulate(ovb_ctx *ctx, int n, int steps, const double *F_dev, const double *G_dev, const double *qc_dev, double *Phi_dev,
                            double *Q_dev);

#define OVB_PDL_ENTER()                                                     \
  do {                                                                      \
    asm volatile("griddepcontrol.launch_dependents;" ::: "memory");         \
    asm volatile("griddepcontrol.wait;" ::: "memory");                      \
  } while (0)

#ifdef __CUDACC__
template <typename... KArgs, typename... Args>
static inline void ovb_launch(ovb_ctx *ctx, void (*kern)(KArgs...), dim3 grid, dim3 block, size_t smem, Args &&...args) {
  cudaLaunchConfig_t cfg = {};
  cfg.gridDim = grid;
  cfg.blockDim = block;
  cfg.dynamicSmemBytes = smem;
  cfg.stream = ctx->stream;
  cudaLaunchAttribute at[1];
  at[0].id = cudaLaunchAttributeProgrammaticStreamSerialization;
  at[0].val.programmaticStreamSerializationAllowed = 1;
  cfg.attrs = at;
  cfg.numAttrs = (ctx->tsqr_pdl && !ctx->prof_on) ? 1 : 0;
  const bool prof = ctx->prof_on && ctx->prof_n < 96 && ctx->prof_ev[0] != nullptr;
  if (prof)
    cudaEventRecord(ctx->prof_ev[2 * ctx->prof_n], ctx->stream);
  cudaLaunchKernelEx(&cfg, kern, static_cast<KArgs>(args)...);
  if (prof) {
    cudaEventRecord(ctx->prof_ev[2 * ctx->prof_n + 1], ctx->stream);
    ctx->prof_fn[ctx->prof_n++] = (const void *)kern;
  }
}
#endif
```

Baseline: 2544.

## Stream second Cholesky columns into TRMM and fold z extraction into prep

The second Gram Cholesky now publishes finished columns through the epoch counter, using a dedicated publisher warp synchronised with named barriers. The TRMM kernel triggers its dependents early and polls for the columns it needs, so it can overlap with the factorisation. The residual z is also written directly by TRMM, or copied by the EKF prep kernel, which removes the separate k_take_z launch. The prep launch for info flags moves to the side stream. In exchange this adds polling-based synchronisation with a timeout fallback and a more intricate barrier protocol.

```diff
diff --git a/open_vins_b200/csrc/chol_tiles.cuh b/open_vins_b200/csrc/chol_tiles.cuh
--- a/open_vins_b200/csrc/chol_tiles.cuh
+++ b/open_vins_b200/csrc/chol_tiles.cuh
@@ -229,6 +229,7 @@
 }
 
 struct CtNoPublish {
+  static constexpr bool streams = false;
   __device__ __forceinline__ void column(const CtView &, int) const {}
 };
 template <int THREADS, typename PUB = CtNoPublish>
@@ -236,6 +237,7 @@
   const int tid = threadIdx.x, lane = tid & 31, wid = tid >> 5;
   constexpr int NW = THREADS / 32, NH = NW - (NW + 3) / 4;
   static_assert(NH >= 1, "need at least one helper warp");
+  static_assert(!PUB::streams || NW >= 9, "a publisher needs warp 8");
   const bool helper = (wid & 3) != 0;
   const int hr = wid - 1 - (wid >> 2);
   constexpr bool LINV = NW >= 8;
@@ -256,6 +258,17 @@
     ct_linv8(sm.T, sm.invd, sm.Linv0);
   }
   __syncthreads();
+  if constexpr (PUB::streams) {
+    if (wid == 8) {
+      asm volatile("bar.arrive 0, %0;" ::"n"(THREADS) : "memory");
+      for (int k = 0; k + 1 < NB; k++) {
+        asm volatile("bar.sync 4, %0;" ::"n"(THREADS) : "memory");
+        asm volatile("bar.arrive 0, %0;" ::"n"(THREADS) : "memory");
+        pub.column(sm, k);
+      }
+      return;
+    }
+  }
   for (int k = 0; k < NB; k++) {
     const int par = k & 1;
     double *Xk = par ? sm.Xp1 : sm.Xp0, *Xn = par ? sm.Xp0 : sm.Xp1;
@@ -319,10 +332,14 @@
         }
       }
       CT_PROBE_T(p3);
-    } else if (wid == 8 && k > 0) {
-      pub.column(sm, k - 1);
-    }
-    __syncthreads();
+    }
+    if constexpr (PUB::streams) {
+      asm volatile("bar.sync 0, %0;" ::"n"(THREADS) : "memory");
+      if (k + 1 < NB)
+        asm volatile("bar.arrive 4, %0;" ::"n"(THREADS) : "memory");
+    } else {
+      __syncthreads();
+    }
     CT_PROBE_T(p5);
 #ifdef CQ_PROBE
     if (wid == 0) {
diff --git a/open_vins_b200/csrc/k_cholqr.cu b/open_vins_b200/csrc/k_cholqr.cu
--- a/open_vins_b200/csrc/k_cholqr.cu
+++ b/open_vins_b200/csrc/k_cholqr.cu
@@ -39,6 +39,11 @@
   unsigned long long v;
   asm volatile("ld.acquire.gpu.global.u64 %0, [%1];" : "=l"(v) : "l"(ctr) : "memory");
   return v;
+}
+__device__ __forceinline__ unsigned long long cq_globaltimer() {
+  unsigned long long t;
+  asm volatile("mov.u64 %0, %%globaltimer;" : "=l"(t));
+  return t;
 }
 __device__ __forceinline__ void cq_fence_proxy() { asm volatile("fence.proxy.async.global;" ::: "memory"); }
 __device__ __forceinline__ void cq_mbar_init(unsigned bar) { asm volatile("mbarrier.init.shared::cta.b64 [%0], 1;" ::"r"(bar) : "memory"); }
@@ -271,6 +276,7 @@
 namespace {
 
 struct CqPublish {
+  static constexpr bool streams = true;
   double *Lpk;
   unsigned long long *ctr, epoch;
   int n;
@@ -590,23 +596,22 @@
 
 #define CQ_STREAM_POLL_NS 20000000ull
 
+__device__ __forceinline__ void cq_stream_reach(const unsigned long long *ctr, unsigned long long v, unsigned long long t0, bool &poll) {
+  while (poll && cq_pub_load(ctr) < v) {
+    if (cq_globaltimer() - t0 > CQ_STREAM_POLL_NS) {
+      asm volatile("griddepcontrol.wait;" ::: "memory");
+      poll = false;
+    } else {
+      __nanosleep(64);
+    }
+  }
+}
+
 __device__ void cq_stream_fetch(unsigned long long *bars, double *Lt, double *Ri, const double *__restrict__ Lpk, int NB, int NBP,
                                 const unsigned long long *ctr, unsigned long long epoch) {
-  const unsigned long long base = epoch << 6;
-  unsigned long long t0, t;
-  asm volatile("mov.u64 %0, %%globaltimer;" : "=l"(t0));
+  const unsigned long long base = epoch << 6, t0 = cq_globaltimer();
   bool poll = true;
-  auto reach = [&](int s) {
-    while (poll && cq_pub_load(ctr) < (base | (unsigned long long)s)) {
-      asm volatile("mov.u64 %0, %%globaltimer;" : "=l"(t));
-      if (t - t0 > CQ_STREAM_POLL_NS) {
-        asm volatile("griddepcontrol.wait;" ::: "memory");
-        poll = false;
-      } else {
-        __nanosleep(64);
-      }
-    }
-  };
+  auto reach = [&](int s) { cq_stream_reach(ctr, base | (unsigned long long)s, t0, poll); };
   reach(1);
   cq_mbar_arrive(s_u32(bars));
   for (int j = NB; j < NBP; j++)
@@ -903,14 +908,21 @@
     cq_launch_solve_gram_t<10, 10>(ctx, nslab, A, ldA, m, nt, Lpk, slab_rows, BW, Gpart, Qtail, pub_ctr, epoch);
 }
 
-__global__ void __launch_bounds__(256) k_cq_trmm(const double *__restrict__ L2, const double *__restrict__ L1, int nt, double *__restrict__ Rout, int ldR) {
-  OVB_PDL_ENTER();
+__global__ void __launch_bounds__(256) k_cq_trmm(const double *L2, const double *L1, int nt, double *__restrict__ Rout, int ldR,
+                                                 const unsigned long long *pub_ctr, unsigned long long epoch, double *__restrict__ z_out) {
+  asm volatile("griddepcontrol.launch_dependents;" ::: "memory");
   __shared__ double As[16][CQ_MAXN + 1];
   __shared__ double Bs[CQ_MAXN][17];
   const int ti = blockIdx.y, tj = blockIdx.x;
   const int tid = threadIdx.x, tx = tid & 15, ty = tid >> 4;
   const int n = nt - 1;
   const int i = ti * 16 + ty, j = tj * 16 + tx;
+  if (tid == 0) {
+    const int NB = (nt + 7) >> 3, last = min(2 * ti + 1, NB - 1);
+    bool poll = true;
+    cq_stream_reach(pub_ctr, (epoch << 6) | (unsigned long long)(tj >= ti ? 2 + last : 1), cq_globaltimer(), poll);
+  }
+  __syncthreads();
   double acc = 0.0;
   if (tj >= ti) {
     const int k0 = ti * 16, k1 = min(nt, tj * 16 + 16);
@@ -918,12 +930,12 @@
     for (int e = tid; e < 16 * K; e += 256) {
       const int a = e / K, k = e - a * K;
       const int ii = ti * 16 + a, kk = k0 + k;
-      As[a][k] = (ii < nt && kk >= ii) ? L2[(size_t)(tri(kk >> 3) + (ii >> 3)) * 64 + (kk & 7) * 8 + (ii & 7)] : 0.0;
+      As[a][k] = (ii < nt && kk >= ii) ? __ldcg(L2 + (size_t)(tri(kk >> 3) + (ii >> 3)) * 64 + (kk & 7) * 8 + (ii & 7)) : 0.0;
     }
     for (int e = tid; e < 16 * K; e += 256) {
       const int k = e >> 4, b = e & 15;
       const int kk = k0 + k, jj = tj * 16 + b;
-      Bs[k][b] = (jj < nt && jj >= kk) ? L1[(size_t)(tri(jj >> 3) + (kk >> 3)) * 64 + (jj & 7) * 8 + (kk & 7)] : 0.0;
+      Bs[k][b] = (jj < nt && jj >= kk) ? __ldcg(L1 + (size_t)(tri(jj >> 3) + (kk >> 3)) * 64 + (jj & 7) * 8 + (kk & 7)) : 0.0;
     }
     __syncthreads();
     double a0 = 0.0, a1 = 0.0, a2 = 0.0, a3 = 0.0;
@@ -940,6 +952,10 @@
   }
   if (i < n && j < nt)
     Rout[(size_t)i * ldR + j] = (j >= i) ? acc : 0.0;
+  if (z_out != nullptr && i < n && j == n)
+    z_out[i] = acc;
+  if (tid == 0)
+    asm volatile("griddepcontrol.wait;" ::: "memory");
 }
 
 #define CQ_GN_T 256
@@ -1307,7 +1323,7 @@
   return launches + 1;
 }
 
-int launch_compress_cholqr2(ovb_ctx *ctx, double *A, int m, int n, int ldA, double *Rout, int ldR) {
+int launch_compress_cholqr2(ovb_ctx *ctx, double *A, int m, int n, int ldA, double *Rout, int ldR, double *z_out, bool *z_written) {
   const int nt = n + 1;
   if ((ldA & 1) || m < 1)
     return -1;
@@ -1351,9 +1367,13 @@
   ovb_launch(ctx, k_cq_chol_gram, dim3(1), dim3(CQ_CHOL_T), sizeof(CqCholSmem), (const double *)G, ldW, nt, 1e-11, L1, 1, ctx->d_pub, epoch);
   cq_launch_solve_gram(ctx, nslab, (const double *)A, ldA, m, nt, (const double *)L1, slab_rows, BW, ctx->d_Gpart, ctx->d_Gpart + part_doubles, ctx->d_pub, epoch);
   ovb_launch(ctx, k_cq_reduce, dim3(CQ_RED_GX, nblk), dim3(CQ_RED_T), (size_t)0, (const double *)ctx->d_Gpart, nslab, nblk, BW, nblk_side, nt, G, ldW, 1);
-  ovb_launch(ctx, k_cq_chol_gram, dim3(1), dim3(CQ_CHOL_T), sizeof(CqCholSmem), (const double *)G, ldW, nt, 1e-13, L2, 1, (unsigned long long *)nullptr, 0ull);
+  const unsigned long long epoch2 = ++ctx->pub_epoch;
+  ovb_launch(ctx, k_cq_chol_gram, dim3(1), dim3(CQ_CHOL_T), sizeof(CqCholSmem), (const double *)G, ldW, nt, 1e-13, L2, 1, ctx->d_pub, epoch2);
   const int nT16 = (nt + 15) / 16;
-  ovb_launch(ctx, k_cq_trmm, dim3(nT16, nT16), dim3(256), (size_t)0, (const double *)L2, (const double *)L1, nt, Rout, ldR);
+  ovb_launch(ctx, k_cq_trmm, dim3(nT16, nT16), dim3(256), (size_t)0, (const double *)L2, (const double *)L1, nt, Rout, ldR, (const unsigned long long *)ctx->d_pub,
+             epoch2, z_out);
+  if (z_out != nullptr)
+    *z_written = true;
   ctx->n_launch += 7;
   return 7;
 }
diff --git a/open_vins_b200/csrc/k_ekf.cu b/open_vins_b200/csrc/k_ekf.cu
--- a/open_vins_b200/csrc/k_ekf.cu
+++ b/open_vins_b200/csrc/k_ekf.cu
@@ -368,19 +368,32 @@
   }
 }
 
-__global__ void k_ekf_prep(DevUpdateInfo *info, const int *skip) {
+__global__ void k_ekf_prep(DevUpdateInfo *info, const int *skip, const double *__restrict__ zsrc, int ldz, int rows, int col, double *__restrict__ w) {
   OVB_PDL_ENTER();
-  info->neg_diag_index = 0x7fffffff;
-  info->not_spd = (skip && *skip) ? 1 : 0;
-  info->nonfinite = 0;
-}
+  if (blockIdx.x == 0 && threadIdx.x == 0) {
+    info->neg_diag_index = 0x7fffffff;
+    info->not_spd = (skip && *skip) ? 1 : 0;
+    info->nonfinite = 0;
+  }
+  const int i = blockIdx.x * blockDim.x + threadIdx.x;
+  if (zsrc != nullptr && i < rows)
+    w[i] = zsrc[(size_t)i * ldz + col];
+}
+
+static void launch_ekf_prep_skip(ovb_ctx *ctx, const int *skip_dev) {
+  ovb_launch(ctx, k_ekf_prep, dim3(1), dim3(1), (size_t)(0), ctx->d_info, skip_dev, (const double *)nullptr, 0, 0, 0, (double *)nullptr);
+}
+void launch_ekf_prep(ovb_ctx *ctx) { launch_ekf_prep_skip(ctx, nullptr); }
 
 void launch_ekf_update(ovb_ctx *ctx, const double *H, int ldHm, int r, int n, bool gate_only, double sigma2, const double *Rdiag_dev,
-                       const int *skip_dev) {
+                       const int *skip_dev, bool z_in_H, bool info_ready) {
   const int N = ctx->N;
   const int ld = ctx->ldP;
   double *P = ctx->P[ctx->cur];
-  ovb_launch(ctx, k_ekf_prep, dim3(1), dim3(1), (size_t)(0), ctx->d_info, skip_dev);
+  if (z_in_H && r > 0)
+    ovb_launch(ctx, k_ekf_prep, dim3((r + 127) / 128), dim3(128), (size_t)(0), ctx->d_info, skip_dev, H, ldHm, r, n, ctx->d_w);
+  else if (!info_ready)
+    launch_ekf_prep_skip(ctx, skip_dev);
   if (r <= 0 || n <= 0)
     return;
   if (!ctx->attr_done[2]) {
@@ -672,7 +685,7 @@
 void launch_cov_propagate(ovb_ctx *ctx, int new_off, int p, int q, const int *old_idx_dev, const double *Phi_dev, const double *Q_dev) {
   double *P = ctx->P[ctx->cur];
   int N = ctx->N, ld = ctx->ldP;
-  ovb_launch(ctx, k_ekf_prep, dim3(1), dim3(1), (size_t)(0), ctx->d_info, (const int *)nullptr);
+  launch_ekf_prep(ctx);
   k_prop_C<<<(N * p + 255) / 256, 256, 0, ctx->stream>>>(P, ld, N, p, q, old_idx_dev, Phi_dev, ctx->d_M, ld);
   k_prop_PCP<<<(p * p + 255) / 256, 256, 0, ctx->stream>>>(ctx->d_M, ld, p, q, old_idx_dev, Phi_dev, Q_dev, ctx->d_S, ld);
   k_prop_write<<<(N * p + 255) / 256, 256, 0, ctx->stream>>>(P, ld, N, new_off, p, ctx->d_M, ld, ctx->d_S, ld, ctx->d_info);
diff --git a/open_vins_b200/csrc/ovb_api.cu b/open_vins_b200/csrc/ovb_api.cu
--- a/open_vins_b200/csrc/ovb_api.cu
+++ b/open_vins_b200/csrc/ovb_api.cu
@@ -958,7 +958,8 @@
 }
 
 __global__ void k_take_z(const double *R, int ldR, int rows, int col, double *w);
-static int compress_system(ovb_ctx *ctx, int mode, double *A, int m, int n, int ldA, double *Rout, int ldR);
+static int compress_system(ovb_ctx *ctx, int mode, double *A, int m, int n, int ldA, double *Rout, int ldR, double *z_out = nullptr,
+                           bool *z_written = nullptr);
 
 ovb_status ovb_slam_delayed_init(ovb_ctx *ctx, const ovb_frame *frame, const ovb_feat_batch *feats, const ovb_opts *opts, const double *sigma_pix,
                                  const double *chi2_multipler, ovb_init_callback on_init, void *user, ovb_feat_out *out, int32_t *lm_off_out) {
@@ -1081,9 +1082,8 @@
       rr = compress_system(ctx, OVB_COMPRESS_CHOLQR2, ctx->d_Hs + (size_t)d.row0 * pk.ldH, rows, n, pk.ldH, ctx->d_R, pk.ldH);
       Hdev = ctx->d_R;
     }
-    ovb_launch(ctx, k_take_z, dim3((rr + 127) / 128), dim3(128), (size_t)(0), Hdev, pk.ldH, rr, n, ctx->d_w);
     ctx->N = N0 + k;
-    launch_ekf_update(ctx, Hdev, pk.ldH, rr, n, false, d.sigma_sq, nullptr, skip);
+    launch_ekf_update(ctx, Hdev, pk.ldH, rr, n, false, d.sigma_sq, nullptr, skip, true);
     ctx->N = N0;
     OVB_CUDA_CHECK(ctx, cudaGetLastError());
     const size_t flag_bytes = sizeof(DevUpdateInfo) - offsetof(DevUpdateInfo, neg_diag_index);
@@ -1190,8 +1190,8 @@
     P[(size_t)i * ldP + j] = P_prior[(size_t)i * ldP + j];
 }
 
-static int compress_system(ovb_ctx *ctx, int mode, double *A, int m, int n, int ldA, double *Rout, int ldR) {
-  if (mode == OVB_COMPRESS_CHOLQR2 && launch_compress_cholqr2(ctx, A, m, n, ldA, Rout, ldR) >= 0)
+static int compress_system(ovb_ctx *ctx, int mode, double *A, int m, int n, int ldA, double *Rout, int ldR, double *z_out, bool *z_written) {
+  if (mode == OVB_COMPRESS_CHOLQR2 && launch_compress_cholqr2(ctx, A, m, n, ldA, Rout, ldR, z_out, z_written) >= 0)
     return n;
   if (mode == OVB_COMPRESS_NORMAL_EQUATIONS && launch_compress_gram(ctx, A, m, n, ldA, Rout, ldR) >= 0)
     return n;
@@ -1211,7 +1211,7 @@
     launch_triangulate(ctx, F, bv);
     ctx->n_launch += 2;
   }
-  ctx->n_launch += 1;
+  ctx->n_launch += 2;
   if (ev)
     cudaEventRecord(ev[1], ctx->stream);
   launch_feature_system(ctx, F, bv, ldH, slam ? 2 : 0);
@@ -1227,6 +1227,7 @@
     } else {
       launch_column_map(ctx, F, bv, 3);
     }
+    launch_ekf_prep(ctx);
     ctx->stream = main_stream;
     cudaEventRecord(ctx->ev_join, ctx->side_stream);
   }
@@ -1244,8 +1245,10 @@
   const int ldR = ldH;
   const double *Rfinal = ctx->d_R;
   int r = 0;
+  bool z_staged = false;
   if (m_total > 0) {
-    r = compress_system(ctx, ctx->h_opts->o.compress, ctx->d_Hs, m_total, n_all, ldH, ctx->d_R, ldR);
+    r = compress_system(ctx, ctx->h_opts->o.compress, ctx->d_Hs, m_total, n_all, ldH, ctx->d_R, ldR,
+                        col_order == OVB_COLS_REFERENCE_FIRST_SEEN ? nullptr : ctx->d_w, &z_staged);
     cudaStreamWaitEvent(ctx->stream, ctx->ev_join, 0);
     if (col_order == OVB_COLS_REFERENCE_FIRST_SEEN) {
       launch_reorder_R(ctx, ctx->d_R, n_all, ldR, ctx->d_R2, ldR);
@@ -1257,9 +1260,8 @@
   if (ev)
     cudaEventRecord(ev[4], ctx->stream);
   if (r > 0) {
-    ovb_launch(ctx, k_take_z, dim3((r + 127) / 128), dim3(128), (size_t)(0), Rfinal, ldR, r, n_all, ctx->d_w);
-    launch_ekf_update(ctx, Rfinal, ldR, r, n_all, false, slam ? 1.0 : ctx->h_opts->sigma_pix_sq, nullptr);
-    ctx->n_launch += 7;
+    launch_ekf_update(ctx, Rfinal, ldR, r, n_all, false, slam ? 1.0 : ctx->h_opts->sigma_pix_sq, nullptr, nullptr, !z_staged, true);
+    ctx->n_launch += z_staged ? 5 : 6;
   } else {
     k_fill_zero_dx<<<(N + 127) / 128, 128, 0, ctx->stream>>>(ctx->d_dx, N);
     ctx->n_launch += 1;
@@ -1704,9 +1706,8 @@
     compress_system(ctx, ctx->h_opts->o.compress, stacked_dev, n_blocks * n_all, n_all, ld, ctx->d_R, ld);
     Rfinal = ctx->d_R;
   }
-  ovb_launch(ctx, k_take_z, dim3((n_all + 127) / 128), dim3(128), (size_t)(0), Rfinal, ld, n_all, n_all, ctx->d_w);
-  launch_ekf_update(ctx, Rfinal, ld, n_all, n_all, false, ctx->h_opts->sigma_pix_sq, nullptr);
-  ctx->n_launch += 7;
+  launch_ekf_update(ctx, Rfinal, ld, n_all, n_all, false, ctx->h_opts->sigma_pix_sq, nullptr, nullptr, true);
+  ctx->n_launch += 6;
   cudaEventRecord(ctx->ev[5], ctx->stream);
   OVB_CUDA_CHECK(ctx, cudaGetLastError());
   OVB_CUDA_CHECK(ctx, cudaMemcpyAsync(ctx->h_feat, ctx->d_feat, sizeof(DevFeat) * (size_t)F, cudaMemcpyDeviceToHost, ctx->stream));
@@ -1907,8 +1908,7 @@
     rr = compress_system(ctx, OVB_COMPRESS_CHOLQR2, ctx->d_Hs, r, n, ld, ctx->d_R, ld);
     Hdev = ctx->d_R;
   }
-  ovb_launch(ctx, k_take_z, dim3((rr + 127) / 128), dim3(128), (size_t)(0), Hdev, ld, rr, n, ctx->d_w);
-  launch_ekf_update(ctx, Hdev, ld, rr, n, false, s2, nullptr);
+  launch_ekf_update(ctx, Hdev, ld, rr, n, false, s2, nullptr, nullptr, true);
   OVB_CUDA_CHECK(ctx, cudaGetLastError());
   OVB_CUDA_CHECK(ctx, cudaMemcpyAsync(ctx->h_info, ctx->d_info, sizeof(DevUpdateInfo), cudaMemcpyDeviceToHost, ctx->stream));
   OVB_CUDA_CHECK(ctx, cudaMemcpyAsync(ctx->h_dx, ctx->d_dx, sizeof(double) * (size_t)N, cudaMemcpyDeviceToHost, ctx->stream));
@@ -2077,8 +2077,7 @@
   for (int i = 0; i < N + k; i++)
     dx[i] = 0.0;
   if (rup > 0) {
-    ovb_launch(ctx, k_take_z, dim3((rr + 127) / 128), dim3(128), (size_t)(0), Hdev, ld, rr, n, ctx->d_w);
-    launch_ekf_update(ctx, Hdev, ld, rr, n, false, sigma2, nullptr);
+    launch_ekf_update(ctx, Hdev, ld, rr, n, false, sigma2, nullptr, nullptr, true);
     OVB_CUDA_CHECK(ctx, cudaGetLastError());
     OVB_CUDA_CHECK(ctx, cudaMemcpyAsync(ctx->h_info, ctx->d_info, sizeof(DevUpdateInfo), cudaMemcpyDeviceToHost, ctx->stream));
     OVB_CUDA_CHECK(ctx, cudaMemcpyAsync(ctx->h_dx, ctx->d_dx, sizeof(double) * (size_t)(N + k), cudaMemcpyDeviceToHost, ctx->stream));
diff --git a/open_vins_b200/csrc/ovb_internal.cuh b/open_vins_b200/csrc/ovb_internal.cuh
--- a/open_vins_b200/csrc/ovb_internal.cuh
+++ b/open_vins_b200/csrc/ovb_internal.cuh
@@ -215,14 +215,15 @@
 void launch_column_map_slam(ovb_ctx *ctx, int n_feats, bool full_map);
 void launch_tsqr(ovb_ctx *ctx, double *A, int m, int n, int ldA, double *Rout, int ldR);
 int launch_compress_gram(ovb_ctx *ctx, const double *A, int m, int n, int ldA, double *Rout, int ldR);
-int launch_compress_cholqr2(ovb_ctx *ctx, double *A, int m, int n, int ldA, double *Rout, int ldR);
+int launch_compress_cholqr2(ovb_ctx *ctx, double *A, int m, int n, int ldA, double *Rout, int ldR, double *z_out = nullptr, bool *z_written = nullptr);
 bool launch_chol_ekf_dmma(ovb_ctx *ctx, double *S, int ldS, int r, const double *res, double *w, double *invdiag, double **Lpk_out,
                           unsigned long long *epoch_out);
 bool launch_trsm_rows(ovb_ctx *ctx, double *A, int ldA, int m, int nt, const double *Lpk, unsigned long long epoch);
 bool launch_chol_solve_wide(ovb_ctx *ctx, double *S, int ldS, int r, double *w, double *invdiag, double *M, int ldM, int N, bool gate_only);
 void launch_reorder_R(ovb_ctx *ctx, const double *Rin, int n_all, int ldRin, double *Rout, int ldRout);
 void launch_ekf_update(ovb_ctx *ctx, const double *H, int ldHm, int r, int n, bool gate_only, double sigma2, const double *Rdiag_dev,
-                       const int *skip_dev = nullptr);
+                       const int *skip_dev = nullptr, bool z_in_H = false, bool info_ready = false);
+void launch_ekf_prep(ovb_ctx *ctx);
 bool launch_cov_init_augment(ovb_ctx *ctx, int k, int n, const double *Hx_dev, const double *Hinv_dev, double sigma2,
                              const int *skip_dev = nullptr);
 void launch_cov_clone(ovb_ctx *ctx, int old_off, int size, const double *dnc_dt_dev, int dt_off, const int *neg_diag_dev = nullptr);
```

New measurement: 2624, median of 6. 1.03x the previous value.
